# laiviet/ed-gated-gcn

Measured on AMD Instinct MI355X. Metric: gated_gcn_forward_edges_per_sec, higher is better.
Workload: dtype f32 (fp16 MFMA + block-scaled fp8 correction MFMA, fp32 accumulate)

## Files before the change

### ed-gated-gcn_amd/_capi.py

```python
import ctypes
import os

_HERE = os.path.dirname(os.path.abspath(__file__))
_LIB = None

c_i32, c_i64, c_vp, c_sz = ctypes.c_int, ctypes.c_int64, ctypes.c_void_p, ctypes.c_size_t

PROTOTYPES = {
    "ggcn_abi_version": (c_i32, []),
    "ggcn_has_f16mx6": (c_i32, []),
    "ggcn_last_error": (ctypes.c_char_p, []),
    "ggcn_csr_workspace_bytes": (c_sz, [c_i64]),
    "ggcn_csr_from_dense": (c_i32, [c_vp, c_i32, c_i32, c_i32, c_i64, c_i64, c_i64, c_vp, c_vp, c_vp,
                                    c_i64, c_vp, c_vp, c_vp, c_vp]),
    "ggcn_rowmask_from_dense": (c_i32, [c_vp, c_i32, c_i32, c_i32, c_i64, c_i64, c_i64, c_vp, c_vp, c_vp]),
    "ggcn_csr_transpose": (c_i32, [c_vp, c_vp, c_vp, c_i32, c_i32, c_vp, c_vp, c_vp, c_vp, c_vp]),
    "ggcn_csr_rowmask": (c_i32, [c_vp, c_vp, c_i32, c_i32, c_vp, c_vp]),
    "ggcn_graph_edge_lists_bytes": (c_sz, [c_i32]),
    "ggcn_graph_edge_lists": (c_i32, [c_vp, c_i32, c_i32, c_vp, c_vp]),
    "ggcn_graph_operands_bytes": (c_sz, [c_i32]),
    "ggcn_graph_operands": (c_i32, [c_vp, c_i32, c_i32, c_vp, c_vp]),
    "ggcn_graph_operands2_bytes": (c_sz, [c_i32]),
    "ggcn_graph_operands2": (c_i32, [c_vp, c_i32, c_i32, c_i32, c_vp, c_vp]),
    "ggcn_graph_operands_weighted": (c_i32, [c_vp, c_vp, c_vp, c_i32, c_i32, c_i32, c_vp, c_vp, c_vp]),
    "ggcn_layer_fused_weighted": (c_i32, [c_vp, c_i64, c_vp, c_vp, c_vp, c_vp, c_i32, c_i32, c_i32, c_i32, c_vp, c_vp, c_vp,
                                          c_vp, c_i64, c_vp, c_vp, c_vp, c_vp, c_vp, c_i32, c_vp]),
    "ggcn_layer_fused": (c_i32, [c_vp, c_i64, c_vp, c_vp, c_vp, c_vp, c_i32, c_i32, c_i32, c_i32, c_vp, c_vp, c_vp,
                                 c_vp, c_i64, c_vp, c_vp, c_vp, c_vp, c_vp, c_i32, c_vp]),
    "ggcn_layer_fused_prebias": (c_i32, [c_vp, c_i64, c_vp, c_vp, c_vp, c_vp, c_i32, c_i32, c_i32, c_i32, c_vp, c_vp, c_vp,
                                         c_vp, c_i64, c_vp, c_vp, c_i32, c_vp]),
    "ggcn_block_fused": (c_i32, [c_vp, c_i64, c_vp, c_vp, c_vp, c_vp, c_vp, c_vp, c_vp, c_i32, c_i32, c_i32, c_i32,
                                 c_vp, c_vp, c_vp, c_i64, c_vp, c_i64, c_vp, c_vp, c_vp, c_vp, c_i32, c_vp]),
    "ggcn_overlap_reduce": (c_i32, [c_vp, c_i32, c_i32, c_vp, c_vp]),
    "ggcn_transpose": (c_i32, [c_vp, c_i32, c_i32, c_i64, c_vp, c_vp]),
    "ggcn_gate_mlp": (c_i32, [c_vp, c_i64, c_i32, c_i32, c_vp, c_vp, c_vp, c_vp, c_vp, c_vp, c_vp, c_vp, c_vp, c_vp, c_vp]),
    "ggcn_scores_head": (c_i32, [c_vp, c_i64, c_vp, c_i64, c_vp, c_i64, c_vp, c_i64, c_vp, c_vp, c_i64, c_i32, c_i32,
                                 c_i32, c_i32, c_vp, c_i64, c_vp, c_vp]),
    "ggcn_absmax": (c_i32, [c_vp, c_i32, c_i64, c_i64, c_i32, c_vp, c_vp]),
    "ggcn_range_flag": (c_i32, [c_vp, c_i32, c_vp]),
    "ggcn_debug_poison_lds": (c_i32, [ctypes.c_uint32, c_vp]),
    "ggcn_lab_block_fused8": (c_i32, [c_vp, c_i64, c_vp, c_vp, c_vp, c_vp, c_vp, c_vp, c_vp, c_i32, c_i32, c_i32, c_i32, c_vp, c_vp,
                                      c_vp, c_i64, c_vp, c_vp, c_vp, c_vp, c_vp, c_vp]),
    "ggcn_debug_mfma_calibrate": (c_i32, [c_i32, c_i32, c_vp, c_vp, c_vp]),
    "ggcn_debug_block_fused_stamped": (c_i32, [c_vp, c_i64, c_vp, c_vp, c_vp, c_vp, c_vp, c_vp, c_vp, c_i32, c_i32, c_i32, c_i32,
                                               c_vp, c_vp, c_vp, c_i64, c_vp, c_i64, c_vp, c_vp, c_vp, c_vp, c_i32, c_vp, c_vp]),
    "ggcn_subword_pool": (c_i32, [c_vp, c_i64, c_i64, c_i64, c_vp, c_i64, c_i64, c_vp, c_i64, c_i64,
                                  c_i32, c_i32, c_i32, c_i32, c_vp]),
    "ggcn_subword_pool_bf16": (c_i32, [c_vp, c_i64, c_i64, c_i64, c_vp, c_i64, c_i64, c_vp, c_i64, c_i64,
                                       c_i32, c_i32, c_i32, c_i32, c_vp]),
    "ggcn_linear_bf16": (c_i32, [c_vp, c_i64, c_vp, c_vp, c_i64, c_i64, c_i32, c_i32, c_vp]),
    "ggcn_linear_out_bf16": (c_i32, [c_vp, c_i64, c_vp, c_vp, c_i64, c_i64, c_i32, c_i32, c_vp]),
    "ggcn_layer_fused_bf16": (c_i32, [c_vp, c_i64, c_vp, c_vp, c_vp, c_i32, c_i32, c_i32, c_i32, c_vp, c_vp, c_vp,
                                      c_vp, c_i64, c_vp, c_vp, c_vp, c_vp, c_vp, c_vp]),
    "ggcn_layer_fused_bf16_drop": (c_i32, [c_vp, c_i64, c_vp, c_vp, c_vp, c_i32, c_i32, c_i32, c_i32, c_vp, c_vp, c_vp,
                                           c_vp, c_i64, c_vp, c_vp, c_vp, c_vp, c_vp,
                                           ctypes.c_float, ctypes.c_uint64, c_i32, c_i32, c_i32, c_vp]),
    "ggcn_layer_fused_bf16_wide": (c_i32, [c_vp, c_i64, c_vp, c_vp, c_vp, c_vp, c_i32, c_i32, c_i32, c_i32, c_vp, c_vp, c_vp,
                                           c_vp, c_i64, c_vp, c_vp, c_vp, c_vp, c_vp,
                                           ctypes.c_float, ctypes.c_uint64, c_i32, c_i32, c_i32, c_vp]),
    "ggcn_block_fused_bf16": (c_i32, [c_vp, c_i64, c_vp, c_vp, c_vp, c_vp, c_vp, c_vp, c_vp, c_i32, c_i32, c_i32, c_i32,
                                      c_vp, c_vp, c_vp, c_i64, c_vp, c_i64, c_vp, c_vp, c_vp, c_vp, c_vp]),
    "ggcn_aggregate_bf16": (c_i32, [c_vp, c_i64, c_vp, c_vp, c_vp, c_i32, c_i32, c_i32, c_vp, c_i64, c_vp]),
    "ggcn_dweight_bf16_workspace_bytes": (c_sz, [c_i64, c_i32, c_i32]),
    "ggcn_dweight_bf16": (c_i32, [c_vp, c_i64, c_vp, c_i64, c_i64, c_i32, c_i32, c_vp, c_i64, c_vp, c_vp]),
    "ggcn_weight_pack_bytes": (c_sz, [c_i32, c_i32, c_i32]),
    "ggcn_weight_pack": (c_i32, [c_vp, c_i64, c_i32, c_i32, c_i32, c_i32, c_vp, c_vp]),
    "ggcn_linear": (c_i32, [c_vp, c_i64, c_vp, c_i64, c_vp, c_vp, c_i64, c_i64, c_i32, c_i32, c_i32, c_vp]),
    "ggcn_aggregate": (c_i32, [c_vp, c_i64, c_vp, c_vp, c_vp, c_vp, c_i32, c_i32, c_i32, c_vp, c_vp, c_vp,
                               c_vp, c_i64, c_vp, c_vp, c_vp]),
    "ggcn_gate_pool_backward": (c_i32, [c_vp, c_i64, c_vp, c_vp, c_vp, c_vp, c_i64, c_vp, c_vp, c_i32, c_i32, c_i32,
                                        c_vp, c_i64, c_vp, c_vp, c_vp, c_vp, c_vp]),
    "ggcn_gate_pool_backward_drop": (c_i32, [c_vp, c_i64, c_vp, c_vp, c_vp, c_vp, c_i64, c_vp, c_vp, c_i32, c_i32, c_i32,
                                             c_vp, c_i64, c_vp, c_vp, c_vp, c_vp, ctypes.c_float, ctypes.c_uint64, c_i32, c_i32, c_i32, c_vp]),
    "ggcn_gate_pool_backward_agg": (c_i32, [c_vp, c_i64, c_vp, c_vp, c_vp, c_vp, c_i64, c_vp, c_vp, c_vp, c_i32, c_i32, c_i32,
                                            c_vp, c_i64, c_vp, c_vp, c_vp, c_vp, ctypes.c_float, ctypes.c_uint64, c_i32, c_i32, c_i32, c_vp, c_vp]),
    "ggcn_rowmask_transpose": (c_i32, [c_vp, c_i32, c_i32, c_vp, c_vp]),
    "ggcn_gate_pool_backward_mma": (c_i32, [c_vp, c_i64, c_vp, c_vp, c_vp, c_vp, c_i64, c_vp, c_vp, c_vp, c_vp, c_i32, c_i32, c_i32,
                                            c_vp, c_i64, c_vp, c_vp, c_vp, c_vp, c_vp, c_vp]),
    "ggcn_linear_scaled": (c_i32, [c_vp, c_i64, c_vp, c_vp, c_i64, c_i64, c_i32, c_i32, c_vp, c_vp]),
    "ggcn_layer_fused_drop": (c_i32, [c_vp, c_i64, c_vp, c_vp, c_vp, c_vp, c_i32, c_i32, c_i32, c_i32, c_vp, c_vp, c_vp,
                                      c_vp, c_i64, c_vp, c_vp, c_i32, ctypes.c_float, ctypes.c_uint64, c_i32, c_i32, c_i32, c_vp]),
    "ggcn_dropout_mask": (c_i32, [c_i64, c_i32, ctypes.c_float, ctypes.c_uint64, c_i32, c_vp, c_vp]),
    "ggcn_colsum_workspace_bytes": (c_sz, [c_i32]),
    "ggcn_colsum": (c_i32, [c_vp, c_i64, c_i64, c_i32, c_vp, c_vp, c_vp]),
    "ggcn_dweight_workspace_bytes": (c_sz, [c_i64, c_i32, c_i32, c_i32]),
    "ggcn_dweight": (c_i32, [c_vp, c_i64, c_vp, c_i64, c_i64, c_i32, c_i32, c_vp, c_i64, c_i32, c_vp, c_vp]),
    "ggcn_inv_denominators": (c_i32, [c_vp, c_vp, c_i64, c_vp, c_vp]),
    "ggcn_aggregate_t": (c_i32, [c_vp, c_i64, c_vp, c_vp, c_vp, c_vp, c_i32, c_i32, c_i32, c_vp, c_i64, c_vp]),
    "ggcn_adjacency_grad": (c_i32, [c_vp, c_i64, c_vp, c_i64, c_vp, c_vp, c_vp, c_vp, c_i32, c_i32, c_i32, c_vp, c_vp]),
    "ggcn_linear_h": (c_i32, [c_vp, c_i64, c_vp, c_vp, c_i64, c_i64, c_i32, c_i32, c_i32, c_vp]),
    "ggcn_aggregate_h": (c_i32, [c_vp, c_i64, c_vp, c_vp, c_vp, c_vp, c_i32, c_i32, c_i32, c_vp, c_vp, c_vp,
                                 c_vp, c_i64, c_vp, c_vp, c_vp]),
    "ggcn_layer_fused_h": (c_i32, [c_vp, c_i64, c_vp, c_vp, c_vp, c_vp, c_vp, c_i32, c_i32, c_i32, c_i32, c_vp, c_vp, c_vp,
                                   c_vp, c_i64, c_vp, c_vp, c_vp]),
    "ggcn_block_fused_form": (c_i32, [c_i32, c_i32, c_i32, c_i32]),
    "ggcn_dense_head": (c_i32, [c_vp, c_i64, c_vp, c_i64, c_vp, c_i32, c_i32, c_i32, c_vp, c_i64, c_vp, c_i32, c_vp, c_vp]),
    "ggcn_dense_head_signal": (c_i32, [c_vp, c_i64, c_vp, c_i64, c_vp, c_i32, c_i32, c_i32, c_vp, c_i64, c_vp, c_i32, c_vp, c_vp, c_vp]),
    "ggcn_overlap_workspace_bytes": (c_sz, [c_i32]),
    "ggcn_gate_overlap": (c_i32, [c_vp, c_vp, c_i32, c_i32, c_vp, c_vp, c_vp]),
}

ABI_VERSION = 14
PREC = {"bf16x3": 0, "fp32": 1, "f16mx8": 2, "f16": 3, "f16mx6": 4}
PACKED = ("bf16x3", "f16mx8", "f16", "f16mx6")
FLAG_WEIGHTED = 1
RANGE_OVERFLOW, RANGE_WINDOW, RANGE_HIDDEN = 1, 2, 4


def has_f16mx6():
    return bool(load_library().ggcn_has_f16mx6())


def lib_path():
    return os.environ.get("GGCN_LIB", os.path.join(_HERE, "libggcn_hip.so"))


def load_library():
    global _LIB
    if _LIB is not None:
        return _LIB
    path = lib_path()
    if not os.path.exists(path):
        raise RuntimeError(
            "libggcn_hip.so not found at %s: build it with `python -c 'import __graft_entry__ as g; "
            "g.build()'` or `make -C ed-gated-gcn_amd/csrc` (no CPU fallback exists)" % path)
    lib = ctypes.CDLL(path)
    for name, (res, args) in PROTOTYPES.items():
        fn = getattr(lib, name)
        fn.restype, fn.argtypes = res, args
    if lib.ggcn_abi_version() != ABI_VERSION:
        raise RuntimeError("libggcn_hip.so ABI %d != binding ABI %d" % (lib.ggcn_abi_version(), ABI_VERSION))
    _LIB = lib
    return lib


def check(rc, what):
    if rc != 0:
        msg = load_library().ggcn_last_error().decode("utf-8", "replace")
        raise RuntimeError("%s failed (code %d): %s" % (what, rc, msg))


def ptr(t):
    return None if t is None else ctypes.c_void_p(t.data_ptr())


def stream_of(device):
    import torch
    return ctypes.c_void_p(torch.cuda.current_stream(device).cuda_stream)
```

### ed-gated-gcn_amd/csrc/capi.hip

```cpp
#include "common.h"
#include <cstdlib>
#include "dropout_hash.h"

#include <cstring>

namespace ggcn {

char *error_buffer()
{
    static thread_local char buf[512] = "";
    return buf;
}

int fail(int code, const char *fmt, ...)
{
    va_list ap;
    va_start(ap, fmt);
    vsnprintf(error_buffer(), 512, fmt, ap);
    va_end(ap);
    return code;
}

}

using namespace ggcn;

extern "C" {

int ggcn_abi_version(void) { return GGCN_ABI_VERSION; }

int ggcn_has_f16mx6(void)
{
#ifdef GGCN_WITH_F16MX6
    return 1;
#else
    return 0;
#endif
}

const char *ggcn_last_error(void) { return error_buffer(); }

size_t ggcn_csr_workspace_bytes(int64_t n_rows) { return csr_workspace_bytes(n_rows); }

int ggcn_csr_from_dense(const void *adj, int adj_dtype, int B, int T, int64_t stride_b,
                        int64_t stride_r, int64_t stride_c, int32_t *rowptr, int32_t *colidx,
                        float *vals, int64_t capacity, uint32_t *rowmask, int32_t *flags,
                        void *workspace, ggcn_stream_t stream)
{
    return csr_from_dense(adj, adj_dtype, B, T, stride_b, stride_r, stride_c, rowptr, colidx, vals,
                          capacity, rowmask, flags, workspace, as_stream(stream));
}

int ggcn_csr_transpose(const int32_t *rowptr, const int32_t *colidx, const float *vals, int B, int T,
                       int32_t *rowptr_t, int32_t *colidx_t, float *vals_t, void *workspace, ggcn_stream_t stream)
{
    return csr_transpose(rowptr, colidx, vals, B, T, rowptr_t, colidx_t, vals_t, workspace, as_stream(stream));
}

int ggcn_rowmask_from_dense(const void *adj, int adj_dtype, int B, int T, int64_t stride_b, int64_t stride_r,
                            int64_t stride_c, uint32_t *rowmask, int32_t *flags, ggcn_stream_t stream)
{
    return rowmask_from_dense(adj, adj_dtype, B, T, stride_b, stride_r, stride_c, rowmask, flags, as_stream(stream));
}

int ggcn_csr_rowmask(const int32_t *rowptr, const int32_t *colidx, int B, int T, uint32_t *rowmask,
                     ggcn_stream_t stream)
{
    return csr_rowmask(rowptr, colidx, B, T, rowmask, as_stream(stream));
}

size_t ggcn_graph_operands_bytes(int B) { return B > 0 ? (size_t)B * GGCN_GRAPH_OPS_BYTES : 0; }
size_t ggcn_graph_operands2_bytes(int B) { return B > 0 ? (size_t)B * GGCN_GRAPH_OPS2_BYTES : 0; }
int ggcn_graph_operands2(const uint32_t *rowmask, int B, int T, int plane, void *graph_ops2, ggcn_stream_t stream)
{
    return graph_operands2(rowmask, B, T, plane, graph_ops2, as_stream(stream));
}

size_t ggcn_graph_edge_lists_bytes(int B) { return B > 0 ? (size_t)B * GGCN_EDGE_LISTS_BYTES : 0; }

int ggcn_graph_edge_lists(const uint32_t *rowmask, int B, int T, void *lists, ggcn_stream_t stream)
{
    return graph_edge_lists(rowmask, B, T, lists, as_stream(stream));
}

int ggcn_graph_operands(const uint32_t *rowmask, int B, int T, void *graph_ops, ggcn_stream_t stream)
{
    return graph_operands(rowmask, B, T, graph_ops, as_stream(stream));
}

int ggcn_layer_fused(const float *X, int64_t ldx, const void *wpack, const uint32_t *rowmask, const void *graph_ops,
                     const float *bias, int B, int T, int K, int F, const float *store_gate,
                     const float *pool_gate_a, const float *pool_gate_b, float *out, int64_t ldo,
                     float *pool_a, float *pool_b, float *overlap_partial, const float *overlap_in,
                     float *overlap_out, int precision, ggcn_stream_t stream)
{
    return layer_fused(X, ldx, wpack, rowmask, graph_ops, bias, B, T, K, F, store_gate, pool_gate_a, pool_gate_b, out,
                       ldo, pool_a, pool_b, overlap_partial, overlap_in, overlap_out, precision, as_stream(stream));
}

int ggcn_layer_fused_prebias(const float *X, int64_t ldx, const void *wpack, const uint32_t *rowmask, const float *bias,
                             const float *bias_pre, int B, int T, int K, int F, const float *store_gate,
                             const float *pool_gate_a, const float *pool_gate_b, float *out, int64_t ldo,
                             float *pool_a, float *pool_b, int precision, ggcn_stream_t stream)
{
    if (!bias_pre) return fail(GGCN_EINVAL, "ggcn_layer_fused_prebias: null bias_pre (ggcn_layer_fused is the plain form)");
    return layer_fused(X, ldx, wpack, rowmask, nullptr, bias, B, T, K, F, store_gate, pool_gate_a, pool_gate_b, out,
                       ldo, pool_a, pool_b, nullptr, nullptr, nullptr, precision, as_stream(stream), nullptr, bias_pre);
}

int ggcn_graph_operands_weighted(const int32_t *rowptr, const int32_t *colidx, const float *vals, int B, int T, int plane,
                                 void *graph_opsw, int32_t *flag, ggcn_stream_t stream)
{
    return graph_operands_weighted(rowptr, colidx, vals, B, T, plane, graph_opsw, flag, as_stream(stream));
}

int ggcn_layer_fused_weighted(const float *X, int64_t ldx, const void *wpack, const void *graph_opsw, const float *bias,
                              const float *zero_mid, int B, int T, int K, int F, const float *store_gate,
                              const float *pool_gate_a, const float *pool_gate_b, float *out, int64_t ldo, float *pool_a,
                              float *pool_b, float *overlap_partial, const float *overlap_in, float *overlap_out, int precision,
                              ggcn_stream_t stream)
{
    return layer_fused_weighted(X, ldx, wpack, graph_opsw, bias, zero_mid, B, T, K, F, store_gate, pool_gate_a, pool_gate_b, out, ldo,
                                pool_a, pool_b, overlap_partial, overlap_in, overlap_out, precision, as_stream(stream));
}

int ggcn_block_fused(const float *X, int64_t ldx, const void *wpack1, const void *wpack12, const void *graph_ops,
                     const void *graph_ops2, const float *bias1, const float *bias_mid, const float *bias2, int B, int T, int K, int F,
                     const float *gate1, const float *gate2, float *gcn1, int64_t ld1, float *x_out, int64_t ld2,
                     float *x1, float *y1, float *pool_out, float *overlap_partial, int precision,
                     ggcn_stream_t stream)
{
    return block_fused(X, ldx, wpack1, wpack12, graph_ops, graph_ops2, bias1, bias_mid, bias2, B, T, K, F, gate1, gate2, gcn1, ld1,
                       x_out, ld2, x1, y1, pool_out, overlap_partial, precision, as_stream(stream));
}

int ggcn_overlap_reduce(const float *partials, int B, int F, float *xy, ggcn_stream_t stream)
{
    return overlap_reduce(partials, B, F, xy, as_stream(stream));
}

size_t ggcn_weight_pack_bytes(int K, int F, int precision) { return weight_pack_bytes(K, F, precision); }

int ggcn_weight_pack(const float *W, int64_t ldw, int K, int F, int precision, int transposed, void *wpack,
                     ggcn_stream_t stream)
{
    return weight_pack(W, ldw, K, F, precision, transposed != 0, wpack, as_stream(stream));
}

int ggcn_aggregate_t(const float *G, int64_t ldg, const int32_t *rowptr_t, const int32_t *colidx_t,
                     const float *vals_t, const float *src_scale, int B, int T, int F, float *out, int64_t ldo,
                     ggcn_stream_t stream)
{
    return aggregate_t(G, ldg, rowptr_t, colidx_t, vals_t, src_scale, B, T, F, out, ldo, as_stream(stream));
}

int ggcn_inv_denominators(const int32_t *rowptr, const float *vals, int64_t n_rows, float *inv,
                          ggcn_stream_t stream)
{
    return inv_denominators(rowptr, vals, n_rows, inv, as_stream(stream));
}

int ggcn_adjacency_grad(const float *dY, int64_t ldy, const float *hidden, int64_t ldh, const float *inv, const int32_t *rowptr,
                        const int32_t *colidx, const float *vals, int B, int T, int F, float *d_adj, ggcn_stream_t stream)
{
    return adjacency_grad(dY, ldy, hidden, ldh, inv, rowptr, colidx, vals, B, T, F, d_adj, as_stream(stream));
}

int ggcn_linear(const float *X, int64_t ldx, const float *W, int64_t ldw, const void *wpack, float *Y,
                int64_t ldy, int64_t M, int K, int F, int precision, ggcn_stream_t stream)
{
    if (!X || !Y) return fail(GGCN_EINVAL, "ggcn_linear: null pointer");
    if (M <= 0 || K <= 0 || F <= 0)
        return fail(GGCN_EINVAL, "ggcn_linear: M=%lld K=%d F=%d must be positive", (long long)M, K, F);
    if (ldx < K || ldy < F) return fail(GGCN_EINVAL, "ggcn_linear: leading dimension too small");
    switch (precision) {
        case GGCN_PREC_BF16X3:
        case GGCN_PREC_F16MX8:
            return linear_packed(X, ldx, wpack, Y, ldy, M, K, F, precision, as_stream(stream));
        case GGCN_PREC_FP32:
            if (!W) return fail(GGCN_EINVAL, "ggcn_linear(fp32): W is NULL");
            if (ldw < F) return fail(GGCN_EINVAL, "ggcn_linear(fp32): ldw < F");
            return linear_fp32(X, ldx, W, ldw, Y, ldy, M, K, F, as_stream(stream));
        default:
            return fail(GGCN_EINVAL, "ggcn_linear: unknown precision %d", precision);
    }
}

int ggcn_linear_bf16(const void *X, int64_t ldx, const void *wpack, float *Y, int64_t ldy, int64_t M, int K, int F,
                     ggcn_stream_t stream)
{
    if (!X || !Y || !wpack) return fail(GGCN_EINVAL, "ggcn_linear_bf16: null pointer");
    if (M <= 0 || K <= 0 || F <= 0)
        return fail(GGCN_EINVAL, "ggcn_linear_bf16: M=%lld K=%d F=%d must be positive", (long long)M, K, F);
    if (ldx < K || ldy < F) return fail(GGCN_EINVAL, "ggcn_linear_bf16: leading dimension too small");
    if (reinterpret_cast<uintptr_t>(X) % 2 || reinterpret_cast<uintptr_t>(Y) % 4)
        return fail(GGCN_EINVAL, "ggcn_linear_bf16: X / Y not aligned to their element size");
    return linear_bf16(X, ldx, wpack, Y, ldy, M, K, F, as_stream(stream));
}

int ggcn_linear_out_bf16(const float *X, int64_t ldx, const void *wpack, void *Y, int64_t ldy, int64_t M, int K, int F,
                         ggcn_stream_t stream)
{
    if (!X || !Y || !wpack) return fail(GGCN_EINVAL, "ggcn_linear_out_bf16: null pointer");
    if (M <= 0 || K <= 0 || F <= 0)
        return fail(GGCN_EINVAL, "ggcn_linear_out_bf16: M=%lld K=%d F=%d must be positive", (long long)M, K, F);
    if (ldx < K || ldy < F) return fail(GGCN_EINVAL, "ggcn_linear_out_bf16: leading dimension too small");
    if (reinterpret_cast<uintptr_t>(X) % 4 || reinterpret_cast<uintptr_t>(Y) % 2)
        return fail(GGCN_EINVAL, "ggcn_linear_out_bf16: X / Y not aligned to their element size");
    return linear_out_bf16(X, ldx, wpack, Y, ldy, M, K, F, as_stream(stream));
}

namespace {
int bf16_entry_checks(const char *who, const void *X, float p, int sel_store, int sel_a, int sel_b)
{
    if (X && reinterpret_cast<uintptr_t>(X) % 2) return fail(GGCN_EINVAL, "%s: X not 2-byte aligned", who);
    if (!(p >= 0.0f && p < 1.0f) || sel_store < 0 || sel_store > 2 || sel_a < 0 || sel_a > 2 || sel_b < 0 || sel_b > 2)
        return fail(GGCN_EINVAL, "%s: p=%g streams %d %d %d", who, (double)p, sel_store, sel_a, sel_b);
    return GGCN_OK;
}
}

int ggcn_layer_fused_bf16(const void *X, int64_t ldx, const void *wpack, const void *graph_ops, const float *bias, int B, int T,
                          int K, int F, const float *store_gate, const float *pool_gate_a, const float *pool_gate_b, float *out,
                          int64_t ldo, float *pool_a, float *pool_b, float *overlap_partial, const float *overlap_in,
                          float *overlap_out, ggcn_stream_t stream)
{
    const char *who = "ggcn_layer_fused_bf16";
    if (int rc = bf16_entry_checks(who, X, 0.0f, 0, 0, 0)) return rc;
    if (T > 32) return fail(GGCN_EUNSUPPORTED, "%s: T=%d > 32 (use ggcn_layer_fused_bf16_wide up to %d nodes, ggcn_linear_bf16 + ggcn_aggregate beyond)", who, T, GGCN_MASK_MAX_T);
    return layer_fused_bf16(who, X, ldx, wpack, nullptr, graph_ops, bias, B, T, K, F, store_gate, pool_gate_a, pool_gate_b, out, ldo, pool_a,
                            pool_b, overlap_partial, overlap_in, overlap_out, as_stream(stream));
}

int ggcn_layer_fused_bf16_drop(const void *X, int64_t ldx, const void *wpack, const void *graph_ops, const float *bias, int B, int T,
                               int K, int F, const float *store_gate, const float *pool_gate_a, const float *pool_gate_b, float *out,
                               int64_t ldo, float *pool_a, float *pool_b, float *overlap_partial, const float *overlap_in,
                               float *overlap_out, float p, uint64_t seed, int sel_store, int sel_a, int sel_b, ggcn_stream_t stream)
{
    const char *who = "ggcn_layer_fused_bf16_drop";
    if (int rc = bf16_entry_checks(who, X, p, sel_store, sel_a, sel_b)) return rc;
    if (T > 32) return fail(GGCN_EUNSUPPORTED, "%s: T=%d > 32 (use ggcn_layer_fused_bf16_wide up to %d nodes)", who, T, GGCN_MASK_MAX_T);
    const DropSpec d = make_drop_spec(p, seed, sel_store, sel_a, sel_b);
    return layer_fused_bf16(who, X, ldx, wpack, nullptr, graph_ops, bias, B, T, K, F, store_gate, pool_gate_a, pool_gate_b, out, ldo, pool_a,
                            pool_b, overlap_partial, overlap_in, overlap_out, as_stream(stream), &d);
}

int ggcn_layer_fused_bf16_wide(const void *X, int64_t ldx, const void *wpack, const uint32_t *rowmask, const void *edge_lists,
                               const float *bias, int B, int T, int K, int F, const float *store_gate, const float *pool_gate_a,
                               const float *pool_gate_b, float *out, int64_t ldo, float *pool_a, float *pool_b, float *overlap_partial,
                               const float *overlap_in, float *overlap_out, float p, uint64_t seed, int sel_store, int sel_a, int sel_b,
                               ggcn_stream_t stream)
{
    const char *who = "ggcn_layer_fused_bf16_wide";
    if (int rc = bf16_entry_checks(who, X, p, sel_store, sel_a, sel_b)) return rc;
    if (T <= 32) return fail(GGCN_EUNSUPPORTED, "%s: T=%d <= 32 (use ggcn_layer_fused_bf16 / ggcn_layer_fused_bf16_drop)", who, T);
    if (T > GGCN_MASK_MAX_T) return fail(GGCN_EUNSUPPORTED, "%s: T=%d > %d (use ggcn_linear_bf16 + ggcn_aggregate)", who, T, GGCN_MASK_MAX_T);
    const DropSpec d = make_drop_spec(p, seed, sel_store, sel_a, sel_b);
    return layer_fused_bf16(who, X, ldx, wpack, rowmask, T > 128 ? edge_lists : nullptr, bias, B, T, K, F, store_gate, pool_gate_a,
                            pool_gate_b, out, ldo, pool_a, pool_b, overlap_partial, overlap_in, overlap_out, as_stream(stream), &d);
}

int ggcn_block_fused_bf16(const void *X, int64_t ldx, const void *wpack1, const void *wpack12, const void *graph_ops,
                          const void *graph_ops2, const float *bias1, const float *bias_mid, const float *bias2, int B, int T, int K,
                          int F, const float *gate1, const float *gate2, float *gcn1, int64_t ld1, float *x_out, int64_t ld2,
                          float *x1, float *y1, float *pool_out, float *overlap_partial, ggcn_stream_t stream)
{
    if (int rc = bf16_entry_checks("ggcn_block_fused_bf16", X, 0.0f, 0, 0, 0)) return rc;
    return block_fused_bf16(X, ldx, wpack1, wpack12, graph_ops, graph_ops2, bias1, bias_mid, bias2, B, T, K, F, gate1, gate2, gcn1, ld1,
                            x_out, ld2, x1, y1, pool_out, overlap_partial, as_stream(stream));
}

int ggcn_aggregate_bf16(const void *X, int64_t ldx, const int32_t *rowptr, const int32_t *colidx, const float *vals, int B, int T,
                        int K, float *Z, int64_t ldz, ggcn_stream_t stream)
{
    return aggregate_bf16(X, ldx, rowptr, colidx, vals, B, T, K, Z, ldz, as_stream(stream));
}

int ggcn_aggregate(const float *Hd, int64_t ldh, const int32_t *rowptr, const int32_t *colidx,
                   const float *vals, const float *bias, int B, int T, int F, const float *store_gate,
                   const float *pool_gate_a, const float *pool_gate_b, float *out, int64_t ldo,
                   float *pool_a, float *pool_b, ggcn_stream_t stream)
{
    return aggregate(Hd, ldh, rowptr, colidx, vals, bias, B, T, F, store_gate, pool_gate_a, pool_gate_b,
                     out, ldo, pool_a, pool_b, as_stream(stream));
}

int ggcn_linear_h(const void *X, int64_t ldx, const void *wpack, void *Y, int64_t ldy, int64_t M, int K, int F,
// ... 246 lines not shown
```

### ed-gated-gcn_amd/csrc/common.h

```cpp
#pragma once
#include <hip/hip_runtime.h>
#include <cstdarg>
#include <cstdint>
#include <cstdio>

#include "../../include/ggcn.h"

namespace ggcn {

struct DropSpec;
constexpr int kWave = 64;

char *error_buffer();
int fail(int code, const char *fmt, ...);

inline hipStream_t as_stream(ggcn_stream_t s) { return reinterpret_cast<hipStream_t>(s); }

inline int check_launch(const char *what) {
    hipError_t e = hipGetLastError();
    if (e != hipSuccess) return fail(GGCN_ELAUNCH, "%s: %s", what, hipGetErrorString(e));
    return GGCN_OK;
}

inline bool aligned16(const void *p) { return (reinterpret_cast<uintptr_t>(p) & 15u) == 0; }

int csr_from_dense(const void *adj, int adj_dtype, int B, int T, int64_t sb, int64_t sr, int64_t sc,
                   int32_t *rowptr, int32_t *colidx, float *vals, int64_t capacity, uint32_t *rowmask,
                   int32_t *flags, void *workspace, hipStream_t st);
size_t csr_workspace_bytes(int64_t n_rows);
int csr_transpose(const int32_t *rowptr, const int32_t *colidx, const float *vals, int B, int T, int32_t *rowptr_t,
                  int32_t *colidx_t, float *vals_t, void *workspace, hipStream_t st);
int rowmask_from_dense(const void *adj, int adj_dtype, int B, int T, int64_t sb, int64_t sr, int64_t sc,
                       uint32_t *rowmask, int32_t *flags, hipStream_t st);

int linear_fp32(const float *X, int64_t ldx, const float *W, int64_t ldw, float *Y, int64_t ldy,
                int64_t M, int K, int F, hipStream_t st);

size_t weight_pack_bytes(int K, int F, int precision);
int weight_pack(const float *W, int64_t ldw, int K, int F, int precision, bool transposed, void *wpack, hipStream_t st);
int linear_packed(const float *X, int64_t ldx, const void *wpack, float *Y, int64_t ldy,
                  int64_t M, int K, int F, int precision, hipStream_t st);

bool linear_scaled_takes(const float *X, int64_t ldx, const float *Y, int64_t ldy, int K, int F);
int linear_scaled(const float *X, int64_t ldx, const void *wpack, float *Y, int64_t ldy, int64_t M, int K, int F, const float *amax,
                  hipStream_t st);
int linear_packed_h(const void *X, int64_t ldx, const void *wpack, void *Y, int64_t ldy, int64_t M, int K,
                    int F, int precision, hipStream_t st);
int linear_bf16(const void *X, int64_t ldx, const void *wpack, float *Y, int64_t ldy, int64_t M, int K, int F, hipStream_t st);
int linear_out_bf16(const float *X, int64_t ldx, const void *wpack, void *Y, int64_t ldy, int64_t M, int K, int F, hipStream_t st);
int aggregate_t(const float *G, int64_t ldg, const int32_t *rowptr_t, const int32_t *colidx_t,
                const float *vals_t, const float *src_scale, int B, int T, int F, float *out, int64_t ldo,
                hipStream_t st);
int inv_denominators(const int32_t *rowptr, const float *vals, int64_t n, float *inv, hipStream_t st);
int adjacency_grad(const float *dY, int64_t ldy, const float *hidden, int64_t ldh, const float *inv, const int32_t *rowptr,
                   const int32_t *colidx, const float *vals, int B, int T, int F, float *d_adj, hipStream_t st);
int aggregate_h(const void *Hd, int64_t ldh, const int32_t *rowptr, const int32_t *colidx, const float *vals,
                const float *bias, int B, int T, int F, const float *store_gate, const float *pool_gate_a,
                const float *pool_gate_b, void *out, int64_t ldo, float *pool_a, float *pool_b, hipStream_t st);

int layer_fused_h(const void *X, int64_t ldx, const void *wpack, const int32_t *rowptr, const int32_t *colidx,
                  const float *vals, const float *bias, int B, int T, int K, int F, const float *store_gate,
                  const float *pool_gate_a, const float *pool_gate_b, void *out, int64_t ldo, float *pool_a,
                  float *pool_b, hipStream_t st);

int aggregate(const float *Hd, int64_t ldh, const int32_t *rowptr, const int32_t *colidx,
              const float *vals, const float *bias, int B, int T, int F, const float *store_gate,
              const float *pool_gate_a, const float *pool_gate_b, float *out, int64_t ldo,
              float *pool_a, float *pool_b, hipStream_t st);

int aggregate_bf16(const void *X, int64_t ldx, const int32_t *rowptr, const int32_t *colidx, const float *vals, int B, int T, int K,
                   float *Z, int64_t ldz, hipStream_t st);

int subword_pool(const float *A, int64_t sa_b, int64_t sa_r, int64_t sa_c, const float *X, int64_t x_batch,
                 int64_t ldx, float *Y, int64_t y_batch, int64_t ldy, int B, int R, int C, int D, hipStream_t st);
int subword_pool_bf16(const float *A, int64_t sa_b, int64_t sa_r, int64_t sa_c, const void *X, int64_t x_batch,
                      int64_t ldx, void *Y, int64_t y_batch, int64_t ldy, int B, int R, int C, int D, hipStream_t st);
int csr_rowmask(const int32_t *rowptr, const int32_t *colidx, int B, int T, uint32_t *rowmask, hipStream_t st);
int graph_operands(const uint32_t *rowmask, int B, int T, void *ops, hipStream_t st);
int graph_edge_lists(const uint32_t *rowmask, int B, int T, void *lists, hipStream_t st);
int graph_operands2(const uint32_t *rowmask, int B, int T, int plane, void *ops2, hipStream_t st);
int graph_operands_weighted(const int32_t *rowptr, const int32_t *colidx, const float *vals, int B, int T, int plane, void *ops,
                            int *flag, hipStream_t st);
int layer_fused_weighted(const float *X, int64_t ldx, const void *wpack, const void *graph_opsw, const float *bias, const float *zero_mid,
                         int B, int T, int K, int F, const float *store_gate, const float *pool_gate_a, const float *pool_gate_b,
                         float *out, int64_t ldo, float *pool_a, float *pool_b, float *overlap_partial, const float *overlap_in,
                         float *overlap_out, int precision, hipStream_t st);
int layer_fused(const float *X, int64_t ldx, const void *wpack, const uint32_t *rowmask, const void *graph_ops, const float *bias,
                int B, int T, int K, int F, const float *store_gate, const float *pool_gate_a,
                const float *pool_gate_b, float *out, int64_t ldo, float *pool_a, float *pool_b,
                float *overlap_partial, const float *overlap_in, float *overlap_out, int precision, hipStream_t st,
                const struct DropSpec *drop = nullptr, const float *bias_pre = nullptr);
int layer_fused_bf16(const char *who, const void *X, int64_t ldx, const void *wpack, const uint32_t *rowmask, const void *graph_ops,
                     const float *bias, int B, int T, int K, int F,
                     const float *store_gate, const float *pool_gate_a, const float *pool_gate_b, float *out, int64_t ldo,
                     float *pool_a, float *pool_b, float *overlap_partial, const float *overlap_in, float *overlap_out,
                     hipStream_t st, const struct DropSpec *drop = nullptr);
int block_fused_bf16(const void *X, int64_t ldx, const void *wpack1, const void *wpack12, const void *graph_ops, const void *graph_ops2,
                     const float *bias1, const float *bias_mid, const float *bias2, int B, int T, int K, int F,
                     const float *gate1, const float *gate2, float *gcn1, int64_t ld1, float *x_out, int64_t ld2,
                     float *x1, float *y1, float *pool_out, float *overlap_partial, hipStream_t st);
int dropout_mask(int64_t rows, int F, float p, uint64_t seed, int sel, float *out, hipStream_t st);

int block_fused(const float *X, int64_t ldx, const void *wpack1, const void *wpack12, const void *graph_ops, const void *graph_ops2,
                const float *bias1, const float *bias_mid, const float *bias2, int B, int T, int K, int F,
                const float *gate1, const float *gate2, float *gcn1, int64_t ld1, float *x_out, int64_t ld2,
                float *x1, float *y1, float *pool_out, float *overlap_partial, int precision, hipStream_t st,
                unsigned long long *stamps = nullptr);
int mfma_calibrate(int n_wg, int stages, unsigned long long *stamps, float *sink, hipStream_t st);
int overlap_reduce(const float *partials, int B, int F, float *xy, hipStream_t st);

int gate_pool_backward(const float *out, int64_t ldo, const float *store_gate, const float *gate_a,
                       const float *gate_b, const float *d_out, int64_t ldd, const float *d_pa,
                       const float *d_pb, int B, int T, int F, float *dY, int64_t ldy, float *d_sg,
                       float *d_ga, float *d_gb, float *d_bsum, hipStream_t st, const struct DropSpec *drop = nullptr);
int gate_pool_backward_agg(const float *out, int64_t ldo, const float *store_gate, const float *gate_a,
                           const float *gate_b, const float *d_out, int64_t ldd, const float *d_pa,
                           const float *d_pb, const uint32_t *rowmask, int B, int T, int F, float *dH, int64_t ldh,
                           float *d_sg, float *d_ga, float *d_gb, float *d_bsum, hipStream_t st, const struct DropSpec *drop = nullptr,
                           float *dh_amax = nullptr);
int rowmask_transpose(const uint32_t *rowmask, int B, int T, uint32_t *rowmask_t, hipStream_t st);
int gate_pool_backward_mma(const float *out, int64_t ldo, const float *store_gate, const float *gate_a, const float *gate_b,
                           const float *d_out, int64_t ldd, const float *d_pa, const float *d_pb, const void *graph_ops,
                           const void *graph_ops_t, int B, int T, int F, float *dH, int64_t ldh, float *d_sg, float *d_ga,
                           float *d_gb, float *d_bsum, float *dh_amax, hipStream_t st);
size_t colsum_workspace_bytes(int F);
int colsum(const float *X, int64_t ld, int64_t M, int F, float *out, void *workspace, hipStream_t st);

size_t dweight_workspace_bytes(int64_t N, int K, int F);
size_t dweight_bx3_workspace_bytes(int64_t N, int K, int F);
bool dweight_tn_takes(const float *X, int64_t ldx, const float *G, int64_t ldg, int64_t N, int K, int F);
size_t dweight_tn_workspace_bytes(int64_t N, int K, int F);
int dweight_tn(const float *X, int64_t ldx, const float *G, int64_t ldg, int64_t N, int K, int F, float *dW, int64_t lddw,
               void *workspace, hipStream_t st);
int dweight_bx3(const float *X, int64_t ldx, const float *G, int64_t ldg, int64_t N, int K, int F, float *dW,
                int64_t lddw, void *workspace, hipStream_t st);
size_t dweight_bf16_workspace_bytes(int64_t N, int K, int F);
int dweight_bf16(const void *X, int64_t ldx, const float *G, int64_t ldg, int64_t N, int K, int F, float *dW,
                 int64_t lddw, void *workspace, hipStream_t st);
int weight_pack_rows(const float *W, int64_t ldw, int64_t K_valid, int F, int k_steps_total, void *pack, hipStream_t st);
int dweight(const float *X, int64_t ldx, const float *G, int64_t ldg, int64_t N, int K, int F, float *dW,
            int64_t lddw, void *workspace, hipStream_t st);

int absmax(const void *X, int is_half, int64_t ld, int64_t M, int K, float *out, hipStream_t st);
int poison_lds(uint32_t pattern, hipStream_t st);
int range_flag_linear(unsigned int *dst, int clear, hipStream_t st);
int range_flag_fused(unsigned int *dst, int clear, hipStream_t st);
int range_flag_wide(unsigned int *dst, int clear, hipStream_t st);
int range_flag_wide8(unsigned int *dst, int clear, hipStream_t st);
int range_flag_block8(unsigned int *dst, int clear, hipStream_t st);
int lab_block_fused8(const float *X, int64_t ldx, const void *wpack1, const void *wpack12, const void *graph_ops, const void *graph_ops2,
                     const float *bias1, const float *bias_mid, const float *bias2, int B, int T, int K, int F, const float *gate1,
                     const float *gate2, float *x_out, int64_t ld2, float *x1, float *y1, float *pool_out, float *overlap_partial,
                     hipStream_t st, unsigned long long *stamps = nullptr, int flags = 0);
constexpr int kBlock8RowMajor = 1, kBlock8NoDma = 2, kBlock8SameSlots = 4, kBlock8Product = 8;
bool block8_shape(int B, int T, int K, int F);
bool block8_takes(const float *X, int64_t ldx, const void *wpack1, const void *wpack12, int B, int T, int K, int F, const float *gate1,
                  const float *gate2, const float *bias1, const float *bias_mid, const float *bias2, const void *graph_ops,
                  const void *graph_ops2, const float *x_out, int64_t ld2);
int range_flag_fused6(unsigned int *dst, int clear, hipStream_t st);

int transpose_f32(const float *W, int rows, int cols, int64_t ldw, float *Wt, hipStream_t st);
int gate_mlp(const float *aspect, int64_t lda, int B, int H, const float *w1t_a, const float *b1_a, const float *w2t_a,
             const float *b2_a, float *gate_a, const float *w1t_b, const float *b1_b, const float *w2t_b,
             const float *b2_b, float *gate_b, hipStream_t st);
int scores_head(const float *X, int64_t ldx, const float *aspect, int64_t lda, const float *logits, int64_t ldl,
                const float *fcw, int64_t ldw, const float *fcb, const float *dist, int64_t ldd, int B, int T, int H,
                int C, float *scores, int64_t lds_, float *kl_part, hipStream_t st);

int dense_head(const float *pooled, int64_t ldp, const float *Wt, int64_t ldw, const float *bias, int B, int H, int C,
               float *logits, int64_t ldl, const float *partials, int F_block, float *xy, hipStream_t st, unsigned *signal = nullptr);

size_t overlap_workspace_bytes(int B);
int gate_overlap(const float *x1, const float *y1, int B, int F, float *xy, void *workspace,
                 hipStream_t st);

}
```

### ed-gated-gcn_amd/csrc/fused_block8.hip

```cpp
#include "fused_common.h"

#include <cstdlib>

namespace ggcn {
namespace {

constexpr int kB8Threads = 512;
constexpr int kB8Lds = kLdsBytes + 2 * kEpiLdsBytes;

__device__ __forceinline__ bool getenv_slot_same(const FusedArgs &a) { return (a.k_steps & 0x20000000) != 0; }

template <int BASE>
__device__ __forceinline__ float staged_mid_max(const char *lds, bool dma, int lane)
{
    if (dma) {
        const float4 m4 = *reinterpret_cast<const float4 *>(lds + EpiLds<BASE>::kBias + BN * 4 + lane * 16);
        float mm = fmaxf(fmaxf(fabsf(m4.x), fabsf(m4.y)), fmaxf(fabsf(m4.z), fabsf(m4.w)));
#pragma unroll
        for (int d = 32; d >= 1; d >>= 1) mm = fmaxf(mm, __shfl_xor(mm, d));
        return mm;
    }
    const float4 mm = *reinterpret_cast<const float4 *>(lds + EpiLds<BASE>::kMidMax);
    return fmaxf(fmaxf(mm.x, mm.y), fmaxf(mm.z, mm.w));
}

template <bool FULLT, bool VST>
__global__ __launch_bounds__(kB8Threads, 1) void block_fused8_kernel(const FusedArgs a)
{
    extern __shared__ __attribute__((aligned(16))) char lds[];
    const int B = a.B, T = a.T, K = a.K, F = a.F;
    int n_wgi, g_tile;
    if (a.n_parts == 2) {
        const int xcd = blockIdx.x & 7, qb = blockIdx.x >> 3;
        const int total = a.g_tiles * a.n_wg, per_xcd = (total + 7) >> 3;
        const int w = xcd * per_xcd + qb;
        if (qb >= per_xcd || w >= total) return;
        n_wgi = w / a.g_tiles;
        g_tile = w - n_wgi * a.g_tiles;
    } else {
        if (!tile_of_block(blockIdx.x, a.g_tiles, a.n_wg, g_tile, n_wgi)) return;
    }

    const int tid8 = threadIdx.x;
    const unsigned long long t_start = a.stamps ? __builtin_amdgcn_s_memrealtime() : 0;
    const int group = __builtin_amdgcn_readfirstlane(tid8 >> 8);
    const int tid = tid8 & 255;
    const int wave = __builtin_amdgcn_readfirstlane(tid >> 6);
    const LayerPart &lp = a.part[group];
    const int gt0 = g_tile * 4, g0 = gt0;
    const int n_tiles_total = (F + NT - 1) / NT;
    const int nt0 = n_wgi * (BN / NT) + wave * RN;

    constexpr int NP = Geom<float>::NP;
    const float *arow[NP];
    bool avalid[NP];
    int rel[NP];
#pragma unroll
    for (int i = 0; i < NP; ++i) {
        const int row = stage_row<float>(i < 2 ? i + 2 * group : 0);
        const int g = gt0 + (row >> 5), r = row & 31;
        avalid[i] = i < 2 && (g < B) && (FULLT || r < T);
        arow[i] = a.X;
        rel[i] = avalid[i] ? (row >> 5) * T + (row & 31) : -1;
    }
    const bool dma = (a.n_wg * BN == F) && (gt0 + 4 <= B) && a.ov_in == nullptr && a.ov_out == nullptr && (a.k_steps & 0x40000000) != 0;
    const int k_steps = a.k_steps & 0x1fffffff;
    if (dma) {
        if (group == 0) stage_epilogue_operands_dma<kLdsBytes>(a, lp, g0, n_wgi, lds, tid);
        else stage_epilogue_operands_dma<kLdsBytes + kEpiLdsBytes>(a, lp, g0, n_wgi, lds, tid);
    } else {
        if (group == 0) stage_epilogue_operands<kLdsBytes>(a, lp, g0, n_wgi, lds, tid);
        else stage_epilogue_operands<kLdsBytes + kEpiLdsBytes>(a, lp, g0, n_wgi, lds, tid);
    }

    f32x16 acc[4][RN];
    float amax;
    const int64_t pack_bytes = (int64_t)n_tiles_total * (k_steps / 2) * mx8::STAGE_PACK_BYTES;
    const float bw1 = *reinterpret_cast<const float *>(a.part[0].wpack + pack_bytes);
    const float bw12 = *reinterpret_cast<const float *>(a.part[1].wpack + pack_bytes);
    const unsigned long long t_loop0 = a.stamps ? __builtin_amdgcn_s_memrealtime() : 0;
    mx8::BufX<float> bx = mx8::make_bufx<float>(a.X, a.ldx, (int64_t)gt0 * T, (int64_t)B * T, rel, tid);
    if (group == 0 || getenv_slot_same(a))
        mx8::mainloop<float, true, true, !FULLT, false, true, 4, false, 2, 0>(arow, avalid, lp.wpack, K, k_steps / 2, 0, nt0, n_tiles_total, lds, acc, 0, 4,
                                                                               &amax, &bx, 1.0f, 2 * group);
    else
        mx8::mainloop<float, true, true, !FULLT, false, true, 4, false, 2, 2>(arow, avalid, lp.wpack, K, k_steps / 2, 0, nt0, n_tiles_total, lds, acc, 0, 4,
                                                                               &amax, &bx, 1.0f, 2 * group);
    unsigned long long t_loop1 = 0;
    if (a.stamps) { asm volatile("" :: "v"(acc[3][RN - 1][15])); t_loop1 = __builtin_amdgcn_s_memrealtime(); }
    mx8::range_verdict(amax, bw12, staged_mid_max<kLdsBytes + kEpiLdsBytes>(lds, dma, tid & 63), true);
    mx8::range_verdict(amax, bw1, 0.0f, false);
    if (group == 0) {
        epilogue<1, FULLT, VST, false, false, kLdsBytes>(a, lp, acc, g0, nt0, n_tiles_total, lds, tid);
    } else {
        if (lp.out) epilogue<1, FULLT, VST, true, true, kLdsBytes + kEpiLdsBytes>(a, lp, acc, g0, nt0, n_tiles_total, lds, tid);
        else epilogue<1, FULLT, VST, true, false, kLdsBytes + kEpiLdsBytes>(a, lp, acc, g0, nt0, n_tiles_total, lds, tid);
    }
    if (a.stamps && tid == 0) {
        unsigned long long *o = a.stamps + ((size_t)blockIdx.x * 2 + group) * 4;
        o[0] = t_start; o[1] = t_loop0; o[2] = t_loop1; o[3] = __builtin_amdgcn_s_memrealtime();
    }
}

}

int device_cu_count()
{
    static int cus = 0;
    if (cus == 0) {
        int dev = 0, n = 0;
        if (hipGetDevice(&dev) != hipSuccess || hipDeviceGetAttribute(&n, hipDeviceAttributeMultiprocessorCount, dev) != hipSuccess || n <= 0) n = 256;
        cus = n;
    }
    return cus;
}
bool block8_shape(int B, int T, int K, int F)
{
    if (B <= 0 || T > 32 || T <= 0 || F <= 0 || K <= 0 || F % BN != 0 || K % BK != 0) return false;
    const int64_t total = (int64_t)((B + 3) / 4) * (F / BN), cus = device_cu_count();
    return total >= 6 * cus || (total >= 3 * cus && total % cus == 0);
}
bool block8_takes(const float *X, int64_t ldx, const void *wpack1, const void *wpack12, int B, int T, int K, int F, const float *gate1,
                  const float *gate2, const float *bias1, const float *bias_mid, const float *bias2, const void *graph_ops,
                  const void *graph_ops2, const float *x_out, int64_t ld2)
{
    if (!block8_shape(B, T, K, F)) return false;
    if (ldx < K || !aligned16(wpack1) || !aligned16(wpack12) || (x_out && ld2 < F)) return false;
    if (!((ldx % 4 == 0) && aligned16(X) && (int64_t)ldx * 4 * 257 < ((int64_t)1 << 31))) return false;
    if (!graph_ops || !graph_ops2 || !gate1 || !gate2 || !bias_mid) return false;
    if (!(aligned16(gate1) && aligned16(gate2) && aligned16(bias1) && aligned16(bias2) && aligned16(bias_mid) && aligned16(graph_ops) &&
          aligned16(graph_ops2)))
        return false;
    if (x_out && !((ld2 % 4 == 0) && aligned16(x_out) && (int64_t)T * ld2 * 4 < ((int64_t)1 << 31))) return false;
    return true;
}

int lab_block_fused8(const float *X, int64_t ldx, const void *wpack1, const void *wpack12, const void *graph_ops, const void *graph_ops2,
                     const float *bias1, const float *bias_mid, const float *bias2, int B, int T, int K, int F, const float *gate1,
                     const float *gate2, float *x_out, int64_t ld2, float *x1, float *y1, float *pool_out, float *overlap_partial,
                     hipStream_t st, unsigned long long *stamps, int flags)
{
    const char *who = (flags & kBlock8Product) ? "ggcn_block_fused" : "ggcn_lab_block_fused8";
    if (!X || !wpack1 || !wpack12 || !graph_ops || !graph_ops2 || !gate1 || !gate2 || !x1 || !y1 || !bias_mid)
        return fail(GGCN_EINVAL, "%s: null pointer", who);
    if (B <= 0 || T <= 0 || T > 32 || K <= 0 || F <= 0) return fail(GGCN_EUNSUPPORTED, "%s: B=%d T=%d K=%d F=%d (graphs of <= 32 nodes)", who, B, T, K, F);
    if (ldx < K) return fail(GGCN_EINVAL, "%s: ldx < K", who);
    if (!aligned16(wpack1) || !aligned16(wpack12)) return fail(GGCN_EINVAL, "%s: wpack must be 16-byte aligned", who);
    if (x_out && ld2 < F) return fail(GGCN_EINVAL, "%s: leading dimension of the output too small", who);
    const bool avec = (K % 4 == 0) && (ldx % 4 == 0) && aligned16(X) && (int64_t)ldx * 4 * 257 < ((int64_t)1 << 31);
    if (!avec || K % BK != 0) return fail(GGCN_EUNSUPPORTED, "%s: fast shapes only (K %% 32 == 0, 16-byte aligned rows)", who);
    if (!x_out && !pool_out) return fail(GGCN_EINVAL, "%s: neither x nor its pool requested", who);
    FusedArgs a = {};
    a.X = X; a.ldx = ldx; a.graph_ops = static_cast<const char *>(graph_ops); a.graph_ops2 = static_cast<const char *>(graph_ops2);
    const bool rowmajor = (flags & kBlock8RowMajor) != 0;
    a.B = B; a.T = T; a.K = K; a.F = F; a.n_parts = rowmajor ? 3 : 2;
    a.part[0] = LayerPart{static_cast<const char *>(wpack1), bias1, nullptr, nullptr, nullptr, gate1, gate2, nullptr, x1, y1, overlap_partial, 0};
    a.part[1] = LayerPart{static_cast<const char *>(wpack12), bias2, bias_mid, nullptr, gate2, gate2, nullptr, x_out, pool_out, nullptr, nullptr, (int)ld2};
    a.stamps = stamps;
    a.k_steps = round_up(K, BK) / KSTEP;
    const bool al = (F % 4 == 0) && aligned16(gate1) && aligned16(gate2) && aligned16(bias1) && aligned16(bias2) && aligned16(bias_mid) &&
                    aligned16(graph_ops) && aligned16(graph_ops2) && !(flags & kBlock8NoDma);
    if (al) a.k_steps |= 0x40000000;
    if (flags & kBlock8SameSlots) a.k_steps |= 0x20000000;
    a.n_wg = (F + BN - 1) / BN;
    a.g_tiles = (B + 3) / 4;
    const bool vst = x_out && (F % 4 == 0) && (ld2 % 4 == 0) && aligned16(x_out) && (int64_t)T * ld2 * 4 < ((int64_t)1 << 31);
    if (x_out && !vst) return fail(GGCN_EUNSUPPORTED, "%s: x needs F %% 4 == 0 and 16-byte aligned rows", who);
    const bool fullt = (T == 32) && (B % 4 == 0);
    const int64_t total = (int64_t)a.g_tiles * a.n_wg;
    const int64_t grid = rowmajor ? grid_for(a.g_tiles, a.n_wg) : 8 * ((total + 7) / 8);
    if (grid > (int64_t)INT32_MAX) return fail(GGCN_EUNSUPPORTED, "%s: batch too large", who);
#define GGCN_L8(FT, VS)                                                                                                           \
    do {                                                                                                                          \
        auto kern = block_fused8_kernel<FT, VS>;                                                                                  \
        if (hipFuncSetAttribute(reinterpret_cast<const void *>(kern), hipFuncAttributeMaxDynamicSharedMemorySize, kB8Lds) != hipSuccess) \
            return fail(GGCN_ELAUNCH, "%s: cannot reserve %d bytes of LDS", who, kB8Lds);                                         \
        hipLaunchKernelGGL(kern, dim3((unsigned)grid), dim3(kB8Threads), kB8Lds, st, a);                                          \
    } while (0)
    if (fullt && vst) GGCN_L8(true, true);
    else if (fullt) GGCN_L8(true, false);
    else if (vst) GGCN_L8(false, true);
    else GGCN_L8(false, false);
#undef GGCN_L8
    return check_launch(who);
}

GGCN_RANGE_FLAG_TU(range_flag_block8)

}
```

### ed-gated-gcn_amd/csrc/fused_common.h

```cpp
#pragma once
#include "f16mx8_core.h"
#include "dropout_hash.h"
#include "lab_hooks.h"

namespace ggcn {

struct LayerPart {
    const char *wpack;
    const float *bias;
    const float *mid;
    const float *pre;
    const float *store_gate;
    const float *pool_gate_a;
    const float *pool_gate_b;
    float *out;
    float *pool_a, *pool_b;
    float *ov_partial;
    int ldo;
};

struct FusedArgs {
    const float *X;
    int64_t ldx;
    const uint32_t *rowmask;
    const char *graph_ops;
    const char *graph_ops2;
    const float *ov_in;
    float *ov_out;
    int B, T, K, F;
    int g_tiles, n_wg, n_parts, k_steps;
    LayerPart part[2];
    DropSpec drop;
    unsigned long long *stamps;
    const __bf16 *Xb;
};


int launch_fused_wide(const char *who, const FusedArgs &a, int precision, int sb, bool fast, bool vst, int64_t grid, hipStream_t st);
int launch_fused_wide8(const char *who, const FusedArgs &a, int precision, bool fast, bool vst, int64_t grid, hipStream_t st);
int launch_fused6(const char *who, const FusedArgs &a, bool fullt, bool vst, int64_t grid, hipStream_t st);

namespace {

using namespace bx3;

template <typename XT>
__device__ __forceinline__ const XT *fused_x(const FusedArgs &a)
{
    if constexpr (std::is_same<XT, float>::value) return a.X;
    else return a.Xb;
}

__device__ __forceinline__ void split2(const f32x16 &acc, bf16x8 (&frag)[2][2])
{
#pragma unroll
    for (int s = 0; s < 2; ++s)
#pragma unroll
        for (int j = 0; j < 8; ++j) {
            const float v = acc[8 * s + j];
            const __bf16 p0 = (__bf16)v;
            frag[0][s][j] = p0;
            frag[1][s][j] = (__bf16)(v - (float)p0);
        }
}

__device__ __forceinline__ void store_out4(float *p, const float4 &v)
{
#if GGCN_LAB_NT_STORE
    typedef float f4 __attribute__((ext_vector_type(4)));
    __builtin_nontemporal_store(f4{v.x, v.y, v.z, v.w}, reinterpret_cast<f4 *>(p));
#else
    *reinterpret_cast<float4 *>(p) = v;
#endif
}

__device__ __forceinline__ void store_out4_stream(float *p, const float4 &v)
{
    typedef float f4 __attribute__((ext_vector_type(4)));
    __builtin_nontemporal_store(f4{v.x, v.y, v.z, v.w}, reinterpret_cast<f4 *>(p));
}

__device__ __forceinline__ float upper_half_to_lower(float v)
{
    const auto r = __builtin_amdgcn_permlane32_swap(__float_as_uint(v), __float_as_uint(v), false, false);
    return __uint_as_float(r[1]);
}

__device__ __forceinline__ void expand_mask(uint32_t mh, bf16x8 (&af)[2])
{
    typedef unsigned short u16x2 __attribute__((ext_vector_type(2)));
    typedef short i16x2 __attribute__((ext_vector_type(2)));
    union { bf16x8 v; uint32_t w[4]; } u[2];
#pragma unroll
    for (int s = 0; s < 2; ++s) {
        const uint32_t m16 = s == 0 ? (mh & 0xFFFFu) : (mh >> 16);
        const u16x2 both = __builtin_bit_cast(u16x2, m16 | (m16 << 16));
#pragma unroll
        for (int q = 0; q < 4; ++q) {
            const int b = 8 * (q >> 1) + 2 * (q & 1);
            const u16x2 top = both << u16x2{(unsigned short)(15 - b), (unsigned short)(14 - b)};
            const i16x2 spread = __builtin_bit_cast(i16x2, top) >> i16x2{15, 15};
            u[s].w[q] = __builtin_bit_cast(uint32_t, spread) & 0x3F803F80u;
        }
    }
    af[0] = u[0].v;
    af[1] = u[1].v;
}

__device__ __forceinline__ f32x16 adj_times(const bf16x8 (&af)[2], const f32x16 &t)
{
    bf16x8 hfrag[2][2];
    split2(t, hfrag);
    f32x16 y;
#pragma unroll
    for (int r = 0; r < 16; ++r) y[r] = 0.0f;
#pragma unroll
    for (int p = 1; p >= 0; --p)
#pragma unroll
        for (int s = 0; s < 2; ++s) y = __builtin_amdgcn_mfma_f32_32x32x16_bf16(af[s], hfrag[p][s], y, 0, 0, 0);
    return y;
}


constexpr int kOpsBytes = GGCN_GRAPH_OPS_BYTES;
static_assert(kOpsBytes == 2048 + 128, "layout above");
constexpr int kOps2Bytes = GGCN_GRAPH_OPS2_BYTES;
static_assert(kOps2Bytes == 4096 + 128, "layout above");
constexpr float kM2Scale = 1024.0f, kM2InvScale = 1.0f / 1024.0f;


typedef _Float16 f16x8e __attribute__((ext_vector_type(8)));
__device__ __forceinline__ void split2h(const f32x16 &acc, f16x8e (&frag)[2][2])
{
    typedef _Float16 h2 __attribute__((ext_vector_type(2)));
    typedef float f2 __attribute__((ext_vector_type(2)));
    union { f16x8e v; uint32_t w[4]; } hi[2], lo[2];
#pragma unroll
    for (int s = 0; s < 2; ++s)
#pragma unroll
        for (int q = 0; q < 4; ++q) {
            const float v0 = acc[8 * s + 2 * q], v1 = acc[8 * s + 2 * q + 1];
            const h2 p = __builtin_convertvector(f2{v0, v1}, h2);
            uint32_t l;
            asm("v_fma_mixlo_f16 %0, %1, -1.0, %2 op_sel_hi:[1,0,0]" : "=v"(l) : "v"(p), "v"(v0));
            asm("v_fma_mixhi_f16 %0, %1, -1.0, %2 op_sel:[1,0,0] op_sel_hi:[1,0,0]" : "+v"(l) : "v"(p), "v"(v1));
            hi[s].w[q] = __builtin_bit_cast(uint32_t, p);
            lo[s].w[q] = l;
        }
    frag[0][0] = hi[0].v; frag[0][1] = hi[1].v;
    frag[1][0] = lo[0].v; frag[1][1] = lo[1].v;
}

template <int SCH> struct AggPlane;
template <> struct AggPlane<0> {
    typedef bf16x8 frag;
    static constexpr uint32_t kOne = 0x3F803F80u;
    static __device__ __forceinline__ void split(const f32x16 &t, frag (&f)[2][2]) { split2(t, f); }
    static __device__ __forceinline__ f32x16 mma(const frag &a, const frag &b, const f32x16 &c) { return __builtin_amdgcn_mfma_f32_32x32x16_bf16(a, b, c, 0, 0, 0); }
};
template <> struct AggPlane<1> {
    typedef f16x8e frag;
    static constexpr uint32_t kOne = 0x3C003C00u;
    static __device__ __forceinline__ void split(const f32x16 &t, frag (&f)[2][2]) { split2h(t, f); }
    static __device__ __forceinline__ f32x16 mma(const frag &a, const frag &b, const f32x16 &c) { return __builtin_amdgcn_mfma_f32_32x32x16_f16(a, b, c, 0, 0, 0); }
};

template <> struct AggPlane<2> : AggPlane<1> {};

__device__ __forceinline__ void reduce_partials(const float *__restrict__ part, int n_part, int B, float *__restrict__ dst,
                                                float *red)
{
    float sdot = 0.0f;
    for (int idx = threadIdx.x; idx < n_part; idx += kThreads) sdot += part[idx];
#pragma unroll
    for (int d = 32; d >= 1; d >>= 1) sdot += __shfl_xor(sdot, d);
    if ((threadIdx.x & 63) == 0) red[threadIdx.x >> 6] = sdot;
    __syncthreads();
    if (threadIdx.x == 0) *dst = ((red[0] + red[1]) + (red[2] + red[3])) / (float)B;
    __syncthreads();
}


template <int BASE>
struct EpiLds {
    static constexpr int kOps = BASE;
    static constexpr int kGate = kOps + 4 * kOps2Bytes;
    static constexpr int kBias = kGate + 3 * 4 * BN * 4;
// ... 131 lines not shown
    v += __uint_as_float(__builtin_amdgcn_update_dpp(0, __float_as_uint(v), 0x140, 0xF, 0xF, true));
    const float r1 = __uint_as_float(__builtin_amdgcn_readlane(__float_as_uint(v), 16));
    const float r2 = __uint_as_float(__builtin_amdgcn_readlane(__float_as_uint(v), 32));
    const float r3 = __uint_as_float(__builtin_amdgcn_readlane(__float_as_uint(v), 48));
    return (v + r1) + (r2 + r3);
}

__device__ __forceinline__ __amdgpu_buffer_rsrc_t out_rsrc(void *p)
{
    return __builtin_amdgcn_make_buffer_rsrc(p, 0, 0x7fffffff, 0x00020000);
}

template <int SCH, bool FULLT, bool VST, bool MID, bool OUT, int BASE = kLdsBytes, bool DROP = false>
__device__ __forceinline__ void epilogue(const FusedArgs &a, const LayerPart &lp, f32x16 (&acc)[4][RN], int g0, int nt0,
                                         int n_tiles_total, char *lds, int tid)
{
    constexpr int kEpiOps = EpiLds<BASE>::kOps, kEpiGate = EpiLds<BASE>::kGate, kEpiBias = EpiLds<BASE>::kBias;
    using P = AggPlane<SCH>;
    typedef typename P::frag frag;
    const int B = a.B, T = a.T, F = a.F;
    float *__restrict__ out = lp.out, *__restrict__ pool_a = lp.pool_a, *__restrict__ pool_b = lp.pool_b;
    float *__restrict__ ov_partial = lp.ov_partial;
    const int ldo = lp.ldo;
    const int lane = tid & 63;
    const int wave = __builtin_amdgcn_readfirstlane(tid >> 6);
    const int c = lane & 31, h = lane >> 5;

    const char *ops_lds = lds + kEpiOps;
    const float *gate_lds = reinterpret_cast<const float *>(lds + kEpiGate);
    const float *bias_lds = reinterpret_cast<const float *>(lds + kEpiBias);
    const int wn = wave % WN;
    float vb[RN], vmid[RN];
    bool col_ok[RN];
#pragma unroll
    for (int j = 0; j < RN; ++j) {
        col_ok[j] = (nt0 + j) * NT + c < F;
        vb[j] = bias_lds[wn * (RN * NT) + j * NT + c];
        vmid[j] = bias_lds[BN + wn * (RN * NT) + j * NT + c];
    }
    const int lane_off = 4 * h * ldo + c;
    float *stage_lds = reinterpret_cast<float *>(lds) + wave * (32 * 64);
    constexpr bool vst = VST && OUT;
    constexpr bool direct_store = !VST && OUT;

#pragma unroll
    for (int i = 0; i < 4; ++i) {
        const int g = g0 + i;
        if (!FULLT && g >= B) break;
        constexpr int kBlk = MID ? kOps2Bytes : kOpsBytes;
        constexpr int kRowOff = MID ? 4096 : 2048;
        frag afv[2], afl[2];
#pragma unroll
        for (int s = 0; s < 2; ++s) {
            const uint4 raw = *reinterpret_cast<const uint4 *>(ops_lds + i * kBlk + s * 1024 + lane * 16);
            union { frag v; uint32_t w[4]; } u;
            if constexpr (MID) {
                u.w[0] = raw.x; u.w[1] = raw.y; u.w[2] = raw.z; u.w[3] = raw.w;
                afv[s] = u.v;
                const uint4 rl = *reinterpret_cast<const uint4 *>(ops_lds + i * kBlk + 2048 + s * 1024 + lane * 16);
                u.w[0] = rl.x; u.w[1] = rl.y; u.w[2] = rl.z; u.w[3] = rl.w;
                afl[s] = u.v;
            } else {
                u.w[0] = raw.x & P::kOne; u.w[1] = raw.y & P::kOne;
                u.w[2] = raw.z & P::kOne; u.w[3] = raw.w & P::kOne;
                afv[s] = u.v;
            }
        }
        float4 rv[4];
#pragma unroll
        for (int q = 0; q < 4; ++q) rv[q] = *reinterpret_cast<const float4 *>(ops_lds + i * kBlk + kRowOff + h * 64 + q * 16);
        float vsg[RN], vga[RN], vgb[RN];
#pragma unroll
        for (int j = 0; j < RN; ++j) {
            const int at = i * BN + wn * (RN * NT) + j * NT + c;
            vsg[j] = gate_lds[at];
            vga[j] = gate_lds[4 * BN + at];
            vgb[j] = gate_lds[8 * BN + at];
        }
        bool tile_ok[RN];
#pragma unroll
        for (int j = 0; j < RN; ++j) tile_ok[j] = nt0 + j < n_tiles_total;

        f32x16 y[RN];
#pragma unroll
        for (int j = 0; j < RN; ++j) {
            frag hf[2][2];
            P::split(acc[i][j], hf);
#pragma unroll
            for (int r = 0; r < 16; ++r) y[j][r] = 0.0f;
            if constexpr (MID) {
#pragma unroll
                for (int s = 0; s < 2; ++s) y[j] = P::mma(afl[s], hf[0][s], y[j]);
#pragma unroll
                for (int s = 0; s < 2; ++s) y[j] = P::mma(afv[s], hf[1][s], y[j]);
#pragma unroll
                for (int s = 0; s < 2; ++s) y[j] = P::mma(afv[s], hf[0][s], y[j]);
            } else {
#pragma unroll
                for (int p = 1; p >= 0; --p)
#pragma unroll
                    for (int s = 0; s < 2; ++s) { if constexpr (!((GGCN_LAB_EPI) & 2)) y[j] = P::mma(afv[s], hf[p][s], y[j]); else y[j][s] += (float)hf[p][s][0]; }
            }
        }
        float rinv[16];
#pragma unroll
        for (int q = 0; q < 4; ++q) {
            rinv[4 * q] = rv[q].x; rinv[4 * q + 1] = rv[q].y; rinv[4 * q + 2] = rv[q].z; rinv[4 * q + 3] = rv[q].w;
        }
        float dot = 0.0f;
#pragma unroll
        for (int j = 0; j < RN; ++j) {
            if (!tile_ok[j]) break;
            const int gn = (nt0 + j) * NT + c;
            float vmax = -INFINITY, vmin = INFINITY, pmax_a = -INFINITY, pmax_b = -INFINITY;
            float *tile = OUT ? out + ((int64_t)g * T) * ldo + (nt0 + j) * NT : nullptr;
            const float sg = vsg[j];
            const float bj = vb[j];
            const uint32_t didx0 = DROP ? (uint32_t)(((int64_t)g * T + 4 * h) * F + gn) : 0u;
#pragma unroll
            for (int r = 0; r < 16; ++r) {
                const int row0 = (r & 3) + 8 * (r >> 2);
                const float v = MID ? fmaf(y[j][r], kM2InvScale, fmaf(rinv[r], vmid[j], bj)) : y[j][r] * rinv[r] + bj;
                float vs = v * sg;
                if constexpr (DROP) {
                    const uint32_t hh = drop_hash(didx0 + (uint32_t)(row0 * F), a.drop.seed_lo, a.drop.seed_hi);
                    vs *= drop_keep(hh, a.drop.sel[0], a.drop.thr, a.drop.scale);
                    if (FULLT || row0 + 4 * h < T) {
                        pmax_a = fmaxf(pmax_a, v * vga[j] * drop_keep(hh, a.drop.sel[1], a.drop.thr, a.drop.scale));
                        pmax_b = fmaxf(pmax_b, v * vgb[j] * drop_keep(hh, a.drop.sel[2], a.drop.thr, a.drop.scale));
                    }
                }
                if constexpr (vst) {
                    stage_lds[(row0 + 4 * h) * 64 + ((32 * j + c) ^ (32 * h))] = vs;
                }
                if (FULLT || row0 + 4 * h < T) {
                    if (direct_store && col_ok[j]) tile[lane_off + row0 * ldo] = vs;
                    if constexpr (!DROP) {
                        vmax = fmaxf(vmax, v);
                        vmin = fminf(vmin, v);
                    }
                }
            }
            float pa, pb;
            if constexpr (DROP) {
                pa = fmaxf(pmax_a, upper_half_to_lower(pmax_a));
                pb = fmaxf(pmax_b, upper_half_to_lower(pmax_b));
            } else {
                meet_halves(vmax, vmin);
                const float ga = vga[j], gb = vgb[j];
                pa = ga * (ga >= 0.0f ? vmax : vmin);
                pb = gb * (gb >= 0.0f ? vmax : vmin);
            }
            if (h == 0 && col_ok[j]) {
                if (pool_a) __builtin_amdgcn_raw_buffer_store_b32(__float_as_uint(pa), out_rsrc(pool_a + (int64_t)g * F), 4 * gn, 0, 0);
                if (pool_b) __builtin_amdgcn_raw_buffer_store_b32(__float_as_uint(pb), out_rsrc(pool_b + (int64_t)g * F), 4 * gn, 0, 0);
                dot = fmaf(pa, pb, dot);
            }
        }
        if (ov_partial && nt0 < n_tiles_total) {
            const float tot = wave_sum_to_lane0(dot);
            if (lane == 0) ov_partial[(int64_t)g * ((F + 63) / 64) + (nt0 >> 1)] = tot;
        }
        if constexpr (vst) {
            __builtin_amdgcn_fence(__ATOMIC_RELEASE, "wavefront");
            __builtin_amdgcn_wave_barrier();
            const int colq = (lane & 15) * 4;
            const int gcol = nt0 * NT + colq;
            const __amdgpu_buffer_rsrc_t orsrc = out_rsrc(out + ((int64_t)g * T) * ldo);
            const int voff = ((lane >> 4) * ldo + gcol) * 4;
#pragma unroll
            for (int it = 0; it < 8; ++it) {
                const int row = 4 * it + (lane >> 4);
                const float4 v4 = *reinterpret_cast<const float4 *>(&stage_lds[row * 64 + (colq ^ (32 * ((row >> 2) & 1)))]);
                typedef uint32_t u32x4 __attribute__((ext_vector_type(4)));
                if ((FULLT || row < T) && gcol < F && !((GGCN_LAB_EPI) & 1))
                    __builtin_amdgcn_raw_buffer_store_b128(__builtin_bit_cast(u32x4, v4), orsrc, voff, 4 * it * ldo * 4, (GGCN_LAB_NT_STORE) ? 2 : 0);
            }
            __builtin_amdgcn_fence(__ATOMIC_ACQUIRE, "wavefront");
            __builtin_amdgcn_wave_barrier();
        }
        if (i == 0) GGCN_TRACE(7);
    }
}


}
}
```

### ed-gated-gcn_amd/csrc/fused_layer.hip

```cpp
#include "fused_common.h"

#include <cstdlib>

namespace ggcn {
namespace {

__global__ __launch_bounds__(256) void graph_operands_kernel(const uint32_t *__restrict__ rowmask, int B, int T,
                                                             char *__restrict__ ops)
{
    const int lane = threadIdx.x & 63;
    const int g = blockIdx.x * 4 + (threadIdx.x >> 6);
    if (g >= B) return;
    const int r = lane & 31, h = lane >> 5;
    const uint32_t m = r < T ? rowmask[(int64_t)g * T + r] : 0u;
    char *blk = ops + (int64_t)g * kOpsBytes;
#pragma unroll
    for (int s = 0; s < 2; ++s) {
        uint32_t w[4];
#pragma unroll
        for (int q = 0; q < 4; ++q) {
            const int b = 16 * s + 8 * (q >> 1) + 2 * (q & 1) + 4 * h;
            const uint32_t two = (m >> b) & 3u;
            w[q] = (two & 1u) * 0xFFFFu + (two >> 1) * 0xFFFF0000u;
        }
        *reinterpret_cast<uint4 *>(blk + s * 1024 + lane * 16) = make_uint4(w[0], w[1], w[2], w[3]);
    }
    const int rr = lane & 15, hh = (lane >> 4) & 1;
    const int row = (rr & 3) + 8 * (rr >> 2) + 4 * hh;
    const uint32_t mrow = __shfl(m, row);
    if (lane < 32) reinterpret_cast<float *>(blk + 2048)[lane] = 1.0f / (float)(__popc(mrow) + 1);
}

template <int PLANE>
__global__ __launch_bounds__(256) void graph_operands2_kernel(const uint32_t *__restrict__ rowmask, int B, int T,
                                                              char *__restrict__ ops2)
{
    const int lane = threadIdx.x & 63;
    const int g = blockIdx.x * 4 + (threadIdx.x >> 6);
    if (g >= B) return;
    const int r = lane & 31, h = lane >> 5;
    const uint32_t m = r < T ? rowmask[(int64_t)g * T + r] : 0u;
    const float inv_r = 1.0f / (float)(__popc(m) + 1);
    float a2[2][8];
#pragma unroll
    for (int s = 0; s < 2; ++s)
#pragma unroll
        for (int e = 0; e < 8; ++e) a2[s][e] = 0.0f;
    for (int j = 0; j < T; ++j) {
        const uint32_t mj = (uint32_t)__builtin_amdgcn_readlane((int)m, j);
        const float invj = 1.0f / (float)(__popc(mj) + 1);
        if ((m >> j) & 1u) {
#pragma unroll
            for (int s = 0; s < 2; ++s)
#pragma unroll
                for (int e = 0; e < 8; ++e) {
                    const int c = 16 * s + 8 * (e >> 2) + 4 * h + (e & 3);
                    a2[s][e] += ((mj >> c) & 1u) ? invj : 0.0f;
                }
        }
    }
    char *blk = ops2 + (int64_t)g * kOps2Bytes;
#pragma unroll
    for (int s = 0; s < 2; ++s) {
        union { uint4 q; unsigned short u[8]; } hi, lo;
#pragma unroll
        for (int e = 0; e < 8; ++e) {
            const float v = a2[s][e] * inv_r * kM2Scale;
            if constexpr (PLANE == 1) {
                const _Float16 vh = (_Float16)v, vl = (_Float16)(v - (float)vh);
                hi.u[e] = __builtin_bit_cast(unsigned short, vh);
                lo.u[e] = __builtin_bit_cast(unsigned short, vl);
            } else {
                const __bf16 vh = (__bf16)v, vl = (__bf16)(v - (float)vh);
                hi.u[e] = __builtin_bit_cast(unsigned short, vh);
                lo.u[e] = __builtin_bit_cast(unsigned short, vl);
            }
        }
        *reinterpret_cast<uint4 *>(blk + s * 1024 + lane * 16) = hi.q;
        *reinterpret_cast<uint4 *>(blk + 2048 + s * 1024 + lane * 16) = lo.q;
    }
    const int rr = lane & 15, hh = (lane >> 4) & 1;
    const int row = (rr & 3) + 8 * (rr >> 2) + 4 * hh;
    const uint32_t mrow = __shfl(m, row);
    if (lane < 32) reinterpret_cast<float *>(blk + 4096)[lane] = (float)__popc(mrow) / (float)(__popc(mrow) + 1);
}

template <int PLANE>
__global__ __launch_bounds__(256) void graph_operands_w_kernel(const int32_t *__restrict__ rowptr, const int32_t *__restrict__ colidx,
                                                               const float *__restrict__ vals, int B, int T, char *__restrict__ ops,
                                                               int *__restrict__ flag)
{
    const int lane = threadIdx.x & 63;
    const int g = blockIdx.x * 4 + (threadIdx.x >> 6);
    if (g >= B) return;
    const int r = lane & 31, h = lane >> 5;
    const int64_t node0 = (int64_t)g * T;
    float a[16], wsum = 0.0f;
#pragma unroll
    for (int e = 0; e < 16; ++e) a[e] = 0.0f;
    if (r < T) {
        const int e1 = rowptr[node0 + r + 1];
        for (int e = rowptr[node0 + r]; e < e1; ++e) {
            const int c = colidx[e] - (int)node0;
            const float w = vals ? vals[e] : 1.0f;
            wsum += w;
            const int idx = ((unsigned)c < 32u && ((c >> 2) & 1) == h) ? (c >> 4) * 8 + ((c >> 3) & 1) * 4 + (c & 3) : -1;
#pragma unroll
            for (int q = 0; q < 16; ++q) a[q] += idx == q ? w : 0.0f;
        }
    }
    const float inv = 1.0f / (wsum + 1.0f);
    char *blk = ops + (int64_t)g * kOps2Bytes;
    bool bad = false;
#pragma unroll
    for (int s = 0; s < 2; ++s) {
        union { uint4 q; unsigned short u[8]; } hi, lo;
#pragma unroll
        for (int e = 0; e < 8; ++e) {
            const float v = a[8 * s + e] * inv * kM2Scale;
            bad = bad || !(fabsf(v) < (PLANE == 1 ? 60000.0f : 3.0e38f));
            if constexpr (PLANE == 1) {
                const _Float16 vh = (_Float16)v, vl = (_Float16)(v - (float)vh);
                hi.u[e] = __builtin_bit_cast(unsigned short, vh);
                lo.u[e] = __builtin_bit_cast(unsigned short, vl);
            } else {
                const __bf16 vh = (__bf16)v, vl = (__bf16)(v - (float)vh);
                hi.u[e] = __builtin_bit_cast(unsigned short, vh);
                lo.u[e] = __builtin_bit_cast(unsigned short, vl);
            }
        }
        *reinterpret_cast<uint4 *>(blk + s * 1024 + lane * 16) = hi.q;
        *reinterpret_cast<uint4 *>(blk + 2048 + s * 1024 + lane * 16) = lo.q;
    }
    if (lane < 32) reinterpret_cast<float *>(blk + 4096)[lane] = 0.0f;
    if (bad && flag) atomicOr(flag, 1);
}

template <int SCH, bool AVEC, bool KFULL, bool FULLT, bool VST, bool STAMP = false, typename XT = float>
__global__ __launch_bounds__(kThreads, kWavesPerSimd) void layer_fused_kernel(const FusedArgs a)
{
    static_assert(std::is_same<XT, float>::value || (SCH == 0 && !STAMP), "bf16 features: the bf16x3 main loop");
    __shared__ __attribute__((aligned(16))) char lds[kLdsBytes + kEpiLdsBytes + GGCN_LAB_LDS_PAD];
    const int B = a.B, T = a.T, K = a.K, F = a.F;
    if (a.ov_in && blockIdx.x == 0) reduce_partials(a.ov_in, B * ((F + 63) / 64), B, a.ov_out, reinterpret_cast<float *>(lds));
    int g_tile, n_wgi;
    bool second = false;
    if (a.n_parts == 1) {
        if (!tile_of_block(blockIdx.x, a.g_tiles, a.n_wg, g_tile, n_wgi)) return;
    } else {
        const int xcd = blockIdx.x & 7, slot = blockIdx.x >> 3;
        second = xcd >= 4;
        g_tile = (slot / a.n_wg) * 4 + (xcd & 3);
        n_wgi = slot % a.n_wg;
        if (g_tile >= a.g_tiles) return;
    }
    GGCN_TRACE_IDS();
    GGCN_TRACE(3);
    const LayerPart &lp = a.part[second ? 1 : 0];
    const char *__restrict__ wpack = lp.wpack;

    const int tid = threadIdx.x;
    const int wave = __builtin_amdgcn_readfirstlane(tid >> 6);
    const int wm = wave / WN, wn = wave % WN;
    const int gt0 = g_tile * (4 * WM);
    const int g0 = gt0 + wm * 4;
    const int n_tiles_total = (F + NT - 1) / NT;
    const int nt0 = n_wgi * (BN / NT) + wn * RN;

    constexpr int NP = Geom<XT>::NP;
    const XT *arow[NP];
    bool avalid[NP];
#pragma unroll
    for (int i = 0; i < NP; ++i) {
        const int row = stage_row<XT>(i);
        const int g = gt0 + (row >> 5), r = row & 31;
        avalid[i] = (g < B) && (FULLT || r < T);
        const int64_t node = avalid[i] ? (int64_t)g * T + r : 0;
        arow[i] = fused_x<XT>(a) + node * a.ldx;
    }

#if !GGCN_LAB_NO_DMA_STAGE
    const bool dma_stage = SCH == 1 && (a.n_wg * BN == F) && (gt0 + 4 <= B) && a.drop.thr == 0 && (F % 4 == 0) &&
                           ((reinterpret_cast<uintptr_t>(lp.store_gate) | reinterpret_cast<uintptr_t>(lp.pool_gate_a) | reinterpret_cast<uintptr_t>(lp.pool_gate_b) |
                             reinterpret_cast<uintptr_t>(lp.bias) | reinterpret_cast<uintptr_t>(lp.mid)) & 15u) == 0;
    if (dma_stage) stage_epilogue_operands_dma<kLdsBytes>(a, lp, g0, n_wgi, lds, tid);
    else
#else
    constexpr bool dma_stage = false;
#endif
    stage_epilogue_operands<kLdsBytes>(a, lp, g0, n_wgi, lds, tid);
    f32x16 acc[4][RN];
    GGCN_TRACE(4);
    unsigned long long stamp_c = 0, stamp_w = 0;
    if constexpr (STAMP) {
        stamp_c = __builtin_readcyclecounter();
        stamp_w = __builtin_amdgcn_s_memrealtime();
    }
    if constexpr (SCH == 0)
        bx3::mainloop<XT, AVEC, KFULL, !FULLT>(arow, avalid, wpack, K, a.k_steps, wm, nt0, n_tiles_total, lds, acc);
    else {
        float amax;
        constexpr bool BUF = AVEC && KFULL;
        mx8::BufX<float> bx;
        if constexpr (BUF) {
            int rel[NP];
#pragma unroll
            for (int i = 0; i < NP; ++i) {
                const int row = stage_row<float>(i);
                rel[i] = avalid[i] ? (row >> 5) * T + (row & 31) : -1;
            }
            bx = mx8::make_bufx<float>(a.X, a.ldx, (int64_t)gt0 * T, (int64_t)B * T, rel, tid);
        }
        mx8::mainloop<float, AVEC, KFULL, !FULLT, false, BUF>(arow, avalid, wpack, K, a.k_steps / 2, wm, nt0, n_tiles_total, lds, acc, 0, 4,
                                                             &amax, &bx);
        if (dma_stage) dma_range_verdict<kLdsBytes>(amax, wpack, (int64_t)n_tiles_total * (a.k_steps / 2) * mx8::STAGE_PACK_BYTES, lds, tid & 63);
        else fused_range_verdict<kLdsBytes>(amax, wpack, (int64_t)n_tiles_total * (a.k_steps / 2) * mx8::STAGE_PACK_BYTES, lds, true);
    }
    GGCN_TRACE(5);
    if constexpr (STAMP) {
        asm volatile("" :: "v"(acc[3][RN - 1][15]));
        const unsigned long long c1 = __builtin_readcyclecounter(), w1 = __builtin_amdgcn_s_memrealtime();
        if (tid == 0 && a.stamps) {
            a.stamps[2 * (size_t)blockIdx.x] = c1 - stamp_c;
            a.stamps[2 * (size_t)blockIdx.x + 1] = w1 - stamp_w;
        }
    }
    if constexpr (((GGCN_LAB_OFF) & 128) != 0) {
        float s = 0.0f;
#pragma unroll
        for (int i = 0; i < 4; ++i)
#pragma unroll
            for (int j = 0; j < RN; ++j)
#pragma unroll
                for (int r = 0; r < 16; ++r) s += acc[i][j][r];
        if (s == 123.456f && lp.pool_a) lp.pool_a[tid] = s;
        return;
    }
    if (a.drop.thr != 0) {
        if (lp.out) epilogue<SCH, FULLT, VST, false, true, kLdsBytes, true>(a, lp, acc, g0, nt0, n_tiles_total, lds, tid);
        else epilogue<SCH, FULLT, VST, false, false, kLdsBytes, true>(a, lp, acc, g0, nt0, n_tiles_total, lds, tid);
    } else if (lp.mid) {
        if (lp.out) epilogue<SCH, FULLT, VST, true, true>(a, lp, acc, g0, nt0, n_tiles_total, lds, tid);
        else epilogue<SCH, FULLT, VST, true, false>(a, lp, acc, g0, nt0, n_tiles_total, lds, tid);
    } else {
        if (lp.out) epilogue<SCH, FULLT, VST, false, true>(a, lp, acc, g0, nt0, n_tiles_total, lds, tid);
        else epilogue<SCH, FULLT, VST, false, false>(a, lp, acc, g0, nt0, n_tiles_total, lds, tid);
    }
    GGCN_TRACE(6);
}


constexpr int kRedThreads = 1024;
__global__ __launch_bounds__(kRedThreads) void overlap_reduce_kernel(const float *__restrict__ part, int n_part, int B,
                                                                     float *__restrict__ dst)
{
    __shared__ float red[kRedThreads / 64];
    const int tid = threadIdx.x;
    float s0 = 0.0f, s1 = 0.0f, s2 = 0.0f, s3 = 0.0f;
    const int n4 = (reinterpret_cast<uintptr_t>(part) & 15u) == 0 ? n_part / 4 : 0;
    const float4 *p4 = reinterpret_cast<const float4 *>(part);
    int i = tid;
    for (; i + 3 * kRedThreads < n4; i += 4 * kRedThreads) {
        const float4 a = p4[i], b = p4[i + kRedThreads], c = p4[i + 2 * kRedThreads], d = p4[i + 3 * kRedThreads];
        s0 += (a.x + a.y) + (a.z + a.w);
        s1 += (b.x + b.y) + (b.z + b.w);
        s2 += (c.x + c.y) + (c.z + c.w);
        s3 += (d.x + d.y) + (d.z + d.w);
    }
    for (; i < n4; i += kRedThreads) {
        const float4 a = p4[i];
        s0 += (a.x + a.y) + (a.z + a.w);
    }
    for (int j = 4 * n4 + tid; j < n_part; j += kRedThreads) s1 += part[j];
    float sdot = (s0 + s1) + (s2 + s3);
#pragma unroll
    for (int d = 32; d >= 1; d >>= 1) sdot += __shfl_xor(sdot, d);
    if ((tid & 63) == 0) red[tid >> 6] = sdot;
    __syncthreads();
    if (tid == 0) {
        float t = 0.0f;
#pragma unroll
        for (int w = 0; w < kRedThreads / 64; ++w) t += red[w];
        *dst = t / (float)B;
    }
}

__global__ __launch_bounds__(256) void rowmask_kernel(const int32_t *__restrict__ rowptr,
                                                      const int32_t *__restrict__ colidx, int64_t n, int T,
                                                      uint32_t *__restrict__ rowmask)
{
    const int64_t i = (int64_t)blockIdx.x * 256 + threadIdx.x;
    if (i >= n) return;
    const int64_t base = i / T * T;
    const int W = (T + 31) >> 5;
    uint32_t m[GGCN_MASK_MAX_T / 32] = {};
    for (int e = rowptr[i]; e < rowptr[i + 1]; ++e) {
        const uint32_t j = (uint32_t)(colidx[e] - base);
#pragma unroll
        for (int w = 0; w < GGCN_MASK_MAX_T / 32; ++w)
            if ((j >> 5) == (uint32_t)w) m[w] |= 1u << (j & 31u);
    }
#pragma unroll
    for (int w = 0; w < GGCN_MASK_MAX_T / 32; ++w)
        if (w < W) rowmask[i * W + w] = m[w];
}

int launch_fused(const char *who, FusedArgs &a, int precision, hipStream_t st)
{
    if (precision != GGCN_PREC_BF16X3 && precision != GGCN_PREC_F16MX8 && precision != GGCN_PREC_F16MX6)
        return fail(GGCN_EUNSUPPORTED, "%s: precision %d (use bf16x3 or f16mx8)", who, precision);
#ifndef GGCN_WITH_F16MX6
    if (precision == GGCN_PREC_F16MX6)
        return fail(GGCN_EUNSUPPORTED, "%s: f16mx6 is an experiment this library was built without (make F16MX6=1); use f16mx8", who);
#endif
    if (!a.X && !a.Xb) return fail(GGCN_EINVAL, "%s: null input pointer", who);
    if (a.T > 32 ? !a.rowmask : !a.graph_ops)
        return fail(GGCN_EINVAL, "%s: graphs of %d nodes need %s", who, a.T,
                    a.T > 32 ? "the row masks" : "the per-graph operand blocks of ggcn_graph_operands");
    if (a.T <= 32 && !aligned16(a.graph_ops)) return fail(GGCN_EINVAL, "%s: graph_ops must be 16-byte aligned", who);
    if (a.T > 128 && a.graph_ops && !aligned16(a.graph_ops)) return fail(GGCN_EINVAL, "%s: the edge-list blocks must be 16-byte aligned", who);
    if (a.B <= 0 || a.T <= 0 || a.K <= 0 || a.F <= 0)
        return fail(GGCN_EINVAL, "%s: B=%d T=%d K=%d F=%d must be positive", who, a.B, a.T, a.K, a.F);
    if (a.T > GGCN_MASK_MAX_T)
        return fail(GGCN_EUNSUPPORTED, "%s: T=%d > %d; use ggcn_linear + ggcn_aggregate", who, a.T, GGCN_MASK_MAX_T);
    if (a.T > 32 && a.n_parts != 1)
        return fail(GGCN_EUNSUPPORTED, "%s: the two-layer form takes graphs of <= 32 nodes (T=%d): one ggcn_layer_fused per layer", who, a.T);
    if (a.ldx < a.K) return fail(GGCN_EINVAL, "%s: ldx < K", who);
    bool vst = true, any_out = false;
    for (int p = 0; p < a.n_parts; ++p) {
        const LayerPart &lp = a.part[p];
        if (!lp.wpack) return fail(GGCN_EINVAL, "%s: null weight image", who);
        if (!aligned16(lp.wpack)) return fail(GGCN_EINVAL, "%s: wpack must be 16-byte aligned", who);
        if (!lp.out && !lp.pool_a && !lp.pool_b) return fail(GGCN_EINVAL, "%s: no output requested", who);
        if (lp.out) {
            if (lp.ldo < a.F) return fail(GGCN_EINVAL, "%s: leading dimension of the output too small", who);
            if ((int64_t)a.T * lp.ldo >= (int64_t)INT32_MAX)
                return fail(GGCN_EUNSUPPORTED, "%s: T*ldo does not fit 32-bit offsets", who);
            any_out = true;
            vst = vst && (a.F % 4 == 0) && (lp.ldo % 4 == 0) && aligned16(lp.out) && (int64_t)a.T * lp.ldo * 4 < ((int64_t)1 << 31);
        }
    }
    vst = vst && any_out;
    if (a.Xb) {
        if (precision != GGCN_PREC_BF16X3)
            return fail(GGCN_EUNSUPPORTED, "%s: bf16 features take the bf16x3 weight image (precision %d)", who, precision);
        bool folded = a.n_parts != 1;
        for (int p = 0; p < a.n_parts; ++p) folded = folded || a.part[p].mid;
        if (a.stamps || a.part[0].pre || a.part[a.n_parts - 1].pre)
            return fail(GGCN_EUNSUPPORTED, "%s: bf16 features take no bias_pre and no stamps", who);
        if (folded && (a.T > 32 || !a.graph_ops2 || !aligned16(a.graph_ops2)))
            return fail(GGCN_EUNSUPPORTED, "%s: the two-layer form takes graphs of <= 32 nodes and their ggcn_graph_operands2 blocks (T=%d)", who, a.T);
        if (folded && a.drop.thr != 0)
            return fail(GGCN_EUNSUPPORTED, "%s: gate dropout is built into the one-launch LAYER, not the two-layer block", who);
        if ((int64_t)a.B * a.T * a.F >= ((int64_t)1 << 32) && a.drop.thr != 0)
            return fail(GGCN_EUNSUPPORTED, "%s: gate dropout indexes elements with 32 bits (B*T*F = %lld)", who, (long long)a.B * a.T * a.F);
        const bool avecb = (a.K % 8 == 0) && (a.ldx % 8 == 0) && aligned16(a.Xb);
        const bool kfullb = (a.K % BK == 0);
        a.k_steps = round_up(a.K, BK) / KSTEP;
        a.n_wg = (a.F + BN - 1) / BN;
        if (a.T > 32) {
            const int sb = a.T <= 64 ? 2 : a.T <= 128 ? 4 : 8;
            const int gpt = sb == 2 ? 2 : 1;
            const int64_t gt = ((int64_t)a.B + gpt - 1) / gpt;
            const int64_t gridw = grid_for(gt, a.n_wg);
            if (gridw > (int64_t)INT32_MAX) return fail(GGCN_EUNSUPPORTED, "%s: batch too large", who);
            a.g_tiles = (int)gt;
            const bool vstw = vst || !any_out;
            if (sb == 8) return launch_fused_wide8(who, a, precision, avecb && kfullb, vstw, gridw, st);
            return launch_fused_wide(who, a, precision, sb, avecb && kfullb, vstw, gridw, st);
        }
        const int64_t g_tiles = ((int64_t)a.B + 4 * WM - 1) / (4 * WM);
        const int64_t grid = a.n_parts == 1 ? grid_for(g_tiles, a.n_wg) : (g_tiles + 3) / 4 * a.n_wg * 8;
        if (grid > (int64_t)INT32_MAX) return fail(GGCN_EUNSUPPORTED, "%s: batch too large", who);
        a.g_tiles = (int)g_tiles;
        const bool fullt = (a.T == 32) && (a.B % (4 * WM) == 0);
        const bool vstb = vst || (folded && !any_out);
#define GGCN_LAUNCH_B(AV, KF, FT, VS) \
    hipLaunchKernelGGL((layer_fused_kernel<0, AV, KF, FT, VS, false, __bf16>), dim3((unsigned)grid), dim3(kThreads), 0, st, a)
        if (avecb && kfullb && fullt && vstb) GGCN_LAUNCH_B(true, true, true, true);
        else if (avecb && kfullb && vstb) GGCN_LAUNCH_B(true, true, false, true);
        else if (avecb && kfullb) GGCN_LAUNCH_B(true, true, false, false);
        else if (avecb && vstb) GGCN_LAUNCH_B(true, false, false, true);
        else if (avecb) GGCN_LAUNCH_B(true, false, false, false);
        else GGCN_LAUNCH_B(false, false, false, false);
#undef GGCN_LAUNCH_B
        return check_launch(who);
    }
    const bool avec = (a.K % 4 == 0) && (a.ldx % 4 == 0) && aligned16(a.X) && (int64_t)a.ldx * 4 * 257 < ((int64_t)1 << 31);
    const bool kfull = (a.K % BK == 0);
    a.k_steps = round_up(a.K, BK) / KSTEP;
    a.n_wg = (a.F + BN - 1) / BN;
    if (a.drop.thr != 0 && (a.n_parts != 1 || precision == GGCN_PREC_F16MX6))
        return fail(GGCN_EUNSUPPORTED, "%s: gate dropout is built into the one-launch LAYER (bf16x3 / f16mx8), not the two-layer block", who);
    if ((int64_t)a.B * a.T * a.F >= ((int64_t)1 << 32) && a.drop.thr != 0)
        return fail(GGCN_EUNSUPPORTED, "%s: gate dropout indexes elements with 32 bits (B*T*F = %lld)", who, (long long)a.B * a.T * a.F);
    if (a.T > 32 && precision == GGCN_PREC_F16MX6)
        return fail(GGCN_EUNSUPPORTED, "%s: f16mx6 takes graphs of <= 32 nodes (T=%d); use f16mx8", who, a.T);
    if (a.T > 32) {
        const int sb = a.T <= 64 ? 2 : a.T <= 128 ? 4 : 8;
        const int gpt = sb == 2 ? 2 : 1;
        const int64_t gt = ((int64_t)a.B + gpt - 1) / gpt;
        const int64_t gridw = grid_for(gt, a.n_wg);
        if (gridw > (int64_t)INT32_MAX) return fail(GGCN_EUNSUPPORTED, "%s: batch too large", who);
        a.g_tiles = (int)gt;
        const bool fast = avec && kfull;
        if (sb == 8 && !GGCN_LAB_WIDE_SB8) return launch_fused_wide8(who, a, precision, fast, vst, gridw, st);
        return launch_fused_wide(who, a, precision, sb, fast, vst, gridw, st);
    }
    const int64_t g_tiles = ((int64_t)a.B + 4 * WM - 1) / (4 * WM);
    const int64_t grid = a.n_parts == 1 ? grid_for(g_tiles, a.n_wg) : (g_tiles + 3) / 4 * a.n_wg * 8;
    if (grid > (int64_t)INT32_MAX) return fail(GGCN_EUNSUPPORTED, "%s: batch too large", who);
    a.g_tiles = (int)g_tiles;
    const bool fullt = (a.T == 32) && (a.B % (4 * WM) == 0);
    if (precision == GGCN_PREC_F16MX6) {
        if (!(avec && kfull) || (int64_t)128 * a.ldx * 4 >= ((int64_t)1 << 31))
            return fail(GGCN_EUNSUPPORTED, "%s: f16mx6 needs K %% 32 == 0 and 16-byte aligned rows of X (K=%d ldx=%lld); use f16mx8",
                        who, a.K, (long long)a.ldx);
        return launch_fused6(who, a, fullt, vst, grid, st);
    }
#define GGCN_LAUNCH(SC, AV, KF, FT, VS) \
    hipLaunchKernelGGL((layer_fused_kernel<SC, AV, KF, FT, VS>), dim3((unsigned)grid), dim3(kThreads), 0, st, a)
#define GGCN_PICK(SC)                                                                 \
    do {                                                                              \
        if (avec && kfull && fullt && vst) GGCN_LAUNCH(SC, true, true, true, true);   \
        else if (avec && kfull && fullt) GGCN_LAUNCH(SC, true, true, true, false);    \
        else if (avec && kfull && vst) GGCN_LAUNCH(SC, true, true, false, true);      \
        else if (avec && kfull) GGCN_LAUNCH(SC, true, true, false, false);            \
        else if (avec) GGCN_LAUNCH(SC, true, false, false, false);                    \
        else GGCN_LAUNCH(SC, false, false, false, false);                             \
    } while (0)
    if (a.stamps) {
        if (!(precision == GGCN_PREC_F16MX8 && avec && kfull && fullt && vst))
            return fail(GGCN_EUNSUPPORTED, "%s: the stamped form takes f16mx8, T = 32, B %% 4 == 0, K %% 32 == 0, 16-byte rows", who);
        hipLaunchKernelGGL((layer_fused_kernel<1, true, true, true, true, true>), dim3((unsigned)grid), dim3(kThreads), 0, st, a);
    } else if (precision == GGCN_PREC_F16MX8) GGCN_PICK(1);
    else GGCN_PICK(0);
#undef GGCN_PICK
#undef GGCN_LAUNCH
    return check_launch(who);
}

}

GGCN_TRACE_READER

int csr_rowmask(const int32_t *rowptr, const int32_t *colidx, int B, int T, uint32_t *rowmask, hipStream_t st)
{
    if (!rowptr || !colidx || !rowmask) return fail(GGCN_EINVAL, "ggcn_csr_rowmask: null pointer");
    if (B <= 0 || T <= 0) return fail(GGCN_EINVAL, "ggcn_csr_rowmask: B=%d T=%d must be positive", B, T);
    if (T > GGCN_MASK_MAX_T)
        return fail(GGCN_EUNSUPPORTED, "ggcn_csr_rowmask: T=%d > %d (row masks cover graphs of at most %d nodes)", T, GGCN_MASK_MAX_T, GGCN_MASK_MAX_T);
    const int64_t n = (int64_t)B * T;
    hipLaunchKernelGGL(rowmask_kernel, dim3((unsigned)((n + 255) / 256)), dim3(256), 0, st, rowptr, colidx, n, T,
                       rowmask);
    return check_launch("ggcn_csr_rowmask");
}

__global__ __launch_bounds__(256) void dropout_mask_kernel(int64_t n, int F, DropSpec d, int sel, float *__restrict__ out)
{
    const int64_t i = (int64_t)blockIdx.x * 256 + threadIdx.x;
    if (i < n) out[i] = drop_keep(drop_hash((uint32_t)i, d.seed_lo, d.seed_hi), sel, d.thr, d.scale);
}

int dropout_mask(int64_t rows, int F, float p, uint64_t seed, int sel, float *out, hipStream_t st)
{
    if (!out) return fail(GGCN_EINVAL, "ggcn_dropout_mask: null pointer");
    if (rows <= 0 || F <= 0 || sel < 0 || sel > 2 || !(p >= 0.0f && p < 1.0f))
        return fail(GGCN_EINVAL, "ggcn_dropout_mask: rows=%lld F=%d sel=%d p=%g", (long long)rows, F, sel, (double)p);
    const int64_t n = rows * F;
    if (n >= ((int64_t)1 << 32)) return fail(GGCN_EUNSUPPORTED, "ggcn_dropout_mask: rows*F must fit 32 bits");
    const DropSpec d = make_drop_spec(p, seed, 0, 0, 0);
    hipLaunchKernelGGL(dropout_mask_kernel, dim3((unsigned)((n + 255) / 256)), dim3(256), 0, st, n, F, d, sel, out);
    return check_launch("ggcn_dropout_mask");
}

int graph_operands(const uint32_t *rowmask, int B, int T, void *ops, hipStream_t st)
{
    if (!rowmask || !ops) return fail(GGCN_EINVAL, "ggcn_graph_operands: null pointer");
    if (B <= 0 || T <= 0) return fail(GGCN_EINVAL, "ggcn_graph_operands: B=%d T=%d must be positive", B, T);
    if (T > 32) return fail(GGCN_EUNSUPPORTED, "ggcn_graph_operands: T=%d > 32 (larger graphs are applied from their row masks)", T);
    if (!aligned16(ops)) return fail(GGCN_EINVAL, "ggcn_graph_operands: ops must be 16-byte aligned");
    hipLaunchKernelGGL(graph_operands_kernel, dim3((unsigned)((B + 3) / 4)), dim3(256), 0, st, rowmask, B, T,
                       static_cast<char *>(ops));
    return check_launch("ggcn_graph_operands");
}

int graph_operands2(const uint32_t *rowmask, int B, int T, int plane, void *ops2, hipStream_t st)
{
    if (!rowmask || !ops2) return fail(GGCN_EINVAL, "ggcn_graph_operands2: null pointer");
    if (B <= 0 || T <= 0) return fail(GGCN_EINVAL, "ggcn_graph_operands2: B=%d T=%d must be positive", B, T);
    if (T > 32) return fail(GGCN_EUNSUPPORTED, "ggcn_graph_operands2: T=%d > 32 (the two-layer block takes graphs of <= 32 nodes)", T);
    if (plane != 0 && plane != 1) return fail(GGCN_EINVAL, "ggcn_graph_operands2: plane %d (0 = bf16 pairs, 1 = fp16 pairs)", plane);
    if (!aligned16(ops2)) return fail(GGCN_EINVAL, "ggcn_graph_operands2: ops2 must be 16-byte aligned");
    const dim3 grid((unsigned)((B + 3) / 4));
    if (plane == 1) hipLaunchKernelGGL(graph_operands2_kernel<1>, grid, dim3(256), 0, st, rowmask, B, T, static_cast<char *>(ops2));
    else hipLaunchKernelGGL(graph_operands2_kernel<0>, grid, dim3(256), 0, st, rowmask, B, T, static_cast<char *>(ops2));
    return check_launch("ggcn_graph_operands2");
}

int graph_operands_weighted(const int32_t *rowptr, const int32_t *colidx, const float *vals, int B, int T, int plane, void *ops,
                            int *flag, hipStream_t st)
{
    const char *who = "ggcn_graph_operands_weighted";
    if (!rowptr || !colidx || !ops) return fail(GGCN_EINVAL, "%s: null pointer", who);
    if (B <= 0 || T <= 0) return fail(GGCN_EINVAL, "%s: B=%d T=%d must be positive", who, B, T);
    if (T > 32) return fail(GGCN_EUNSUPPORTED, "%s: T=%d > 32 (weighted graphs of more nodes: ggcn_linear + ggcn_aggregate)", who, T);
    if (plane != 0 && plane != 1) return fail(GGCN_EINVAL, "%s: plane %d (0 = bf16 pairs, 1 = fp16 pairs)", who, plane);
    if (!aligned16(ops)) return fail(GGCN_EINVAL, "%s: the blocks must be 16-byte aligned", who);
    if ((int64_t)B * T >= (int64_t)INT32_MAX) return fail(GGCN_EUNSUPPORTED, "%s: B*T does not fit int32 node ids", who);
    const dim3 grid((unsigned)((B + 3) / 4));
    if (plane == 1) hipLaunchKernelGGL(graph_operands_w_kernel<1>, grid, dim3(256), 0, st, rowptr, colidx, vals, B, T, static_cast<char *>(ops), flag);
    else hipLaunchKernelGGL(graph_operands_w_kernel<0>, grid, dim3(256), 0, st, rowptr, colidx, vals, B, T, static_cast<char *>(ops), flag);
    return check_launch(who);
}

int layer_fused_weighted(const float *X, int64_t ldx, const void *wpack, const void *graph_opsw, const float *bias, const float *zero_mid,
                         int B, int T, int K, int F, const float *store_gate, const float *pool_gate_a, const float *pool_gate_b,
                         float *out, int64_t ldo, float *pool_a, float *pool_b, float *overlap_partial, const float *overlap_in,
                         float *overlap_out, int precision, hipStream_t st)
{
    const char *who = "ggcn_layer_fused_weighted";
    if ((overlap_in == nullptr) != (overlap_out == nullptr)) return fail(GGCN_EINVAL, "%s: overlap_in and overlap_out go together", who);
    if (!graph_opsw || !zero_mid) return fail(GGCN_EINVAL, "%s: the weighted operand blocks and the zero row are required", who);
    if (T > 32) return fail(GGCN_EUNSUPPORTED, "%s: T=%d > 32 (use ggcn_linear + ggcn_aggregate)", who, T);
    if (precision == GGCN_PREC_F16MX6) return fail(GGCN_EUNSUPPORTED, "%s: bf16x3 or f16mx8", who);
    if (out && ldo > (int64_t)INT32_MAX) return fail(GGCN_EUNSUPPORTED, "%s: ldo too large", who);
    FusedArgs a = {};
    a.X = X; a.ldx = ldx; a.graph_ops = static_cast<const char *>(graph_opsw); a.graph_ops2 = a.graph_ops;
    a.ov_in = overlap_in; a.ov_out = overlap_out;
    a.B = B; a.T = T; a.K = K; a.F = F; a.n_parts = 1;
    a.part[0] = LayerPart{static_cast<const char *>(wpack), bias, zero_mid, nullptr, store_gate, pool_gate_a, pool_gate_b,
                          out, pool_a, pool_b, overlap_partial, (int)ldo};
    return launch_fused(who, a, precision, st);
}

int layer_fused(const float *X, int64_t ldx, const void *wpack, const uint32_t *rowmask, const void *graph_ops,
                const float *bias, int B, int T, int K, int F, const float *store_gate, const float *pool_gate_a,
                const float *pool_gate_b, float *out, int64_t ldo, float *pool_a, float *pool_b,
                float *overlap_partial, const float *overlap_in, float *overlap_out, int precision, hipStream_t st,
                const DropSpec *drop, const float *bias_pre)
{
    if ((overlap_in == nullptr) != (overlap_out == nullptr))
        return fail(GGCN_EINVAL, "ggcn_layer_fused: overlap_in and overlap_out go together");
    if (out && ldo > (int64_t)INT32_MAX) return fail(GGCN_EUNSUPPORTED, "ggcn_layer_fused: ldo too large");
    FusedArgs a = {};
    a.X = X; a.ldx = ldx; a.rowmask = rowmask; a.graph_ops = static_cast<const char *>(graph_ops);
    a.ov_in = overlap_in; a.ov_out = overlap_out;
    a.B = B; a.T = T; a.K = K; a.F = F; a.n_parts = 1;
    if (drop) a.drop = *drop;
    a.part[0] = LayerPart{static_cast<const char *>(wpack), bias, nullptr, bias_pre, store_gate, pool_gate_a, pool_gate_b,
                          out, pool_a, pool_b, overlap_partial, (int)ldo};
    if (bias_pre && T <= 32)
        return fail(GGCN_EUNSUPPORTED, "ggcn_layer_fused_prebias: graphs of <= 32 nodes fold both layers in ggcn_block_fused (its eval form); bias_pre is for 33..256 nodes");
    if (bias_pre && drop)
        return fail(GGCN_EUNSUPPORTED, "ggcn_layer_fused_prebias: an inference form (no gate dropout)");
    return launch_fused("ggcn_layer_fused", a, precision, st);
}

int layer_fused_bf16(const char *who, const void *X, int64_t ldx, const void *wpack, const uint32_t *rowmask, const void *graph_ops,
                     const float *bias, int B, int T, int K, int F,
                     const float *store_gate, const float *pool_gate_a, const float *pool_gate_b, float *out, int64_t ldo,
                     float *pool_a, float *pool_b, float *overlap_partial, const float *overlap_in, float *overlap_out,
                     hipStream_t st, const DropSpec *drop)
{
    if (!X) return fail(GGCN_EINVAL, "%s: null input pointer", who);
    if ((overlap_in == nullptr) != (overlap_out == nullptr)) return fail(GGCN_EINVAL, "%s: overlap_in and overlap_out go together", who);
    if (out && ldo > (int64_t)INT32_MAX) return fail(GGCN_EUNSUPPORTED, "%s: ldo too large", who);
    FusedArgs a = {};
    a.X = static_cast<const float *>(wpack);
    a.Xb = static_cast<const __bf16 *>(X); a.ldx = ldx; a.rowmask = rowmask; a.graph_ops = static_cast<const char *>(graph_ops);
    a.ov_in = overlap_in; a.ov_out = overlap_out;
    a.B = B; a.T = T; a.K = K; a.F = F; a.n_parts = 1;
    if (drop) a.drop = *drop;
    a.part[0] = LayerPart{static_cast<const char *>(wpack), bias, nullptr, nullptr, store_gate, pool_gate_a, pool_gate_b,
                          out, pool_a, pool_b, overlap_partial, (int)ldo};
    return launch_fused(who, a, GGCN_PREC_BF16X3, st);
}

int block_fused(const float *X, int64_t ldx, const void *wpack1, const void *wpack12, const void *graph_ops,
                const void *graph_ops2, const float *bias1, const float *bias_mid, const float *bias2, int B, int T, int K, int F,
                const float *gate1, const float *gate2, float *gcn1, int64_t ld1, float *x_out, int64_t ld2,
                float *x1, float *y1, float *pool_out, float *overlap_partial, int precision, hipStream_t st,
                unsigned long long *stamps)
{
    if (!gate2) return fail(GGCN_EINVAL, "ggcn_block_fused: gate2 is required");
    const bool layer1 = x1 || y1 || gcn1 || overlap_partial;
    if (layer1 && (!x1 || !y1 || !gate1))
        return fail(GGCN_EINVAL, "ggcn_block_fused: layer 1's outputs go together (gate1, x1 and y1; all NULL with gcn1 and overlap_partial = the eval form)");
    if (!x_out && !pool_out) return fail(GGCN_EINVAL, "ggcn_block_fused: neither x nor its pool requested");
    if ((gcn1 && ld1 > (int64_t)INT32_MAX) || (x_out && ld2 > (int64_t)INT32_MAX))
        return fail(GGCN_EUNSUPPORTED, "ggcn_block_fused: leading dimension too large");
    FusedArgs a = {};
    if (!graph_ops2 || !aligned16(graph_ops2))
        return fail(GGCN_EINVAL, "ggcn_block_fused: graph_ops2 (ggcn_graph_operands2 blocks, 16-byte aligned) is required");
    if (layer1 && !gcn1 && !stamps && precision == GGCN_PREC_F16MX8 && X && wpack1 && wpack12 && bias_mid &&
        block8_takes(X, ldx, wpack1, wpack12, B, T, K, F, gate1, gate2, bias1, bias_mid, bias2, graph_ops, graph_ops2, x_out, ld2)) {
        const char *form = getenv("GGCN_BLOCK_FORM");
        if (!(form && form[0] == '4'))
            return lab_block_fused8(X, ldx, wpack1, wpack12, graph_ops, graph_ops2, bias1, bias_mid, bias2, B, T, K, F, gate1, gate2, x_out,
                                    ld2, x1, y1, pool_out, overlap_partial, st, nullptr, kBlock8RowMajor | kBlock8Product);
    }
    a.X = X; a.ldx = ldx; a.graph_ops = static_cast<const char *>(graph_ops); a.graph_ops2 = static_cast<const char *>(graph_ops2);
    a.B = B; a.T = T; a.K = K; a.F = F; a.n_parts = layer1 ? 2 : 1;
    a.stamps = stamps;
    if (!bias_mid) return fail(GGCN_EINVAL, "ggcn_block_fused: bias_mid (W2^T.b1, zeros when gc1 has no bias) is required");
    const LayerPart second = LayerPart{static_cast<const char *>(wpack12), bias2, bias_mid, nullptr, gate2, gate2, nullptr,
                                       x_out, pool_out, nullptr, nullptr, (int)ld2};
    if (layer1) {
        a.part[0] = LayerPart{static_cast<const char *>(wpack1), bias1, nullptr, nullptr, nullptr, gate1, gate2,
                              gcn1, x1, y1, overlap_partial, (int)ld1};
        a.part[1] = second;
    } else {
        if (stamps) return fail(GGCN_EUNSUPPORTED, "ggcn_debug_block_fused_stamped: the eval form is not stamped");
        if (!a.graph_ops) a.graph_ops = a.graph_ops2;
        a.part[0] = second;
    }
    return launch_fused("ggcn_block_fused", a, precision, st);
}

int block_fused_bf16(const void *X, int64_t ldx, const void *wpack1, const void *wpack12, const void *graph_ops,
                     const void *graph_ops2, const float *bias1, const float *bias_mid, const float *bias2, int B, int T, int K, int F,
                     const float *gate1, const float *gate2, float *gcn1, int64_t ld1, float *x_out, int64_t ld2,
                     float *x1, float *y1, float *pool_out, float *overlap_partial, hipStream_t st)
{
    const char *who = "ggcn_block_fused_bf16";
    if (!X) return fail(GGCN_EINVAL, "%s: null input pointer", who);
    if (T > 32)
        return fail(GGCN_EUNSUPPORTED, "%s: T=%d > 32 (one ggcn_layer_fused_bf16_wide per layer up to %d nodes)", who, T, GGCN_MASK_MAX_T);
    if (!gate2) return fail(GGCN_EINVAL, "%s: gate2 is required", who);
    const bool layer1 = x1 || y1 || gcn1 || overlap_partial;
    if (layer1 && (!x1 || !y1 || !gate1))
        return fail(GGCN_EINVAL, "%s: layer 1's outputs go together (gate1, x1 and y1; all NULL with gcn1 and overlap_partial = the eval form)", who);
    if (!x_out && !pool_out) return fail(GGCN_EINVAL, "%s: neither x nor its pool requested", who);
    if ((gcn1 && ld1 > (int64_t)INT32_MAX) || (x_out && ld2 > (int64_t)INT32_MAX))
        return fail(GGCN_EUNSUPPORTED, "%s: leading dimension too large", who);
    if (!wpack12 || (layer1 && !wpack1)) return fail(GGCN_EINVAL, "%s: null weight image", who);
    if (!graph_ops2) return fail(GGCN_EINVAL, "%s: graph_ops2 (the ggcn_graph_operands2 blocks of plane 0) is required", who);
    if (!aligned16(graph_ops2)) return fail(GGCN_EINVAL, "%s: graph_ops2 must be 16-byte aligned", who);
    if (layer1 && !graph_ops) return fail(GGCN_EINVAL, "%s: layer 1 needs the per-graph operand blocks of ggcn_graph_operands", who);
    if (!bias_mid) return fail(GGCN_EINVAL, "%s: bias_mid (W2^T.b1, zeros when gc1 has no bias) is required", who);
    FusedArgs a = {};
    a.X = static_cast<const float *>(wpack12);
    a.Xb = static_cast<const __bf16 *>(X); a.ldx = ldx;
    a.graph_ops = static_cast<const char *>(graph_ops); a.graph_ops2 = static_cast<const char *>(graph_ops2);
    a.B = B; a.T = T; a.K = K; a.F = F; a.n_parts = layer1 ? 2 : 1;
    const LayerPart second = LayerPart{static_cast<const char *>(wpack12), bias2, bias_mid, nullptr, gate2, gate2, nullptr,
                                       x_out, pool_out, nullptr, nullptr, (int)ld2};
    if (layer1) {
        a.part[0] = LayerPart{static_cast<const char *>(wpack1), bias1, nullptr, nullptr, nullptr, gate1, gate2,
                              gcn1, x1, y1, overlap_partial, (int)ld1};
        a.part[1] = second;
    } else {
        if (!a.graph_ops) a.graph_ops = a.graph_ops2;
        a.part[0] = second;
    }
    return launch_fused(who, a, GGCN_PREC_BF16X3, st);
}

int overlap_reduce(const float *partials, int B, int F, float *xy, hipStream_t st)
{
    if (!partials || !xy) return fail(GGCN_EINVAL, "ggcn_overlap_reduce: null pointer");
    if (B <= 0 || F <= 0) return fail(GGCN_EINVAL, "ggcn_overlap_reduce: B=%d F=%d must be positive", B, F);
    hipLaunchKernelGGL(overlap_reduce_kernel, dim3(1), dim3(kRedThreads), 0, st, partials, B * ((F + 63) / 64), B, xy);
    return check_launch("ggcn_overlap_reduce");
}

GGCN_RANGE_FLAG_TU(range_flag_fused)

}
```

### ed-gated-gcn_amd/csrc/heads.hip

```cpp
#include "common.h"

namespace ggcn {
namespace {

__device__ __forceinline__ float sigmoidf(float v) { return 1.0f / (1.0f + expf(-v)); }

__global__ __launch_bounds__(256) void transpose_kernel(const float *__restrict__ W, int rows, int cols, int64_t ldw,
                                                        float *__restrict__ Wt)
{
    __shared__ float tile[32][33];
    const int c0 = blockIdx.x * 32, r0 = blockIdx.y * 32;
    const int tx = threadIdx.x & 31, ty = threadIdx.x >> 5;
    for (int i = ty; i < 32; i += 8)
        if (r0 + i < rows && c0 + tx < cols) tile[i][tx] = W[(int64_t)(r0 + i) * ldw + c0 + tx];
    __syncthreads();
    for (int i = ty; i < 32; i += 8)
        if (c0 + i < cols && r0 + tx < rows) Wt[(int64_t)(c0 + i) * rows + r0 + tx] = tile[tx][i];
}

struct GateParams {
    const float *w1t, *b1, *w2t, *b2;
    float *out;
};

constexpr int kGateRows = 8;

__global__ __launch_bounds__(256) void gate_mlp_kernel(const float *__restrict__ aspect, int64_t lda, int B, int H,
                                                       GateParams ga, GateParams gb)
{
    extern __shared__ float lds_f[];
    float *s = lds_f, *h = lds_f + kGateRows * H;
    const GateParams gp = blockIdx.y == 0 ? ga : gb;
    const int r0 = blockIdx.x * kGateRows;
    const int nr = B - r0 < kGateRows ? B - r0 : kGateRows;
    for (int i = threadIdx.x; i < kGateRows * H; i += 256) {
        const int r = i / H, k = i - r * H;
        s[i] = r < nr ? sigmoidf(aspect[(int64_t)(r0 + r) * lda + k]) : 0.0f;
    }
    __syncthreads();
    for (int layer = 0; layer < 2; ++layer) {
        const float *wt = layer == 0 ? gp.w1t : gp.w2t, *bias = layer == 0 ? gp.b1 : gp.b2;
        const float *in = layer == 0 ? s : h;
        for (int j = threadIdx.x; j < H; j += 256) {
            float acc[kGateRows];
#pragma unroll
            for (int r = 0; r < kGateRows; ++r) acc[r] = 0.0f;
            for (int k = 0; k < H; ++k) {
                const float w = wt[(int64_t)k * H + j];
#pragma unroll
                for (int r = 0; r < kGateRows; ++r) acc[r] = fmaf(in[r * H + k], w, acc[r]);
            }
            const float bj = bias ? bias[j] : 0.0f;
            if (layer == 0) {
#pragma unroll
                for (int r = 0; r < kGateRows; ++r) h[r * H + j] = sigmoidf(acc[r] + bj);
            } else {
#pragma unroll
                for (int r = 0; r < kGateRows; ++r)
                    if (r < nr) gp.out[(int64_t)(r0 + r) * H + j] = sigmoidf(acc[r] + bj);
            }
        }
        __syncthreads();
    }
}

__global__ __launch_bounds__(256) void scores_head_kernel(const float *__restrict__ X, int64_t ldx,
                                                          const float *__restrict__ aspect, int64_t lda,
                                                          const float *__restrict__ logits, int64_t ldl,
                                                          const float *__restrict__ fcw, int64_t ldw,
                                                          const float *__restrict__ fcb, const float *__restrict__ dist,
                                                          int64_t ldd, int T, int H, int C, float *__restrict__ scores,
                                                          int64_t lds_, float *__restrict__ kl_part)
{
    extern __shared__ float lds_f[];
    float *v = lds_f, *u = v + H, *sc = u + C, *red = sc + T;
    const int b = blockIdx.x, tid = threadIdx.x, lane = tid & 63, wave = tid >> 6;
    const float *lg = logits + (int64_t)b * ldl, *a = aspect + (int64_t)b * lda;
    for (int hh = tid; hh < H; hh += 256) {
        float acc = 0.0f;
        for (int c = 0; c < C; ++c) acc = fmaf(lg[c], fcw[(int64_t)c * ldw + hh], acc);
        v[hh] = acc;
    }
    for (int c = wave; c < C; c += 4) {
        float acc = 0.0f;
        for (int hh = lane; hh < H; hh += 64) acc = fmaf(fcw[(int64_t)c * ldw + H + hh], a[hh], acc);
#pragma unroll
        for (int d = 32; d >= 1; d >>= 1) acc += __shfl_xor(acc, d);
        if (lane == 0) u[c] = acc + (fcb ? fcb[c] : 0.0f);
    }
    __syncthreads();
    float c0 = 0.0f;
    for (int c = 0; c < C; ++c) c0 = fmaf(lg[c], u[c], c0);
    for (int t = wave; t < T; t += 4) {
        const float *xr = X + ((int64_t)b * T + t) * ldx;
        float acc = 0.0f;
        for (int hh = lane; hh < H; hh += 64) acc = fmaf(xr[hh], v[hh], acc);
#pragma unroll
        for (int d = 32; d >= 1; d >>= 1) acc += __shfl_xor(acc, d);
        if (lane == 0) {
            sc[t] = acc + c0;
            scores[(int64_t)b * lds_ + t] = acc + c0;
        }
    }
    __syncthreads();
    if (!kl_part) return;
    if (wave == 0) {
        const float *dr = dist + (int64_t)b * ldd;
        float ms = -INFINITY, md = -INFINITY;
        for (int t = lane; t < T; t += 64) { ms = fmaxf(ms, sc[t]); md = fmaxf(md, dr[t]); }
#pragma unroll
        for (int d = 32; d >= 1; d >>= 1) { ms = fmaxf(ms, __shfl_xor(ms, d)); md = fmaxf(md, __shfl_xor(md, d)); }
        float zs = 0.0f, zd = 0.0f, cross = 0.0f;
        for (int t = lane; t < T; t += 64) {
            const float es = expf(sc[t] - ms), ed = expf(dr[t] - md);
            zs += es; zd += ed; cross = fmaf(es, ed, cross);
        }
#pragma unroll
        for (int d = 32; d >= 1; d >>= 1) { zs += __shfl_xor(zs, d); zd += __shfl_xor(zd, d); cross += __shfl_xor(cross, d); }
        if (lane == 0) kl_part[b] = cross / (zs * zd);
    }
    (void)red;
}


__device__ __forceinline__ void head_signal(unsigned *__restrict__ signal, int tid)
{
    if (!signal) return;
    __syncthreads();
    if (tid == 0) {
        __threadfence_system();
        if (atomicAdd(signal, 1u) == gridDim.x - 1) {
            signal[0] = 0u;
            __threadfence_system();
            atomicAdd_system(signal + 1, 1u);
        }
    }
}

constexpr int kHeadRows = 8, kHeadThreads = 1024, kHeadWaves = kHeadThreads / 64;
static_assert(kHeadWaves == 2 * kHeadRows, "two wavefronts stage a pooled row");
__global__ __launch_bounds__(kHeadThreads) void dense_head_kernel(const float *__restrict__ pooled, int64_t ldp, const float *__restrict__ Wt,
                                                                  int64_t ldw, const float *__restrict__ bias, int B, int H, int C,
                                                                  float *__restrict__ logits, int64_t ldl, const float *__restrict__ part,
                                                                  int n_part, float *__restrict__ xy, int head_blocks, unsigned *__restrict__ signal)
{
    extern __shared__ __attribute__((aligned(16))) float head_lds[];
    const int tid = threadIdx.x, lane = tid & 63;
    const int wave = __builtin_amdgcn_readfirstlane(tid >> 6);
    if ((int)blockIdx.x >= head_blocks) {
        float sdot = 0.0f;
        for (int idx = tid; idx < n_part; idx += kHeadThreads) sdot += part[idx];
#pragma unroll
        for (int d = 32; d >= 1; d >>= 1) sdot += __shfl_xor(sdot, d);
        if (lane == 0) head_lds[wave] = sdot;
        __syncthreads();
        if (tid == 0) {
            float t = 0.0f;
#pragma unroll
            for (int w = 0; w < kHeadWaves; ++w) t += head_lds[w];
            *xy = t / (float)B;
        }
        head_signal(signal, tid);
        return;
    }
    const int b0 = blockIdx.x * kHeadRows;
    float *rows = head_lds, *red = head_lds + kHeadRows * H;
    {
        const int r = wave >> 1, hb = (H + 1) >> 1, kb = (wave & 1) * hb, ke = kb + hb < H ? kb + hb : H;
        const bool live = b0 + r < B;
        const float *src = pooled + (int64_t)(live ? b0 + r : 0) * ldp;
        if ((hb & 3) == 0 && (ldp & 3) == 0 && (reinterpret_cast<uintptr_t>(pooled) & 15u) == 0) {
            for (int k = kb + 4 * lane; k < ke; k += 256) {
                const float4 v = *reinterpret_cast<const float4 *>(src + k);
                *reinterpret_cast<float4 *>(rows + r * H + k) = live ? v : make_float4(0.0f, 0.0f, 0.0f, 0.0f);
            }
        } else {
            for (int k = kb + lane; k < ke; k += 64) rows[r * H + k] = live ? src[k] : 0.0f;
        }
    }
    __syncthreads();
    const int kq = (H + kHeadWaves - 1) / kHeadWaves, k0 = wave * kq, k1 = k0 + kq < H ? k0 + kq : H;
    const int c = lane < C ? lane : 0;
    float acc[kHeadRows] = {};
    if ((H & 3) == 0 && (kq & 3) == 0) {
#pragma unroll 4
        for (int k = k0; k < k1; k += 4) {
            float w[4];
#pragma unroll
            for (int q = 0; q < 4; ++q) w[q] = Wt[(int64_t)(k + q) * ldw + c];
#pragma unroll
            for (int r = 0; r < kHeadRows; ++r) {
                const float4 xv = *reinterpret_cast<const float4 *>(rows + r * H + k);
                acc[r] = fmaf(xv.x, w[0], acc[r]); acc[r] = fmaf(xv.y, w[1], acc[r]);
                acc[r] = fmaf(xv.z, w[2], acc[r]); acc[r] = fmaf(xv.w, w[3], acc[r]);
            }
        }
    } else {
#pragma unroll 8
        for (int k = k0; k < k1; ++k) {
            const float w = Wt[(int64_t)k * ldw + c];
#pragma unroll
            for (int r = 0; r < kHeadRows; ++r) acc[r] = fmaf(rows[r * H + k], w, acc[r]);
        }
    }
#pragma unroll
    for (int r = 0; r < kHeadRows; ++r) red[(wave * kHeadRows + r) * 64 + lane] = acc[r];
    __syncthreads();
    if (wave < kHeadRows && lane < C && b0 + wave < B) {
        float t = 0.0f;
#pragma unroll
        for (int w = 0; w < kHeadWaves; ++w) t += red[(w * kHeadRows + wave) * 64 + lane];
        logits[(int64_t)(b0 + wave) * ldl + lane] = t + (bias ? bias[lane] : 0.0f);
    }
    head_signal(signal, tid);
}

}

int transpose_f32(const float *W, int rows, int cols, int64_t ldw, float *Wt, hipStream_t st)
{
    if (!W || !Wt) return fail(GGCN_EINVAL, "ggcn_transpose: null pointer");
    if (rows <= 0 || cols <= 0 || ldw < cols) return fail(GGCN_EINVAL, "ggcn_transpose: rows=%d cols=%d ldw=%lld", rows, cols, (long long)ldw);
    hipLaunchKernelGGL(transpose_kernel, dim3((unsigned)((cols + 31) / 32), (unsigned)((rows + 31) / 32)), dim3(256), 0, st,
                       W, rows, cols, ldw, Wt);
    return check_launch("ggcn_transpose");
}

int gate_mlp(const float *aspect, int64_t lda, int B, int H, const float *w1t_a, const float *b1_a, const float *w2t_a,
             const float *b2_a, float *gate_a, const float *w1t_b, const float *b1_b, const float *w2t_b,
             const float *b2_b, float *gate_b, hipStream_t st)
{
    if (!aspect || !w1t_a || !w2t_a || !gate_a) return fail(GGCN_EINVAL, "ggcn_gate_mlp: null pointer");
    if ((gate_b != nullptr) != (w1t_b != nullptr && w2t_b != nullptr))
        return fail(GGCN_EINVAL, "ggcn_gate_mlp: the second gate needs both of its weights and its output (or none)");
    if (B <= 0 || H <= 0 || lda < H) return fail(GGCN_EINVAL, "ggcn_gate_mlp: B=%d H=%d lda=%lld", B, H, (long long)lda);
    const size_t lds = (size_t)2 * kGateRows * H * sizeof(float);
    if (lds > 64 * 1024) return fail(GGCN_EUNSUPPORTED, "ggcn_gate_mlp: H=%d needs more than 64 KiB of LDS", H);
    GateParams ga{w1t_a, b1_a, w2t_a, b2_a, gate_a}, gb{w1t_b, b1_b, w2t_b, b2_b, gate_b};
    hipLaunchKernelGGL(gate_mlp_kernel, dim3((unsigned)((B + kGateRows - 1) / kGateRows), gate_b ? 2u : 1u), dim3(256), lds, st,
                       aspect, lda, B, H, ga, gb);
    return check_launch("ggcn_gate_mlp");
}

int scores_head(const float *X, int64_t ldx, const float *aspect, int64_t lda, const float *logits, int64_t ldl,
                const float *fcw, int64_t ldw, const float *fcb, const float *dist, int64_t ldd, int B, int T, int H,
                int C, float *scores, int64_t lds_, float *kl_part, hipStream_t st)
{
    if (!X || !aspect || !logits || !fcw || !scores) return fail(GGCN_EINVAL, "ggcn_scores_head: null pointer");
    if ((kl_part != nullptr) != (dist != nullptr)) return fail(GGCN_EINVAL, "ggcn_scores_head: dist and kl_part go together");
    if (B <= 0 || T <= 0 || H <= 0 || C <= 0) return fail(GGCN_EINVAL, "ggcn_scores_head: B=%d T=%d H=%d C=%d", B, T, H, C);
    if (ldx < H || lda < H || ldl < C || ldw < 2 * H || lds_ < T || (dist && ldd < T))
        return fail(GGCN_EINVAL, "ggcn_scores_head: leading dimension too small");
    const size_t lds = (size_t)(H + C + T + 8) * sizeof(float);
    if (lds > 64 * 1024) return fail(GGCN_EUNSUPPORTED, "ggcn_scores_head: H + C + T = %d needs more than 64 KiB of LDS", H + C + T);
    hipLaunchKernelGGL(scores_head_kernel, dim3((unsigned)B), dim3(256), lds, st, X, ldx, aspect, lda, logits, ldl, fcw, ldw,
                       fcb, dist, ldd, T, H, C, scores, lds_, kl_part);
    return check_launch("ggcn_scores_head");
}

int dense_head(const float *pooled, int64_t ldp, const float *Wt, int64_t ldw, const float *bias, int B, int H, int C,
               float *logits, int64_t ldl, const float *partials, int F_block, float *xy, hipStream_t st, unsigned *signal)
{
    if (!pooled || !Wt || !logits) return fail(GGCN_EINVAL, "ggcn_dense_head: null pointer");
    if ((partials != nullptr) != (xy != nullptr)) return fail(GGCN_EINVAL, "ggcn_dense_head: overlap_partials and xy go together");
    if (B <= 0 || H <= 0 || C <= 0 || (partials && F_block <= 0)) return fail(GGCN_EINVAL, "ggcn_dense_head: B=%d H=%d C=%d F_block=%d", B, H, C, F_block);
    if (C > 64) return fail(GGCN_EUNSUPPORTED, "ggcn_dense_head: C=%d classes (one lane per class: at most 64)", C);
    if (ldp < H || ldw < C || ldl < C) return fail(GGCN_EINVAL, "ggcn_dense_head: leading dimension too small");
    const int head_blocks = (B + kHeadRows - 1) / kHeadRows;
    const size_t lds = ((size_t)kHeadRows * H + (size_t)kHeadWaves * kHeadRows * 64) * sizeof(float);
    if (lds > 64 * 1024) return fail(GGCN_EUNSUPPORTED, "ggcn_dense_head: H=%d needs more than 64 KiB of LDS", H);
    hipLaunchKernelGGL(dense_head_kernel, dim3((unsigned)(head_blocks + (partials ? 1 : 0))), dim3(kHeadThreads), lds, st, pooled, ldp, Wt, ldw, bias,
                       B, H, C, logits, ldl, partials, partials ? B * ((F_block + 63) / 64) : 0, xy, head_blocks, signal);
    return check_launch("ggcn_dense_head");
}

}
```

### ed-gated-gcn_amd/gated_block.py

```python
import torch

from . import _capi, range_guard
from .csr import BatchedCSR, tensor_version
from .gcn import BF16_PRECISIONS


def gate_overlap(x1, y1):
    lib = _capi.load_library()
    B, F = x1.shape
    dev = x1.device
    with torch.cuda.device(dev):
        xy = torch.empty((), dtype=torch.float32, device=dev)
        ws = torch.empty(lib.ggcn_overlap_workspace_bytes(B), dtype=torch.uint8, device=dev)
        _capi.check(lib.ggcn_gate_overlap(_capi.ptr(x1), _capi.ptr(y1), B, F, _capi.ptr(xy), _capi.ptr(ws),
                                          _capi.stream_of(dev)), "ggcn_gate_overlap")
    return xy


def _block_operands(gc1, gc2, lib, st, precision=None):
    w1, w2, b1 = gc1.weight, gc2.weight, gc1.bias
    precision = precision or gc1.precision
    prec = _capi.PREC[precision]
    key = (w1.data_ptr(), tensor_version(w1), w2.data_ptr(), tensor_version(w2), None if b1 is None else (b1.data_ptr(), tensor_version(b1)),
           w1.device, prec)
    store = getattr(gc2, "_block_ops", None)
    if not isinstance(store, dict):
        store = gc2._block_ops = {}
    cached = store.get(prec)
    if cached is None or cached[0] != key:
        K, F1, F2 = gc1.in_features, gc1.out_features, gc2.out_features
        dev = w1.device
        w1c, w2c = w1.detach().contiguous(), w2.detach().contiguous()
        w12 = torch.empty(K, F2, dtype=torch.float32, device=dev)
        _capi.check(lib.ggcn_linear(_capi.ptr(w1c), F1, _capi.ptr(w2c), F2, None, _capi.ptr(w12), F2, K, F1, F2,
                                    _capi.PREC["fp32"], st), "ggcn_linear(W1.W2)")
        mid = torch.zeros(F2, dtype=torch.float32, device=dev)
        if b1 is not None:
            b1c = b1.detach().contiguous()
            _capi.check(lib.ggcn_linear(_capi.ptr(b1c), F1, _capi.ptr(w2c), F2, None, _capi.ptr(mid), F2, 1, F1, F2,
                                        _capi.PREC["fp32"], st), "ggcn_linear(b1.W2)")
        pack12 = torch.empty(lib.ggcn_weight_pack_bytes(K, F2, prec), dtype=torch.uint8, device=dev)
        _capi.check(lib.ggcn_weight_pack(_capi.ptr(w12), F2, K, F2, prec, 0, _capi.ptr(pack12), st), "ggcn_weight_pack(W12)")
        cached = (key, pack12, mid)
        store[prec] = cached
    return gc1._packed_weight(lib, st, precision=precision), cached[1], cached[2]


def takes_folded_eval_path(x, csr, gc1, gc2):
    return (32 < csr.T <= 256 and gc1.takes_fused_path(x, csr) and gc2.takes_fused_path(x, csr) and gc1.precision == gc2.precision
            and gc1.precision in ("f16mx8", "bf16x3") and gc1.out_features == gc2.in_features
            and gc1.in_features == gc1.out_features == gc2.out_features)


def _folded_eval(x, csr, gate2, gc1, gc2, want_x):
    gc1._check(x)
    bf16 = x.dtype == torch.bfloat16
    if not bf16:
        range_guard.before(x.device)
    lib = _capi.load_library()
    B, T, K = x.shape
    F = gc2.out_features
    dev = x.device
    x2d = x.reshape(B * T, K)
    if x2d.stride(1) != 1:
        x2d = x2d.contiguous()
    if not (isinstance(gate2, torch.Tensor) and gate2.is_cuda and gate2.dtype == torch.float32 and tuple(gate2.shape) == (B, F)
            and gate2.is_contiguous()):
        raise RuntimeError("gate2 must be a contiguous float32 [B,F]=[%d,%d] GPU tensor" % (B, F))
    with torch.cuda.device(dev):
        st = _capi.stream_of(dev)
        prec = "bf16x3" if bf16 else gc1.precision
        _, pack12, mid = _block_operands(gc1, gc2, lib, st, precision=prec)
        z = torch.empty(B * T, K, dtype=torch.float32, device=dev)
        if bf16:
            _capi.check(lib.ggcn_aggregate_bf16(_capi.ptr(x2d), x2d.stride(0), _capi.ptr(csr.rowptr), _capi.ptr(csr.colidx),
                                                _capi.ptr(csr.vals), B, T, K, _capi.ptr(z), K, st), "ggcn_aggregate_bf16(D.A.X)")
        else:
            _capi.check(lib.ggcn_aggregate(_capi.ptr(x2d), x2d.stride(0), _capi.ptr(csr.rowptr), _capi.ptr(csr.colidx), _capi.ptr(csr.vals),
                                           None, B, T, K, None, None, None, _capi.ptr(z), K, None, None, st), "ggcn_aggregate(D.A.X)")
        xo = torch.empty(B * T, F, dtype=torch.float32, device=dev) if want_x else None
        out = torch.empty(B, F, dtype=torch.float32, device=dev)
        b2 = None if gc2.bias is None else gc2.bias.detach()
        _capi.check(lib.ggcn_layer_fused_prebias(_capi.ptr(z), K, _capi.ptr(pack12), _capi.ptr(csr.rowmask), _capi.ptr(b2), _capi.ptr(mid),
                                                 B, T, K, F, _capi.ptr(gate2), _capi.ptr(gate2), None, _capi.ptr(xo), F,
                                                 _capi.ptr(out), None, _capi.PREC[prec], st), "ggcn_layer_fused_prebias")
    if prec == "f16mx8":
        range_guard.after(x.device)
    return (None if xo is None else xo.view(B, T, F)), out


def _bf16_block_on(x, gc1):
    return bool(getattr(gc1, "bf16_block", False)) and isinstance(x, torch.Tensor) and x.is_cuda and x.dtype == torch.bfloat16


def takes_bf16_block_path(x, csr, gc1, gc2):
    return (_bf16_block_on(x, gc1) and csr.T <= 32 and gc1.takes_bf16_fused_path(x, csr) and bool(gc2.fused)
            and gc1.precision in BF16_PRECISIONS and gc2.precision in BF16_PRECISIONS
            and gc1.out_features == gc2.in_features and gc1.out_features == gc2.out_features)


def takes_bf16_folded_eval_path(x, csr, gc1, gc2):
    return (_bf16_block_on(x, gc1) and 32 < csr.T <= 256 and bool(csr.is_binary) and csr.rowmask is not None and csr.rowmask.is_cuda
            and gc1.precision in BF16_PRECISIONS and gc2.takes_fused_path(_layer2_input(x, gc1), csr)
            and gc1.out_features == gc2.in_features and gc1.in_features == gc1.out_features == gc2.out_features)


def takes_block_path(x, csr, gc1, gc2):
    return (csr.T <= 32 and gc1.takes_fused_path(x, csr) and gc2.takes_fused_path(x, csr) and gc1.precision == gc2.precision
            and gc1.out_features == gc2.in_features and gc1.out_features == gc2.out_features)


def _layer2_input(x, gc1):
    if x.dtype == torch.float32:
        return x
    return torch.zeros(1, dtype=torch.float32, device=x.device).expand(x.shape[0], x.shape[1], gc1.out_features)


def _layer1_takes_fused(x, csr, gc1):
    return gc1.takes_fused_path(x, csr) or gc1.takes_bf16_fused_path(x, csr) or gc1.takes_bf16_wide_path(x, csr)


BLOCK_OUTPUTS = ("x1", "y1", "xy", "x", "out")


def gated_gcn_block(x, adj, gate1, gate2, gc1, gc2, want_gcn1=False, one_launch=True, want=None, dense_head=None):
    if dense_head is not None:
        from .heads import dense_head as _dense_head
        if torch.is_grad_enabled() and (gc1._needs_grad(x, gate1, gate2, adj=adj) or gc2._needs_grad(x, gate2, adj=adj)):
            raise RuntimeError("dense_head= is an inference feature; under autograd apply the classifier's own dense layer")
        r = _gated_gcn_block(x, adj, gate1, gate2, gc1, gc2, want_gcn1, one_launch, want, _defer_xy=True)
        part = r.pop("_xy_partials", None)
        sig = dense_head[2] if len(dense_head) > 2 else None
        if r["out"] is None:
            raise RuntimeError("dense_head= needs `out` among want=")
        if r["out"].shape[0] == 0:
            r["logits"] = r["out"].new_zeros((0, dense_head[0].shape[1]))
            return r
        if part is not None:
            r["logits"], r["xy"] = _dense_head(r["out"], dense_head[0], dense_head[1], partials=part, f_block=gc2.out_features, signal=sig)
        else:
            r["logits"] = _dense_head(r["out"], dense_head[0], dense_head[1], signal=sig)
        return r
    return _gated_gcn_block(x, adj, gate1, gate2, gc1, gc2, want_gcn1, one_launch, want)


def _bf16_block(x, csr, gate1, gate2, gc1, gc2, want, want_gcn1, pick, defer_xy):
    gc1._check(x)
    w_l1 = any(k in want for k in ("x1", "y1", "xy"))
    lib = _capi.load_library()
    B, T, K = x.shape
    F = gc2.out_features
    dev = x.device
    x2d = x.reshape(B * T, K)
    if x2d.stride(1) != 1:
        x2d = x2d.contiguous()
    layer1 = w_l1 or want_gcn1
    for name, g in (("gate1", gate1), ("gate2", gate2)):
        if g is None and name == "gate1" and not layer1:
            continue
        if not (isinstance(g, torch.Tensor) and g.is_cuda and g.dtype == torch.float32
                and tuple(g.shape) == (B, F) and g.is_contiguous()):
            raise RuntimeError("%s must be a contiguous float32 [B,F]=[%d,%d] GPU tensor" % (name, B, F))
    with torch.cuda.device(dev):
        st = _capi.stream_of(dev)
        pack1, pack12, mid = _block_operands(gc1, gc2, lib, st, precision="bf16x3")
        gcn1 = torch.empty(B * T, F, dtype=torch.float32, device=dev) if want_gcn1 else None
        xo = torch.empty(B * T, F, dtype=torch.float32, device=dev) if "x" in want else None
        x1 = torch.empty(B, F, dtype=torch.float32, device=dev) if layer1 else None
        y1 = torch.empty(B, F, dtype=torch.float32, device=dev) if layer1 else None
        out = torch.empty(B, F, dtype=torch.float32, device=dev)
        part = torch.empty(B, (F + 63) // 64, dtype=torch.float32, device=dev) if "xy" in want else None
        xy = torch.empty((), dtype=torch.float32, device=dev) if "xy" in want else None
        b1 = None if gc1.bias is None else gc1.bias.detach()
        b2 = None if gc2.bias is None else gc2.bias.detach()
        _capi.check(lib.ggcn_block_fused_bf16(_capi.ptr(x2d), x2d.stride(0), _capi.ptr(pack1 if layer1 else None), _capi.ptr(pack12),
                                              _capi.ptr(csr.graph_ops), _capi.ptr(csr.graph_ops2(0)),
                                              _capi.ptr(b1), _capi.ptr(mid), _capi.ptr(b2),
                                              B, T, K, F, _capi.ptr(gate1 if layer1 else None), _capi.ptr(gate2), _capi.ptr(gcn1), F,
                                              _capi.ptr(xo), F, _capi.ptr(x1), _capi.ptr(y1), _capi.ptr(out),
                                              _capi.ptr(part), st), "ggcn_block_fused_bf16")
        if part is not None and not defer_xy:
            _capi.check(lib.ggcn_overlap_reduce(_capi.ptr(part), B, F, _capi.ptr(xy), st), "ggcn_overlap_reduce")
    r = pick({"gcn1": None if gcn1 is None else gcn1.view(B, T, F), "x1": x1, "y1": y1, "xy": xy,
              "x": None if xo is None else xo.view(B, T, F), "out": out})
    if defer_xy and part is not None:
        r["_xy_partials"] = part
    return r


def _gated_gcn_block(x, adj, gate1, gate2, gc1, gc2, want_gcn1=False, one_launch=True, want=None, _defer_xy=False):
    want = BLOCK_OUTPUTS if want is None else tuple(want)
    bad = [k for k in want if k not in BLOCK_OUTPUTS]
    if bad:
        raise ValueError("want: unknown output(s) %s (choose from %s; gcn1 has its own flag want_gcn1)" % (bad, list(BLOCK_OUTPUTS)))
    w_l1 = any(k in want for k in ("x1", "y1", "xy"))
    w_x = "x" in want
    if x.shape[0] == 0:
        gc1._check(x)
        B, T, F = 0, x.shape[1], gc2.out_features
        z2 = x.new_zeros((0, F), dtype=torch.float32)
        dt = torch.float32 if _bf16_block_on(x, gc1) else x.dtype
        return {"gcn1": x.new_zeros((0, T, gc1.out_features), dtype=dt), "x1": x.new_zeros((0, gc1.out_features), dtype=dt),
                "y1": x.new_zeros((0, gc1.out_features), dtype=dt), "xy": x.new_full((), float("nan"), dtype=dt),
                "x": x.new_zeros((0, T, F), dtype=dt), "out": z2}
    csr = adj if isinstance(adj, BatchedCSR) else gc1._as_csr(adj, x)
    training = torch.is_grad_enabled() and (gc1._needs_grad(x, gate1, gate2, adj=adj) or gc2._needs_grad(x, gate2, adj=adj))
    if training and set(want) != set(BLOCK_OUTPUTS):
        raise RuntimeError("want= selects outputs of the inference block; under autograd every output is produced")

    def pick(r):
        for k in BLOCK_OUTPUTS:
            if k not in want:
                r[k] = None
        return r
    if not training and one_launch and takes_block_path(x, csr, gc1, gc2):
        gc1._check(x)
        range_guard.before(x.device)
        lib = _capi.load_library()
        B, T, K = x.shape
        F = gc2.out_features
        dev = x.device
        x2d = x.reshape(B * T, K)
        if x2d.stride(1) != 1:
            x2d = x2d.contiguous()
        for name, g in (("gate1", gate1), ("gate2", gate2)):
            if g is None and name == "gate1" and not (w_l1 or want_gcn1):
                continue
            if not (isinstance(g, torch.Tensor) and g.is_cuda and g.dtype == torch.float32
                    and tuple(g.shape) == (B, F) and g.is_contiguous()):
                raise RuntimeError("%s must be a contiguous float32 [B,F]=[%d,%d] GPU tensor" % (name, B, F))
        with torch.cuda.device(dev):
            st = _capi.stream_of(dev)
            kprec = gc1.kernel_precision(x2d, csr)
            pack1, pack12, mid = _block_operands(gc1, gc2, lib, st, precision=kprec)
            layer1 = w_l1 or want_gcn1
            gcn1 = torch.empty(B * T, F, dtype=torch.float32, device=dev) if want_gcn1 else None
            xo = torch.empty(B * T, F, dtype=torch.float32, device=dev) if w_x else None
            x1 = torch.empty(B, F, dtype=torch.float32, device=dev) if layer1 else None
            y1 = torch.empty(B, F, dtype=torch.float32, device=dev) if layer1 else None
            out = torch.empty(B, F, dtype=torch.float32, device=dev)
            part = torch.empty(B, (F + 63) // 64, dtype=torch.float32, device=dev) if "xy" in want else None
            xy = torch.empty((), dtype=torch.float32, device=dev) if "xy" in want else None
            b1 = None if gc1.bias is None else gc1.bias.detach()
            b2 = None if gc2.bias is None else gc2.bias.detach()
            _capi.check(lib.ggcn_block_fused(_capi.ptr(x2d), x2d.stride(0), _capi.ptr(pack1), _capi.ptr(pack12),
                                             _capi.ptr(csr.graph_ops), _capi.ptr(csr.graph_ops2(0 if kprec == "bf16x3" else 1)),
                                             _capi.ptr(b1), _capi.ptr(mid), _capi.ptr(b2),
                                             B, T, K, F, _capi.ptr(gate1 if layer1 else None), _capi.ptr(gate2), _capi.ptr(gcn1), F,
                                             _capi.ptr(xo), F, _capi.ptr(x1), _capi.ptr(y1), _capi.ptr(out),
                                             _capi.ptr(part), _capi.PREC[kprec], st), "ggcn_block_fused")
            if part is not None and not _defer_xy:
                _capi.check(lib.ggcn_overlap_reduce(_capi.ptr(part), B, F, _capi.ptr(xy), st), "ggcn_overlap_reduce")
        if kprec in ("f16mx8", "f16mx6"):
            range_guard.after(x.device)
        r = pick({"gcn1": None if gcn1 is None else gcn1.view(B, T, F), "x1": x1, "y1": y1, "xy": xy,
                  "x": None if xo is None else xo.view(B, T, F), "out": out})
        if _defer_xy and part is not None:
            r["_xy_partials"] = part
        return r
    if not training and one_launch and takes_bf16_block_path(x, csr, gc1, gc2):
        return _bf16_block(x, csr, gate1, gate2, gc1, gc2, want, want_gcn1, pick, _defer_xy)
    if not training and one_launch and not w_l1 and not want_gcn1 and takes_bf16_folded_eval_path(x, csr, gc1, gc2):
        x2, out = _folded_eval(x, csr, gate2, gc1, gc2, w_x)
        return pick({"gcn1": None, "x1": None, "y1": None, "xy": None, "x": x2, "out": out})
    if (not training and _layer1_takes_fused(x, csr, gc1) and gc2.takes_fused_path(_layer2_input(x, gc1), csr)
            and gc1.out_features == gc2.out_features):
        B, F = x.shape[0], gc1.out_features
        if not w_l1 and not want_gcn1 and one_launch and takes_folded_eval_path(x, csr, gc1, gc2):
            x2, out = _folded_eval(x, csr, gate2, gc1, gc2, w_x)
            return pick({"gcn1": None, "x1": None, "y1": None, "xy": None, "x": x2, "out": out})
        if not w_l1:
            gcn1, _, _ = gc1.forward_gated(x, csr)
            x2, out, _ = gc2.forward_gated(gcn1, csr, store_gate=gate2, pool_gate_a=gate2, want_out=w_x, want_pool_a=True)
            return pick({"gcn1": gcn1 if want_gcn1 else None, "x1": None, "y1": None, "xy": None, "x": x2, "out": out})
        part = torch.empty(B, (F + 63) // 64, dtype=torch.float32, device=x.device)
        xy = torch.empty((), dtype=torch.float32, device=x.device)
        gcn1, x1, y1 = gc1.forward_gated(x, csr, store_gate=None, pool_gate_a=gate1, pool_gate_b=gate2,
                                         want_pool_a=True, want_pool_b=True, overlap_partial=part)
        x2, out, _ = gc2.forward_gated(gcn1, csr, store_gate=gate2, pool_gate_a=gate2, want_pool_a=True,
                                       want_out=w_x, overlap_reduce=(part, xy))
        return pick({"gcn1": gcn1, "x1": x1, "y1": y1, "xy": xy, "x": x2, "out": out})
    if not training and not w_l1:
        gcn1, _, _ = gc1.forward_gated(x, csr)
        x2, out, _ = gc2.forward_gated(gcn1, csr, store_gate=gate2, pool_gate_a=gate2, want_out=w_x, want_pool_a=True)
        return pick({"gcn1": gcn1 if want_gcn1 else None, "x1": None, "y1": None, "xy": None, "x": x2, "out": out})
    graph = adj if gc1._differentiable_adj(adj) is not None else csr
    gcn1, x1, y1 = gc1.forward_gated(x, graph, store_gate=None, pool_gate_a=gate1, pool_gate_b=gate2,
                                     want_pool_a=True, want_pool_b=True)
    if torch.is_grad_enabled() and (x1.requires_grad or y1.requires_grad):
        xy = (x1 * y1).sum(1).mean()
    else:
        xy = gate_overlap(x1, y1) if "xy" in want else None
    x2, out, _ = gc2.forward_gated(gcn1, graph, store_gate=gate2, pool_gate_a=gate2,
                                   want_out=training or w_x, want_pool_a=True)
    return pick({"gcn1": gcn1, "x1": x1, "y1": y1, "xy": xy, "x": x2, "out": out})
```

### include/ggcn.h

```cpp
#ifndef GGCN_H
#define GGCN_H

#include <stddef.h>
#include <stdint.h>

#ifdef __cplusplus
extern "C" {
#endif

#define GGCN_ABI_VERSION 14
#define GGCN_MASK_MAX_T 256

typedef void *ggcn_stream_t;

enum ggcn_status {
    GGCN_OK = 0,
    GGCN_EINVAL = 1,
    GGCN_ELAUNCH = 2,
    GGCN_EUNSUPPORTED = 3
};

enum ggcn_adj_dtype {
    GGCN_ADJ_F32 = 0,
    GGCN_ADJ_U8 = 1,
    GGCN_ADJ_I32 = 2,
    GGCN_ADJ_I64 = 3,
    GGCN_ADJ_F64 = 4,
    GGCN_ADJ_F16 = 5
};

enum ggcn_csr_flags {
    GGCN_FLAG_WEIGHTED = 1
};

enum ggcn_precision {
    GGCN_PREC_BF16X3 = 0,
    GGCN_PREC_FP32 = 1,
    GGCN_PREC_F16MX8 = 2,
    GGCN_PREC_F16 = 3,
    GGCN_PREC_F16MX6 = 4
};

int ggcn_abi_version(void);
int ggcn_has_f16mx6(void);
const char *ggcn_last_error(void);

size_t ggcn_csr_workspace_bytes(int64_t n_rows);
int ggcn_csr_from_dense(const void *adj, int adj_dtype, int B, int T,
                        int64_t stride_b, int64_t stride_r, int64_t stride_c,
                        int32_t *rowptr, int32_t *colidx, float *vals, int64_t capacity,
                        uint32_t *rowmask, int32_t *flags,
                        void *workspace, ggcn_stream_t stream);

int ggcn_rowmask_from_dense(const void *adj, int adj_dtype, int B, int T,
                            int64_t stride_b, int64_t stride_r, int64_t stride_c,
                            uint32_t *rowmask, int32_t *flags, ggcn_stream_t stream);

int ggcn_csr_transpose(const int32_t *rowptr, const int32_t *colidx, const float *vals, int B, int T,
                       int32_t *rowptr_t, int32_t *colidx_t, float *vals_t, void *workspace,
                       ggcn_stream_t stream);

#define GGCN_GRAPH_OPS_BYTES 2176
#define GGCN_GRAPH_OPS2_BYTES 4224
#define GGCN_EDGE_LISTS_BYTES 11264
size_t ggcn_graph_edge_lists_bytes(int B);
int ggcn_graph_edge_lists(const uint32_t *rowmask, int B, int T, void *lists, ggcn_stream_t stream);
size_t ggcn_graph_operands_bytes(int B);
int ggcn_graph_operands(const uint32_t *rowmask, int B, int T, void *graph_ops, ggcn_stream_t stream);
size_t ggcn_graph_operands2_bytes(int B);
int ggcn_graph_operands2(const uint32_t *rowmask, int B, int T, int plane, void *graph_ops2, ggcn_stream_t stream);

int ggcn_csr_rowmask(const int32_t *rowptr, const int32_t *colidx, int B, int T,
                     uint32_t *rowmask, ggcn_stream_t stream);

size_t ggcn_weight_pack_bytes(int K, int F, int precision);
int ggcn_weight_pack(const float *W, int64_t ldw, int K, int F, int precision, int transposed,
                     void *wpack, ggcn_stream_t stream);
int ggcn_linear(const float *X, int64_t ldx, const float *W, int64_t ldw, const void *wpack,
                float *Y, int64_t ldy, int64_t M, int K, int F, int precision,
                ggcn_stream_t stream);

int ggcn_aggregate(const float *Hd, int64_t ldh,
                   const int32_t *rowptr, const int32_t *colidx, const float *vals,
                   const float *bias, int B, int T, int F,
                   const float *store_gate, const float *pool_gate_a, const float *pool_gate_b,
                   float *out, int64_t ldo, float *pool_a, float *pool_b,
                   ggcn_stream_t stream);

int ggcn_gate_pool_backward(const float *out, int64_t ldo,
                            const float *store_gate, const float *gate_a, const float *gate_b,
                            const float *d_out, int64_t ldd, const float *d_pa, const float *d_pb,
                            int B, int T, int F, float *dY, int64_t ldy,
                            float *d_sg, float *d_ga, float *d_gb, float *d_bsum, ggcn_stream_t stream);
int ggcn_gate_pool_backward_drop(const float *out, int64_t ldo, const float *store_gate, const float *gate_a,
                                 const float *gate_b, const float *d_out, int64_t ldd, const float *d_pa,
                                 const float *d_pb, int B, int T, int F, float *dY, int64_t ldy, float *d_sg,
                                 float *d_ga, float *d_gb, float *d_bsum, float p, uint64_t seed, int stream_store,
                                 int stream_a, int stream_b, ggcn_stream_t stream);
int ggcn_gate_pool_backward_agg(const float *out, int64_t ldo, const float *store_gate, const float *gate_a,
                                const float *gate_b, const float *d_out, int64_t ldd, const float *d_pa,
                                const float *d_pb, const uint32_t *rowmask, int B, int T, int F, float *dH, int64_t ldh,
                                float *d_sg, float *d_ga, float *d_gb, float *d_bsum, float p, uint64_t seed,
                                int stream_store, int stream_a, int stream_b, float *dh_amax, ggcn_stream_t stream);
int ggcn_linear_scaled(const float *X, int64_t ldx, const void *wpack, float *Y, int64_t ldy, int64_t M, int K, int F,
                       const float *amax, ggcn_stream_t stream);
int ggcn_rowmask_transpose(const uint32_t *rowmask, int B, int T, uint32_t *rowmask_t, ggcn_stream_t stream);
int ggcn_gate_pool_backward_mma(const float *out, int64_t ldo, const float *store_gate, const float *gate_a,
                                const float *gate_b, const float *d_out, int64_t ldd, const float *d_pa, const float *d_pb,
                                const void *graph_ops, const void *graph_ops_t, int B, int T, int F, float *dH, int64_t ldh,
                                float *d_sg, float *d_ga, float *d_gb, float *d_bsum, float *dh_amax, ggcn_stream_t stream);
size_t ggcn_colsum_workspace_bytes(int F);
int ggcn_colsum(const float *X, int64_t ld, int64_t M, int F, float *out, void *workspace, ggcn_stream_t stream);
size_t ggcn_dweight_workspace_bytes(int64_t n_rows, int K, int F, int precision);
int ggcn_dweight(const float *X, int64_t ldx, const float *dH, int64_t ldg, int64_t n_rows, int K, int F,
                 float *dW, int64_t lddw, int precision, void *workspace, ggcn_stream_t stream);
int ggcn_inv_denominators(const int32_t *rowptr, const float *vals, int64_t n_rows, float *inv,
                          ggcn_stream_t stream);
int ggcn_aggregate_t(const float *G, int64_t ldg,
                     const int32_t *rowptr_t, const int32_t *colidx_t, const float *vals_t,
                     const float *src_scale, int B, int T, int F,
                     float *out, int64_t ldo, ggcn_stream_t stream);
int ggcn_adjacency_grad(const float *dY, int64_t ldy, const float *hidden, int64_t ldh,
                        const float *inv,
                        const int32_t *rowptr, const int32_t *colidx, const float *vals,
                        int B, int T, int F, float *d_adj, ggcn_stream_t stream);

int ggcn_linear_h(const void *X, int64_t ldx, const void *wpack, void *Y, int64_t ldy,
                  int64_t M, int K, int F, int precision, ggcn_stream_t stream);
int ggcn_aggregate_h(const void *Hd, int64_t ldh,
                     const int32_t *rowptr, const int32_t *colidx, const float *vals,
                     const float *bias, int B, int T, int F,
                     const float *store_gate, const float *pool_gate_a, const float *pool_gate_b,
                     void *out, int64_t ldo, float *pool_a, float *pool_b,
                     ggcn_stream_t stream);

#define GGCN_LONG_MAX_T 512
int ggcn_layer_fused_h(const void *X, int64_t ldx, const void *wpack,
                       const int32_t *rowptr, const int32_t *colidx, const float *vals,
                       const float *bias, int B, int T, int K, int F,
                       const float *store_gate, const float *pool_gate_a, const float *pool_gate_b,
                       void *out, int64_t ldo, float *pool_a, float *pool_b,
                       ggcn_stream_t stream);

int ggcn_layer_fused(const float *X, int64_t ldx, const void *wpack,
                     const uint32_t *rowmask, const void *graph_ops,
                     const float *bias, int B, int T, int K, int F,
                     const float *store_gate, const float *pool_gate_a, const float *pool_gate_b,
                     float *out, int64_t ldo, float *pool_a, float *pool_b,
                     float *overlap_partial, const float *overlap_in, float *overlap_out,
                     int precision, ggcn_stream_t stream);

int ggcn_layer_fused_prebias(const float *X, int64_t ldx, const void *wpack, const uint32_t *rowmask,
                             const float *bias, const float *bias_pre, int B, int T, int K, int F,
                             const float *store_gate, const float *pool_gate_a, const float *pool_gate_b,
                             float *out, int64_t ldo, float *pool_a, float *pool_b, int precision, ggcn_stream_t stream);

int ggcn_graph_operands_weighted(const int32_t *rowptr, const int32_t *colidx, const float *vals, int B, int T, int plane,
                                 void *graph_opsw, int32_t *flag, ggcn_stream_t stream);
int ggcn_layer_fused_weighted(const float *X, int64_t ldx, const void *wpack, const void *graph_opsw, const float *bias,
                              const float *zero_mid, int B, int T, int K, int F, const float *store_gate,
                              const float *pool_gate_a, const float *pool_gate_b, float *out, int64_t ldo, float *pool_a,
                              float *pool_b, float *overlap_partial, const float *overlap_in, float *overlap_out, int precision,
                              ggcn_stream_t stream);

int ggcn_block_fused(const float *X, int64_t ldx, const void *wpack1, const void *wpack12,
                     const void *graph_ops, const void *graph_ops2, const float *bias1, const float *bias_mid, const float *bias2,
                     int B, int T, int K, int F, const float *gate1, const float *gate2,
                     float *gcn1, int64_t ld1, float *x_out, int64_t ld2,
                     float *x1, float *y1, float *pool_out, float *overlap_partial,
                     int precision, ggcn_stream_t stream);
int ggcn_layer_fused_drop(const float *X, int64_t ldx, const void *wpack, const uint32_t *rowmask, const void *graph_ops,
                          const float *bias, int B, int T, int K, int F,
                          const float *store_gate, const float *pool_gate_a, const float *pool_gate_b,
                          float *out, int64_t ldo, float *pool_a, float *pool_b, int precision,
                          float p, uint64_t seed, int stream_store, int stream_a, int stream_b, ggcn_stream_t stream);
int ggcn_dropout_mask(int64_t rows, int F, float p, uint64_t seed, int stream_id, float *mask, ggcn_stream_t stream);

int ggcn_overlap_reduce(const float *partials, int B, int F, float *xy, ggcn_stream_t stream);

int ggcn_dense_head(const float *pooled, int64_t ldp, const float *Wt, int64_t ldw, const float *bias, int B, int H, int C,
                    float *logits, int64_t ldl, const float *overlap_partials, int F_block, float *xy, ggcn_stream_t stream);

int ggcn_dense_head_signal(const float *pooled, int64_t ldp, const float *Wt, int64_t ldw, const float *bias, int B, int H, int C,
                           float *logits, int64_t ldl, const float *overlap_partials, int F_block, float *xy, uint32_t *signal,
                           ggcn_stream_t stream);

size_t ggcn_overlap_workspace_bytes(int B);
int ggcn_gate_overlap(const float *x1, const float *y1, int B, int F, float *xy,
                      void *workspace, ggcn_stream_t stream);

int ggcn_transpose(const float *W, int rows, int cols, int64_t ldw, float *Wt, ggcn_stream_t stream);
int ggcn_gate_mlp(const float *aspect, int64_t lda, int B, int H,
                  const float *w1t_a, const float *b1_a, const float *w2t_a, const float *b2_a, float *gate_a,
                  const float *w1t_b, const float *b1_b, const float *w2t_b, const float *b2_b, float *gate_b,
                  ggcn_stream_t stream);

int ggcn_scores_head(const float *X, int64_t ldx, const float *aspect, int64_t lda,
                     const float *logits, int64_t ldl, const float *fc_weight, int64_t ldw, const float *fc_bias,
                     const float *dist, int64_t ldd, int B, int T, int H, int C,
                     float *scores, int64_t ld_scores, float *kl_part, ggcn_stream_t stream);

int ggcn_absmax(const void *X, int is_half, int64_t ld, int64_t M, int K, float *out, ggcn_stream_t stream);

enum ggcn_range_bits { GGCN_RANGE_OVERFLOW = 1, GGCN_RANGE_WINDOW = 2, GGCN_RANGE_HIDDEN = 4 };
int ggcn_range_flag(uint32_t *flag, int clear, ggcn_stream_t stream);

int ggcn_debug_poison_lds(uint32_t pattern, ggcn_stream_t stream);

int ggcn_debug_mfma_calibrate(int n_wg, int stages, uint64_t *stamps, float *sink, ggcn_stream_t stream);
int ggcn_block_fused_form(int B, int T, int K, int F);

int ggcn_lab_block_fused8(const float *X, int64_t ldx, const void *wpack1, const void *wpack12, const void *graph_ops,
                          const void *graph_ops2, const float *bias1, const float *bias_mid, const float *bias2,
                          int B, int T, int K, int F, const float *gate1, const float *gate2, float *x_out, int64_t ld2,
                          float *x1, float *y1, float *pool_out, float *overlap_partial, uint64_t *stamps, ggcn_stream_t stream);
int ggcn_debug_block_fused_stamped(const float *X, int64_t ldx, const void *wpack1, const void *wpack12,
                                   const void *graph_ops, const void *graph_ops2, const float *bias1, const float *bias_mid,
                                   const float *bias2, int B, int T, int K, int F, const float *gate1, const float *gate2,
                                   float *gcn1, int64_t ld1, float *x_out, int64_t ld2, float *x1, float *y1, float *pool_out,
                                   float *overlap_partial, int precision, uint64_t *stamps, ggcn_stream_t stream);

int ggcn_subword_pool(const float *A, int64_t sa_b, int64_t sa_r, int64_t sa_c,
                      const float *X, int64_t x_batch, int64_t ldx,
                      float *Y, int64_t y_batch, int64_t ldy,
                      int B, int R, int C, int D, ggcn_stream_t stream);
int ggcn_subword_pool_bf16(const float *A, int64_t sa_b, int64_t sa_r, int64_t sa_c,
                           const void *X, int64_t x_batch, int64_t ldx,
                           void *Y, int64_t y_batch, int64_t ldy,
                           int B, int R, int C, int D, ggcn_stream_t stream);

int ggcn_linear_bf16(const void *X, int64_t ldx, const void *wpack, float *Y, int64_t ldy,
                     int64_t M, int K, int F, ggcn_stream_t stream);
int ggcn_linear_out_bf16(const float *X, int64_t ldx, const void *wpack, void *Y, int64_t ldy,
                         int64_t M, int K, int F, ggcn_stream_t stream);
int ggcn_layer_fused_bf16(const void *X, int64_t ldx, const void *wpack, const void *graph_ops,
                          const float *bias, int B, int T, int K, int F,
                          const float *store_gate, const float *pool_gate_a, const float *pool_gate_b,
                          float *out, int64_t ldo, float *pool_a, float *pool_b,
                          float *overlap_partial, const float *overlap_in, float *overlap_out,
                          ggcn_stream_t stream);
int ggcn_layer_fused_bf16_drop(const void *X, int64_t ldx, const void *wpack, const void *graph_ops,
                               const float *bias, int B, int T, int K, int F,
                               const float *store_gate, const float *pool_gate_a, const float *pool_gate_b,
                               float *out, int64_t ldo, float *pool_a, float *pool_b,
                               float *overlap_partial, const float *overlap_in, float *overlap_out,
                               float p, uint64_t seed, int stream_store, int stream_a, int stream_b, ggcn_stream_t stream);
int ggcn_layer_fused_bf16_wide(const void *X, int64_t ldx, const void *wpack, const uint32_t *rowmask, const void *edge_lists,
                               const float *bias, int B, int T, int K, int F,
                               const float *store_gate, const float *pool_gate_a, const float *pool_gate_b,
                               float *out, int64_t ldo, float *pool_a, float *pool_b,
                               float *overlap_partial, const float *overlap_in, float *overlap_out,
                               float p, uint64_t seed, int stream_store, int stream_a, int stream_b, ggcn_stream_t stream);
int ggcn_block_fused_bf16(const void *X, int64_t ldx, const void *wpack1, const void *wpack12,
                          const void *graph_ops, const void *graph_ops2,
                          const float *bias1, const float *bias_mid, const float *bias2,
                          int B, int T, int K, int F, const float *gate1, const float *gate2,
                          float *gcn1, int64_t ld1, float *x_out, int64_t ld2,
                          float *x1, float *y1, float *pool_out, float *overlap_partial,
                          ggcn_stream_t stream);
int ggcn_aggregate_bf16(const void *X, int64_t ldx, const int32_t *rowptr, const int32_t *colidx,
                        const float *vals, int B, int T, int K, float *Z, int64_t ldz,
                        ggcn_stream_t stream);
size_t ggcn_dweight_bf16_workspace_bytes(int64_t n_rows, int K, int F);
int ggcn_dweight_bf16(const void *X, int64_t ldx, const float *dH, int64_t ldg, int64_t n_rows, int K, int F,
                      float *dW, int64_t lddw, void *workspace, ggcn_stream_t stream);

#ifdef __cplusplus
}
#endif
#endif
```

Before: 855.3 million.

## Fold overlap reduction and dense head into block-fused launch via last-block tail

Adds an in-launch tail to the fused block kernels. Workgroups count their arrival with atomic counters, and the last one to arrive reduces the overlap partials into xy and computes the dense-head logits. This removes the separate overlap_reduce and dense_head kernel launches and their launch gaps. In exchange it adds a vmcnt wait and barrier at the end of every workgroup, plus a serialized tail on a single block, and it needs persistent counter buffers per stream. The feature is on by default through an environment variable.

Measured after the change: 848.8 million. About the same (-0.8%).

```diff
diff --git a/ed-gated-gcn_amd/_capi.py b/ed-gated-gcn_amd/_capi.py
--- a/ed-gated-gcn_amd/_capi.py
+++ b/ed-gated-gcn_amd/_capi.py
@@ -31,6 +31,8 @@
                                          c_vp, c_i64, c_vp, c_vp, c_i32, c_vp]),
     "ggcn_block_fused": (c_i32, [c_vp, c_i64, c_vp, c_vp, c_vp, c_vp, c_vp, c_vp, c_vp, c_i32, c_i32, c_i32, c_i32,
                                  c_vp, c_vp, c_vp, c_i64, c_vp, c_i64, c_vp, c_vp, c_vp, c_vp, c_i32, c_vp]),
+    "ggcn_block_tail_arm": (c_i32, [c_vp, c_vp, c_i64, c_vp, c_i64, c_vp, c_i32, c_vp, c_i64]),
+    "ggcn_block_tail_words": (c_i64, [c_i32]),
     "ggcn_overlap_reduce": (c_i32, [c_vp, c_i32, c_i32, c_vp, c_vp]),
     "ggcn_transpose": (c_i32, [c_vp, c_i32, c_i32, c_i64, c_vp, c_vp]),
     "ggcn_gate_mlp": (c_i32, [c_vp, c_i64, c_i32, c_i32, c_vp, c_vp, c_vp, c_vp, c_vp, c_vp, c_vp, c_vp, c_vp, c_vp, c_vp]),
diff --git a/ed-gated-gcn_amd/csrc/block_tail.h b/ed-gated-gcn_amd/csrc/block_tail.h
--- /dev/null
+++ b/ed-gated-gcn_amd/csrc/block_tail.h
@@ -0,0 +1,112 @@
+#pragma once
+#include <hip/hip_runtime.h>
+#include <cstdint>
+
+namespace ggcn {
+
+struct BlockTail {
+    unsigned *words;
+    float *xy;
+    const float *head_wt;
+    const float *head_bias;
+    float *logits;
+    int64_t ldw, ldl;
+    int C;
+};
+
+namespace {
+
+constexpr int kTailVirtual = 1024, kTailSlices = kTailVirtual / 64, kTailRows = 4;
+__host__ __device__ constexpr int tail_head_lds_floats(int H) { return kTailRows * H + kTailSlices * kTailRows * 64; }
+
+__device__ __forceinline__ float tail_share_vec4(const float *part, int n_part, int v)
+{
+    float s0 = 0.0f, s1 = 0.0f, s2 = 0.0f, s3 = 0.0f;
+    const int n4 = (reinterpret_cast<uintptr_t>(part) & 15u) == 0 ? n_part / 4 : 0;
+    const float4 *p4 = reinterpret_cast<const float4 *>(part);
+    int i = v;
+    for (; i + 3 * kTailVirtual < n4; i += 4 * kTailVirtual) {
+        const float4 a = p4[i], b = p4[i + kTailVirtual], c = p4[i + 2 * kTailVirtual], d = p4[i + 3 * kTailVirtual];
+        s0 += (a.x + a.y) + (a.z + a.w);
+        s1 += (b.x + b.y) + (b.z + b.w);
+        s2 += (c.x + c.y) + (c.z + c.w);
+        s3 += (d.x + d.y) + (d.z + d.w);
+    }
+    for (; i < n4; i += kTailVirtual) {
+        const float4 a = p4[i];
+        s0 += (a.x + a.y) + (a.z + a.w);
+    }
+    for (int j = 4 * n4 + v; j < n_part; j += kTailVirtual) s1 += part[j];
+    return (s0 + s1) + (s2 + s3);
+}
+
+__device__ __forceinline__ float tail_share_scalar(const float *part, int n_part, int v)
+{
+    float s = 0.0f;
+    for (int idx = v; idx < n_part; idx += kTailVirtual) s += part[idx];
+    return s;
+}
+
+template <int NTHR, bool VEC4>
+__device__ __forceinline__ void tail_sum_partials(const float *part, int n_part, int B, float *dst, float *red, int tid)
+{
+    static_assert(NTHR % 64 == 0 && kTailVirtual % NTHR == 0, "whole virtual wavefronts per real one");
+    constexpr int kWaves = NTHR / 64, kPlay = kTailVirtual / NTHR;
+    const int lane = tid & 63, wave = tid >> 6;
+#pragma unroll
+    for (int p = 0; p < kPlay; ++p) {
+        const int vw = wave + p * kWaves;
+        float sdot = VEC4 ? tail_share_vec4(part, n_part, vw * 64 + lane) : tail_share_scalar(part, n_part, vw * 64 + lane);
+#pragma unroll
+        for (int d = 32; d >= 1; d >>= 1) sdot += __shfl_xor(sdot, d);
+        if (lane == 0) red[vw] = sdot;
+    }
+    __syncthreads();
+    if (tid == 0) {
+        float t = 0.0f;
+#pragma unroll
+        for (int w = 0; w < kTailSlices; ++w) t += red[w];
+        *dst = t / (float)B;
+    }
+}
+
+template <int NTHR>
+__device__ __forceinline__ void tail_head_logits(const float *pooled, int H, int B, int g0, const float *Wt, int64_t ldw, const float *bias,
+                                                 int C, float *logits, int64_t ldl, float *lds_f, int tid)
+{
+    constexpr int kWaves = NTHR / 64;
+    static_assert(kWaves >= kTailRows && kTailSlices % kWaves == 0, "a wavefront per row finishes it");
+    const int lane = tid & 63, wave = __builtin_amdgcn_readfirstlane(tid >> 6);
+    float *rows = lds_f, *red = lds_f + kTailRows * H;
+#pragma unroll
+    for (int r = 0; r < kTailRows; ++r) {
+        const bool live = g0 + r < B;
+        const float *src = pooled + (int64_t)(live ? g0 + r : g0) * H;
+        for (int k = tid; k < H; k += NTHR) rows[r * H + k] = live ? src[k] : 0.0f;
+    }
+    __syncthreads();
+    const int kq = (H + kTailSlices - 1) / kTailSlices;
+    const int c = lane < C ? lane : 0;
+    for (int s = wave; s < kTailSlices; s += kWaves) {
+        const int k0 = s * kq, k1 = k0 + kq < H ? k0 + kq : H;
+        float acc[kTailRows] = {};
+#pragma unroll 8
+        for (int k = k0; k < k1; ++k) {
+            const float w = Wt[(int64_t)k * ldw + c];
+#pragma unroll
+            for (int r = 0; r < kTailRows; ++r) acc[r] = fmaf(rows[r * H + k], w, acc[r]);
+        }
+#pragma unroll
+        for (int r = 0; r < kTailRows; ++r) red[(s * kTailRows + r) * 64 + lane] = acc[r];
+    }
+    __syncthreads();
+    if (wave < kTailRows && lane < C && g0 + wave < B) {
+        float t = 0.0f;
+#pragma unroll
+        for (int w = 0; w < kTailSlices; ++w) t += red[(w * kTailRows + wave) * 64 + lane];
+        logits[(int64_t)(g0 + wave) * ldl + lane] = t + (bias ? bias[lane] : 0.0f);
+    }
+}
+
+}
+}
diff --git a/ed-gated-gcn_amd/csrc/capi.hip b/ed-gated-gcn_amd/csrc/capi.hip
--- a/ed-gated-gcn_amd/csrc/capi.hip
+++ b/ed-gated-gcn_amd/csrc/capi.hip
@@ -133,6 +133,14 @@
     return block_fused(X, ldx, wpack1, wpack12, graph_ops, graph_ops2, bias1, bias_mid, bias2, B, T, K, F, gate1, gate2, gcn1, ld1,
                        x_out, ld2, x1, y1, pool_out, overlap_partial, precision, as_stream(stream));
 }
+
+int ggcn_block_tail_arm(float *xy, uint32_t *words, int64_t n_words, const float *head_wt, int64_t ldw, const float *head_bias,
+                        int C, float *logits, int64_t ldl)
+{
+    return block_tail_arm(xy, words, n_words, head_wt, ldw, head_bias, C, logits, ldl);
+}
+
+int64_t ggcn_block_tail_words(int B) { return block_tail_words(B); }
 
 int ggcn_overlap_reduce(const float *partials, int B, int F, float *xy, ggcn_stream_t stream)
 {
diff --git a/ed-gated-gcn_amd/csrc/common.h b/ed-gated-gcn_amd/csrc/common.h
--- a/ed-gated-gcn_amd/csrc/common.h
+++ b/ed-gated-gcn_amd/csrc/common.h
@@ -9,6 +9,7 @@
 namespace ggcn {
 
 struct DropSpec;
+struct BlockTail;
 constexpr int kWave = 64;
 
 char *error_buffer();
@@ -106,6 +107,9 @@
                 const float *gate1, const float *gate2, float *gcn1, int64_t ld1, float *x_out, int64_t ld2,
                 float *x1, float *y1, float *pool_out, float *overlap_partial, int precision, hipStream_t st,
                 unsigned long long *stamps = nullptr);
+int block_tail_arm(float *xy, unsigned *words, int64_t n_words, const float *head_wt, int64_t ldw, const float *head_bias, int C,
+                   float *logits, int64_t ldl);
+int64_t block_tail_words(int B);
 int mfma_calibrate(int n_wg, int stages, unsigned long long *stamps, float *sink, hipStream_t st);
 int overlap_reduce(const float *partials, int B, int F, float *xy, hipStream_t st);
 
@@ -151,7 +155,7 @@
 int lab_block_fused8(const float *X, int64_t ldx, const void *wpack1, const void *wpack12, const void *graph_ops, const void *graph_ops2,
                      const float *bias1, const float *bias_mid, const float *bias2, int B, int T, int K, int F, const float *gate1,
                      const float *gate2, float *x_out, int64_t ld2, float *x1, float *y1, float *pool_out, float *overlap_partial,
-                     hipStream_t st, unsigned long long *stamps = nullptr, int flags = 0);
+                     hipStream_t st, unsigned long long *stamps = nullptr, int flags = 0, const BlockTail *tail = nullptr);
 constexpr int kBlock8RowMajor = 1, kBlock8NoDma = 2, kBlock8SameSlots = 4, kBlock8Product = 8;
 bool block8_shape(int B, int T, int K, int F);
 bool block8_takes(const float *X, int64_t ldx, const void *wpack1, const void *wpack12, int B, int T, int K, int F, const float *gate1,
diff --git a/ed-gated-gcn_amd/csrc/fused_block8.hip b/ed-gated-gcn_amd/csrc/fused_block8.hip
--- a/ed-gated-gcn_amd/csrc/fused_block8.hip
+++ b/ed-gated-gcn_amd/csrc/fused_block8.hip
@@ -24,7 +24,7 @@
     return fmaxf(fmaxf(mm.x, mm.y), fmaxf(mm.z, mm.w));
 }
 
-template <bool FULLT, bool VST>
+template <bool FULLT, bool VST, bool TAIL = false>
 __global__ __launch_bounds__(kB8Threads, 1) void block_fused8_kernel(const FusedArgs a)
 {
     extern __shared__ __attribute__((aligned(16))) char lds[];
@@ -100,6 +100,8 @@
         unsigned long long *o = a.stamps + ((size_t)blockIdx.x * 2 + group) * 4;
         o[0] = t_start; o[1] = t_loop0; o[2] = t_loop1; o[3] = __builtin_amdgcn_s_memrealtime();
     }
+    if constexpr (TAIL)
+        block_tail<kB8Threads>(block_tail_ctx(a), (a.tail.xy ? 1u : 0u) | (a.tail.head_wt ? 2u : 0u), g_tile, lds, tid8);
 }
 
 }
@@ -138,7 +140,7 @@
 int lab_block_fused8(const float *X, int64_t ldx, const void *wpack1, const void *wpack12, const void *graph_ops, const void *graph_ops2,
                      const float *bias1, const float *bias_mid, const float *bias2, int B, int T, int K, int F, const float *gate1,
                      const float *gate2, float *x_out, int64_t ld2, float *x1, float *y1, float *pool_out, float *overlap_partial,
-                     hipStream_t st, unsigned long long *stamps, int flags)
+                     hipStream_t st, unsigned long long *stamps, int flags, const BlockTail *tail)
 {
     const char *who = (flags & kBlock8Product) ? "ggcn_block_fused" : "ggcn_lab_block_fused8";
     if (!X || !wpack1 || !wpack12 || !graph_ops || !graph_ops2 || !gate1 || !gate2 || !x1 || !y1 || !bias_mid)
@@ -157,6 +159,7 @@
     a.part[0] = LayerPart{static_cast<const char *>(wpack1), bias1, nullptr, nullptr, nullptr, gate1, gate2, nullptr, x1, y1, overlap_partial, 0};
     a.part[1] = LayerPart{static_cast<const char *>(wpack12), bias2, bias_mid, nullptr, gate2, gate2, nullptr, x_out, pool_out, nullptr, nullptr, (int)ld2};
     a.stamps = stamps;
+    if (tail) a.tail = *tail;
     a.k_steps = round_up(K, BK) / KSTEP;
     const bool al = (F % 4 == 0) && aligned16(gate1) && aligned16(gate2) && aligned16(bias1) && aligned16(bias2) && aligned16(bias_mid) &&
                     aligned16(graph_ops) && aligned16(graph_ops2) && !(flags & kBlock8NoDma);
@@ -172,7 +175,7 @@
     if (grid > (int64_t)INT32_MAX) return fail(GGCN_EUNSUPPORTED, "%s: batch too large", who);
 #define GGCN_L8(FT, VS)                                                                                                           \
     do {                                                                                                                          \
-        auto kern = block_fused8_kernel<FT, VS>;                                                                                  \
+        auto kern = a.tail.words ? block_fused8_kernel<FT, VS, true> : block_fused8_kernel<FT, VS>;                               \
         if (hipFuncSetAttribute(reinterpret_cast<const void *>(kern), hipFuncAttributeMaxDynamicSharedMemorySize, kB8Lds) != hipSuccess) \
             return fail(GGCN_ELAUNCH, "%s: cannot reserve %d bytes of LDS", who, kB8Lds);                                         \
         hipLaunchKernelGGL(kern, dim3((unsigned)grid), dim3(kB8Threads), kB8Lds, st, a);                                          \
diff --git a/ed-gated-gcn_amd/csrc/fused_common.h b/ed-gated-gcn_amd/csrc/fused_common.h
--- a/ed-gated-gcn_amd/csrc/fused_common.h
+++ b/ed-gated-gcn_amd/csrc/fused_common.h
@@ -2,6 +2,7 @@
 #include "f16mx8_core.h"
 #include "dropout_hash.h"
 #include "lab_hooks.h"
+#include "block_tail.h"
 
 namespace ggcn {
 
@@ -33,6 +34,7 @@
     DropSpec drop;
     unsigned long long *stamps;
     const __bf16 *Xb;
+    BlockTail tail;
 };
 
 
@@ -470,14 +472,15 @@
                 pb = gb * (gb >= 0.0f ? vmax : vmin);
             }
             if (h == 0 && col_ok[j]) {
-                if (pool_a) __builtin_amdgcn_raw_buffer_store_b32(__float_as_uint(pa), out_rsrc(pool_a + (int64_t)g * F), 4 * gn, 0, 0);
+                if (pool_a) __builtin_amdgcn_raw_buffer_store_b32(__float_as_uint(pa), out_rsrc(pool_a + (int64_t)g * F), 4 * gn, 0, MID ? 16 : 0);
                 if (pool_b) __builtin_amdgcn_raw_buffer_store_b32(__float_as_uint(pb), out_rsrc(pool_b + (int64_t)g * F), 4 * gn, 0, 0);
                 dot = fmaf(pa, pb, dot);
             }
         }
         if (ov_partial && nt0 < n_tiles_total) {
             const float tot = wave_sum_to_lane0(dot);
-            if (lane == 0) ov_partial[(int64_t)g * ((F + 63) / 64) + (nt0 >> 1)] = tot;
+            if (lane == 0)
+                __builtin_amdgcn_raw_buffer_store_b32(__float_as_uint(tot), out_rsrc(ov_partial + (int64_t)g * ((F + 63) / 64)), 4 * (nt0 >> 1), 0, 16);
         }
         if constexpr (vst) {
             __builtin_amdgcn_fence(__ATOMIC_RELEASE, "wavefront");
@@ -502,5 +505,54 @@
 }
 
 
-}
-}
+struct BlockTailCtx {
+    BlockTail t;
+    const float *partials;
+    const float *pooled;
+    int B, F, n_xy, n_head;
+};
+template <int NTHR>
+__device__ __forceinline__ void block_tail(const BlockTailCtx &c, unsigned flags, int row_block, char *lds, int tid)
+{
+    const BlockTail &t = c.t;
+    asm volatile("s_waitcnt vmcnt(0)" ::: "memory");
+    __syncthreads();
+    unsigned *last = reinterpret_cast<unsigned *>(lds);
+    if (tid == 0) {
+        unsigned f = 0;
+        if ((flags & 1u) && __hip_atomic_fetch_add(t.words, 1u, __ATOMIC_RELAXED, __HIP_MEMORY_SCOPE_AGENT) == (unsigned)c.n_xy - 1u) f |= 1u;
+        if ((flags & 2u) && __hip_atomic_fetch_add(t.words + 1 + row_block, 1u, __ATOMIC_RELAXED, __HIP_MEMORY_SCOPE_AGENT) == (unsigned)c.n_head - 1u)
+            f |= 2u;
+        if (f) {
+            __builtin_amdgcn_fence(__ATOMIC_ACQUIRE, "agent");
+            asm volatile("s_waitcnt vmcnt(0)" ::: "memory");
+        }
+        *last = f;
+    }
+    __syncthreads();
+    const unsigned f = *last;
+    if (f == 0) return;
+    __syncthreads();
+    if (f & 1u) {
+        const int n_part = c.B * ((c.F + 63) / 64);
+        float *red = reinterpret_cast<float *>(lds);
+        if (t.head_wt) tail_sum_partials<NTHR, false>(c.partials, n_part, c.B, t.xy, red, tid);
+        else tail_sum_partials<NTHR, true>(c.partials, n_part, c.B, t.xy, red, tid);
+        if (tid == 0) __hip_atomic_store(t.words, 0u, __ATOMIC_RELAXED, __HIP_MEMORY_SCOPE_AGENT);
+        __syncthreads();
+    }
+    if (f & 2u) {
+        tail_head_logits<NTHR>(c.pooled, c.F, c.B, 4 * row_block, t.head_wt, t.ldw, t.head_bias, t.C, t.logits, t.ldl,
+                               reinterpret_cast<float *>(lds), tid);
+        if (tid == 0) __hip_atomic_store(t.words + 1 + row_block, 0u, __ATOMIC_RELAXED, __HIP_MEMORY_SCOPE_AGENT);
+    }
+}
+__device__ __forceinline__ BlockTailCtx block_tail_ctx(const FusedArgs &a)
+{
+    return BlockTailCtx{a.tail, a.part[0].ov_partial, a.part[1].pool_a, a.B, a.F, a.g_tiles * a.n_wg, a.n_wg};
+}
+constexpr int kTailMaxH = ((kLdsBytes + kEpiLdsBytes) / 4 - kTailSlices * kTailRows * 64) / kTailRows;
+
+
+}
+}
diff --git a/ed-gated-gcn_amd/csrc/fused_layer.hip b/ed-gated-gcn_amd/csrc/fused_layer.hip
--- a/ed-gated-gcn_amd/csrc/fused_layer.hip
+++ b/ed-gated-gcn_amd/csrc/fused_layer.hip
@@ -136,10 +136,11 @@
     if (bad && flag) atomicOr(flag, 1);
 }
 
-template <int SCH, bool AVEC, bool KFULL, bool FULLT, bool VST, bool STAMP = false, typename XT = float>
+template <int SCH, bool AVEC, bool KFULL, bool FULLT, bool VST, bool STAMP = false, typename XT = float, bool TAIL = false>
 __global__ __launch_bounds__(kThreads, kWavesPerSimd) void layer_fused_kernel(const FusedArgs a)
 {
     static_assert(std::is_same<XT, float>::value || (SCH == 0 && !STAMP), "bf16 features: the bf16x3 main loop");
+    static_assert(!TAIL || (std::is_same<XT, float>::value && AVEC && KFULL), "the in-launch tail: float32 features, fast shapes");
     __shared__ __attribute__((aligned(16))) char lds[kLdsBytes + kEpiLdsBytes + GGCN_LAB_LDS_PAD];
     const int B = a.B, T = a.T, K = a.K, F = a.F;
     if (a.ov_in && blockIdx.x == 0) reduce_partials(a.ov_in, B * ((F + 63) / 64), B, a.ov_out, reinterpret_cast<float *>(lds));
@@ -247,6 +248,10 @@
         else epilogue<SCH, FULLT, VST, false, false>(a, lp, acc, g0, nt0, n_tiles_total, lds, tid);
     }
     GGCN_TRACE(6);
+    if constexpr (TAIL) {
+        const unsigned arrive = (!second && a.tail.xy ? 1u : 0u) | (second && a.tail.head_wt ? 2u : 0u);
+        if (arrive) block_tail<kThreads>(block_tail_ctx(a), arrive, g_tile, lds, tid);
+    }
 }
 
 
@@ -255,34 +260,7 @@
                                                                      float *__restrict__ dst)
 {
     __shared__ float red[kRedThreads / 64];
-    const int tid = threadIdx.x;
-    float s0 = 0.0f, s1 = 0.0f, s2 = 0.0f, s3 = 0.0f;
-    const int n4 = (reinterpret_cast<uintptr_t>(part) & 15u) == 0 ? n_part / 4 : 0;
-    const float4 *p4 = reinterpret_cast<const float4 *>(part);
-    int i = tid;
-    for (; i + 3 * kRedThreads < n4; i += 4 * kRedThreads) {
-        const float4 a = p4[i], b = p4[i + kRedThreads], c = p4[i + 2 * kRedThreads], d = p4[i + 3 * kRedThreads];
-        s0 += (a.x + a.y) + (a.z + a.w);
-        s1 += (b.x + b.y) + (b.z + b.w);
-        s2 += (c.x + c.y) + (c.z + c.w);
-        s3 += (d.x + d.y) + (d.z + d.w);
-    }
-    for (; i < n4; i += kRedThreads) {
-        const float4 a = p4[i];
-        s0 += (a.x + a.y) + (a.z + a.w);
-    }
-    for (int j = 4 * n4 + tid; j < n_part; j += kRedThreads) s1 += part[j];
-    float sdot = (s0 + s1) + (s2 + s3);
-#pragma unroll
-    for (int d = 32; d >= 1; d >>= 1) sdot += __shfl_xor(sdot, d);
-    if ((tid & 63) == 0) red[tid >> 6] = sdot;
-    __syncthreads();
-    if (tid == 0) {
-        float t = 0.0f;
-#pragma unroll
-        for (int w = 0; w < kRedThreads / 64; ++w) t += red[w];
-        *dst = t / (float)B;
-    }
+    tail_sum_partials<kRedThreads, true>(part, n_part, B, dst, red, threadIdx.x);
 }
 
 __global__ __launch_bounds__(256) void rowmask_kernel(const int32_t *__restrict__ rowptr,
@@ -429,12 +407,29 @@
         else if (avec) GGCN_LAUNCH(SC, true, false, false, false);                    \
         else GGCN_LAUNCH(SC, false, false, false, false);                             \
     } while (0)
+#define GGCN_LAUNCH_T(SC, FT, VS, STM) \
+    hipLaunchKernelGGL((layer_fused_kernel<SC, true, true, FT, VS, STM, float, true>), dim3((unsigned)grid), dim3(kThreads), 0, st, a)
+#define GGCN_PICK_T(SC)                                                \
+    do {                                                               \
+        if (fullt && vst) GGCN_LAUNCH_T(SC, true, true, false);        \
+        else if (fullt) GGCN_LAUNCH_T(SC, true, false, false);         \
+        else if (vst) GGCN_LAUNCH_T(SC, false, true, false);           \
+        else GGCN_LAUNCH_T(SC, false, false, false);                   \
+    } while (0)
+    if (a.tail.words && !(a.n_parts == 2 && avec && kfull))
+        return fail(GGCN_EUNSUPPORTED, "%s: the in-launch tail takes the two-layer form on fast shapes", who);
     if (a.stamps) {
         if (!(precision == GGCN_PREC_F16MX8 && avec && kfull && fullt && vst))
             return fail(GGCN_EUNSUPPORTED, "%s: the stamped form takes f16mx8, T = 32, B %% 4 == 0, K %% 32 == 0, 16-byte rows", who);
-        hipLaunchKernelGGL((layer_fused_kernel<1, true, true, true, true, true>), dim3((unsigned)grid), dim3(kThreads), 0, st, a);
+        if (a.tail.words) GGCN_LAUNCH_T(1, true, true, true);
+        else hipLaunchKernelGGL((layer_fused_kernel<1, true, true, true, true, true>), dim3((unsigned)grid), dim3(kThreads), 0, st, a);
+    } else if (a.tail.words) {
+        if (precision == GGCN_PREC_F16MX8) GGCN_PICK_T(1);
+        else GGCN_PICK_T(0);
     } else if (precision == GGCN_PREC_F16MX8) GGCN_PICK(1);
     else GGCN_PICK(0);
+#undef GGCN_PICK_T
+#undef GGCN_LAUNCH_T
 #undef GGCN_PICK
 #undef GGCN_LAUNCH
     return check_launch(who);
@@ -577,12 +572,56 @@
     return launch_fused(who, a, GGCN_PREC_BF16X3, st);
 }
 
+namespace {
+struct BlockTailReq {
+    bool armed;
+    BlockTail t;
+    int64_t n_words;
+};
+thread_local BlockTailReq g_tail_req = {};
+BlockTailReq take_block_tail()
+{
+    const BlockTailReq r = g_tail_req;
+    g_tail_req = BlockTailReq{};
+    return r;
+}
+int block_tail_launch(const BlockTailReq &req, const float *pool_out, const float *partials, int B, int F, hipStream_t st)
+{
+    if (!req.armed) return GGCN_OK;
+    if (req.t.head_wt)
+        return dense_head(pool_out, F, req.t.head_wt, req.t.ldw, req.t.head_bias, B, F, req.t.C, req.t.logits, req.t.ldl,
+                          req.t.xy ? partials : nullptr, F, req.t.xy, st);
+    return overlap_reduce(partials, B, F, req.t.xy, st);
+}
+}
+
+int64_t block_tail_words(int B) { return B > 0 ? (1 + ((int64_t)B + 3) / 4 + 3) / 4 * 4 : 4; }
+
+int block_tail_arm(float *xy, unsigned *words, int64_t n_words, const float *head_wt, int64_t ldw, const float *head_bias, int C,
+                   float *logits, int64_t ldl)
+{
+    const char *who = "ggcn_block_tail_arm";
+    g_tail_req = BlockTailReq{};
+    if (!words) return fail(GGCN_EINVAL, "%s: null arrival words", who);
+    if (n_words < 4) return fail(GGCN_EINVAL, "%s: n_words=%lld (ggcn_block_tail_words)", who, (long long)n_words);
+    const bool head = head_wt || head_bias || logits || C != 0 || ldw != 0 || ldl != 0;
+    if (head && (!head_wt || !logits)) return fail(GGCN_EINVAL, "%s: the head's arguments go together (head_wt, C, logits; all NULL / 0 for xy alone)", who);
+    if (head && (C < 1 || C > 64)) return fail(GGCN_EINVAL, "%s: C=%d classes (one lane per class: 1..64)", who, C);
+    if (head && (ldw < C || ldl < C)) return fail(GGCN_EINVAL, "%s: leading dimension too small", who);
+    if (!head && !xy) return fail(GGCN_EINVAL, "%s: neither xy nor a logits head requested", who);
+    g_tail_req.armed = true;
+    g_tail_req.n_words = n_words;
+    g_tail_req.t = BlockTail{words, xy, head_wt, head_bias, logits, ldw, ldl, C};
+    return GGCN_OK;
+}
+
 int block_fused(const float *X, int64_t ldx, const void *wpack1, const void *wpack12, const void *graph_ops,
                 const void *graph_ops2, const float *bias1, const float *bias_mid, const float *bias2, int B, int T, int K, int F,
                 const float *gate1, const float *gate2, float *gcn1, int64_t ld1, float *x_out, int64_t ld2,
                 float *x1, float *y1, float *pool_out, float *overlap_partial, int precision, hipStream_t st,
                 unsigned long long *stamps)
 {
+    const BlockTailReq req = take_block_tail();
     if (!gate2) return fail(GGCN_EINVAL, "ggcn_block_fused: gate2 is required");
     const bool layer1 = x1 || y1 || gcn1 || overlap_partial;
     if (layer1 && (!x1 || !y1 || !gate1))
@@ -593,12 +632,27 @@
     FusedArgs a = {};
     if (!graph_ops2 || !aligned16(graph_ops2))
         return fail(GGCN_EINVAL, "ggcn_block_fused: graph_ops2 (ggcn_graph_operands2 blocks, 16-byte aligned) is required");
+    bool tail_in_launch = false;
+    if (req.armed) {
+        if (B <= 0 || F <= 0) return fail(GGCN_EINVAL, "ggcn_block_fused: B=%d F=%d must be positive", B, F);
+        if (req.t.xy && !overlap_partial) return fail(GGCN_EINVAL, "ggcn_block_fused: the armed xy needs overlap_partial");
+        if (req.t.head_wt && !pool_out) return fail(GGCN_EINVAL, "ggcn_block_fused: the armed logits head needs pool_out");
+        if (req.n_words < block_tail_words(B))
+            return fail(GGCN_EINVAL, "ggcn_block_fused: %lld arrival words armed, B=%d needs %lld (ggcn_block_tail_words)", (long long)req.n_words, B,
+                        (long long)block_tail_words(B));
+        const bool fast = X && (K % BK == 0) && (ldx % 4 == 0) && aligned16(X) && (int64_t)ldx * 4 * 257 < ((int64_t)1 << 31);
+        tail_in_launch = layer1 && !gcn1 && T <= 32 && fast && (precision == GGCN_PREC_F16MX8 || precision == GGCN_PREC_BF16X3) &&
+                         (!req.t.head_wt || F <= kTailMaxH);
+    }
+    const BlockTail *tail = tail_in_launch ? &req.t : nullptr;
     if (layer1 && !gcn1 && !stamps && precision == GGCN_PREC_F16MX8 && X && wpack1 && wpack12 && bias_mid &&
         block8_takes(X, ldx, wpack1, wpack12, B, T, K, F, gate1, gate2, bias1, bias_mid, bias2, graph_ops, graph_ops2, x_out, ld2)) {
         const char *form = getenv("GGCN_BLOCK_FORM");
-        if (!(form && form[0] == '4'))
-            return lab_block_fused8(X, ldx, wpack1, wpack12, graph_ops, graph_ops2, bias1, bias_mid, bias2, B, T, K, F, gate1, gate2, x_out,
-                                    ld2, x1, y1, pool_out, overlap_partial, st, nullptr, kBlock8RowMajor | kBlock8Product);
+        if (!(form && form[0] == '4')) {
+            const int rc = lab_block_fused8(X, ldx, wpack1, wpack12, graph_ops, graph_ops2, bias1, bias_mid, bias2, B, T, K, F, gate1, gate2, x_out,
+                                            ld2, x1, y1, pool_out, overlap_partial, st, nullptr, kBlock8RowMajor | kBlock8Product, tail);
+            return rc != GGCN_OK || tail_in_launch ? rc : block_tail_launch(req, pool_out, overlap_partial, B, F, st);
+        }
     }
     a.X = X; a.ldx = ldx; a.graph_ops = static_cast<const char *>(graph_ops); a.graph_ops2 = static_cast<const char *>(graph_ops2);
     a.B = B; a.T = T; a.K = K; a.F = F; a.n_parts = layer1 ? 2 : 1;
@@ -615,7 +669,9 @@
         if (!a.graph_ops) a.graph_ops = a.graph_ops2;
         a.part[0] = second;
     }
-    return launch_fused("ggcn_block_fused", a, precision, st);
+    if (tail) a.tail = *tail;
+    const int rc = launch_fused("ggcn_block_fused", a, precision, st);
+    return rc != GGCN_OK || tail_in_launch ? rc : block_tail_launch(req, pool_out, overlap_partial, B, F, st);
 }
 
 int block_fused_bf16(const void *X, int64_t ldx, const void *wpack1, const void *wpack12, const void *graph_ops,
diff --git a/ed-gated-gcn_amd/csrc/heads.hip b/ed-gated-gcn_amd/csrc/heads.hip
--- a/ed-gated-gcn_amd/csrc/heads.hip
+++ b/ed-gated-gcn_amd/csrc/heads.hip
@@ -1,4 +1,5 @@
 #include "common.h"
+#include "block_tail.h"
 
 namespace ggcn {
 namespace {
@@ -148,18 +149,7 @@
     const int tid = threadIdx.x, lane = tid & 63;
     const int wave = __builtin_amdgcn_readfirstlane(tid >> 6);
     if ((int)blockIdx.x >= head_blocks) {
-        float sdot = 0.0f;
-        for (int idx = tid; idx < n_part; idx += kHeadThreads) sdot += part[idx];
-#pragma unroll
-        for (int d = 32; d >= 1; d >>= 1) sdot += __shfl_xor(sdot, d);
-        if (lane == 0) head_lds[wave] = sdot;
-        __syncthreads();
-        if (tid == 0) {
-            float t = 0.0f;
-#pragma unroll
-            for (int w = 0; w < kHeadWaves; ++w) t += head_lds[w];
-            *xy = t / (float)B;
-        }
+        tail_sum_partials<kHeadThreads, false>(part, n_part, B, xy, head_lds, tid);
         head_signal(signal, tid);
         return;
     }
diff --git a/ed-gated-gcn_amd/gated_block.py b/ed-gated-gcn_amd/gated_block.py
--- a/ed-gated-gcn_amd/gated_block.py
+++ b/ed-gated-gcn_amd/gated_block.py
@@ -1,8 +1,46 @@
+import os
+
 import torch
 
 from . import _capi, range_guard
 from .csr import BatchedCSR, tensor_version
 from .gcn import BF16_PRECISIONS
+
+
+IN_LAUNCH_TAIL = os.environ.get("GGCN_BLOCK_TAIL", "1") != "0"
+_TAIL_WORDS = {}
+_TAIL_SPARES = {}
+_TAIL_BLOCK = 4096
+_TAIL_N_SPARES = 4
+
+
+def _tail_words(dev, n_words):
+    key = (dev.index, torch.cuda.current_stream(dev).cuda_stream)
+    w = _TAIL_WORDS.get(key)
+    if w is not None and w.numel() >= n_words:
+        return w
+    if torch.cuda.is_current_stream_capturing():
+        spares = _TAIL_SPARES.get(dev.index)
+        if w is not None or not spares or n_words > _TAIL_BLOCK:
+            return None
+        w = _TAIL_WORDS[key] = spares.pop()
+        return w
+    if dev.index not in _TAIL_SPARES:
+        _TAIL_SPARES[dev.index] = [torch.zeros(_TAIL_BLOCK, dtype=torch.int32, device=dev) for _ in range(_TAIL_N_SPARES)]
+        torch.cuda.current_stream(dev).synchronize()
+    w = _TAIL_WORDS[key] = torch.zeros(max(n_words, _TAIL_BLOCK), dtype=torch.int32, device=dev)
+    return w
+
+
+def _check_head(wt, bias, H):
+    if not (isinstance(wt, torch.Tensor) and wt.is_cuda and wt.dtype == torch.float32 and wt.dim() == 2 and wt.stride(1) == 1):
+        raise RuntimeError("wt must be a float32 2-D GPU tensor with unit column stride (no CPU path exists)")
+    if wt.shape[0] != H:
+        raise RuntimeError("wt must be [%d, C], got %s" % (H, tuple(wt.shape)))
+    C = wt.shape[1]
+    if bias is not None and not (bias.is_cuda and bias.dtype == torch.float32 and tuple(bias.shape) == (C,) and bias.is_contiguous()):
+        raise RuntimeError("bias must be a contiguous float32 [%d] GPU tensor" % C)
+    return C
 
 
 def gate_overlap(x1, y1):
@@ -128,9 +166,12 @@
         from .heads import dense_head as _dense_head
         if torch.is_grad_enabled() and (gc1._needs_grad(x, gate1, gate2, adj=adj) or gc2._needs_grad(x, gate2, adj=adj)):
             raise RuntimeError("dense_head= is an inference feature; under autograd apply the classifier's own dense layer")
-        r = _gated_gcn_block(x, adj, gate1, gate2, gc1, gc2, want_gcn1, one_launch, want, _defer_xy=True)
+        sig = dense_head[2] if len(dense_head) > 2 else None
+        r = _gated_gcn_block(x, adj, gate1, gate2, gc1, gc2, want_gcn1, one_launch, want, _defer_xy=True,
+                             _head=(dense_head[0], dense_head[1]) if sig is None else None)
+        if "logits" in r:
+            return r
         part = r.pop("_xy_partials", None)
-        sig = dense_head[2] if len(dense_head) > 2 else None
         if r["out"] is None:
             raise RuntimeError("dense_head= needs `out` among want=")
         if r["out"].shape[0] == 0:
@@ -188,7 +229,7 @@
     return r
 
 
-def _gated_gcn_block(x, adj, gate1, gate2, gc1, gc2, want_gcn1=False, one_launch=True, want=None, _defer_xy=False):
+def _gated_gcn_block(x, adj, gate1, gate2, gc1, gc2, want_gcn1=False, one_launch=True, want=None, _defer_xy=False, _head=None):
     want = BLOCK_OUTPUTS if want is None else tuple(want)
     bad = [k for k in want if k not in BLOCK_OUTPUTS]
     if bad:
@@ -243,19 +284,39 @@
             xy = torch.empty((), dtype=torch.float32, device=dev) if "xy" in want else None
             b1 = None if gc1.bias is None else gc1.bias.detach()
             b2 = None if gc2.bias is None else gc2.bias.detach()
+            logits = None
+            head = _head if (_head is not None and "out" in want) else None
+            tail_xy = part is not None and (not _defer_xy or head is not None)
+            words = _tail_words(dev, lib.ggcn_block_tail_words(B)) if IN_LAUNCH_TAIL and (tail_xy or head is not None) else None
+            if words is None:
+                head, tail_xy = None, False
+            else:
+                C = _check_head(head[0], head[1], F) if head is not None else 0
+                if head is not None and C > 64:
+                    head, tail_xy = None, part is not None and not _defer_xy
+                if head is not None:
+                    logits = torch.empty(B, C, dtype=torch.float32, device=dev)
+                if head is not None or tail_xy:
+                    _capi.check(lib.ggcn_block_tail_arm(_capi.ptr(xy if tail_xy else None), _capi.ptr(words), words.numel(),
+                                                        _capi.ptr(head[0]) if head is not None else None,
+                                                        head[0].stride(0) if head is not None else 0,
+                                                        _capi.ptr(head[1]) if head is not None else None, C,
+                                                        _capi.ptr(logits), C if head is not None else 0), "ggcn_block_tail_arm")
             _capi.check(lib.ggcn_block_fused(_capi.ptr(x2d), x2d.stride(0), _capi.ptr(pack1), _capi.ptr(pack12),
                                              _capi.ptr(csr.graph_ops), _capi.ptr(csr.graph_ops2(0 if kprec == "bf16x3" else 1)),
                                              _capi.ptr(b1), _capi.ptr(mid), _capi.ptr(b2),
                                              B, T, K, F, _capi.ptr(gate1 if layer1 else None), _capi.ptr(gate2), _capi.ptr(gcn1), F,
                                              _capi.ptr(xo), F, _capi.ptr(x1), _capi.ptr(y1), _capi.ptr(out),
                                              _capi.ptr(part), _capi.PREC[kprec], st), "ggcn_block_fused")
-            if part is not None and not _defer_xy:
+            if part is not None and not _defer_xy and not tail_xy:
                 _capi.check(lib.ggcn_overlap_reduce(_capi.ptr(part), B, F, _capi.ptr(xy), st), "ggcn_overlap_reduce")
         if kprec in ("f16mx8", "f16mx6"):
             range_guard.after(x.device)
         r = pick({"gcn1": None if gcn1 is None else gcn1.view(B, T, F), "x1": x1, "y1": y1, "xy": xy,
                   "x": None if xo is None else xo.view(B, T, F), "out": out})
-        if _defer_xy and part is not None:
+        if logits is not None:
+            r["logits"] = logits
+        elif _defer_xy and part is not None:
             r["_xy_partials"] = part
         return r
     if not training and one_launch and takes_bf16_block_path(x, csr, gc1, gc2):
diff --git a/include/ggcn.h b/include/ggcn.h
--- a/include/ggcn.h
+++ b/include/ggcn.h
@@ -169,6 +169,10 @@
                      float *gcn1, int64_t ld1, float *x_out, int64_t ld2,
                      float *x1, float *y1, float *pool_out, float *overlap_partial,
                      int precision, ggcn_stream_t stream);
+int ggcn_block_tail_arm(float *xy, uint32_t *words, int64_t n_words, const float *head_wt, int64_t ldw, const float *head_bias,
+                        int C, float *logits, int64_t ldl);
+int64_t ggcn_block_tail_words(int B);
+
 int ggcn_layer_fused_drop(const float *X, int64_t ldx, const void *wpack, const uint32_t *rowmask, const void *graph_ops,
                           const float *bias, int B, int T, int K, int F,
                           const float *store_gate, const float *pool_gate_a, const float *pool_gate_b,
```
